# Guanys-dar/GM-Diffusion

Hardware: AMD Instinct MI355X
Metric: HDR images/sec @ 512x512, 50 PNDM steps, dual-UNet (higher is better)
Workload: dtype bf16; 1 GPU; SD-v1-5 dual-UNet (SDR 4ch + GM 8ch) 512x512, 50 PNDM steps (51 iterations), CFG 7.5, batch 4/GPU, 2 VAE decodes + Eq.1 HDR tail; global_batch=4, per_gpu_batch=4, resolution=512, inference_steps=50, parallelism=prompt-batch sharding x1, RCCL broadcast of text hidden states + latents

## Files before the change

gm-diffusion_amd/csrc/gemm.hip:

```cpp
#include "gemm_shared.h"
#include <stdlib.h>
#include <type_traits>

namespace {

template <typename HT>
__device__ __forceinline__ void epilogue_store8(const GemmParams& p, int z, int m, int n, float (&v)[8]) {
    const bool vec_ok = (p.ldc % 8 == 0) && (p.sC % 8 == 0) && (p.residual == nullptr || (p.ldr % 8 == 0 && p.sR % 8 == 0));
    const int nvalid = p.N - n < 8 ? p.N - n : 8;
    const float* rb = p.rowbias ? p.rowbias + (int64_t)(m / p.rows_per_group) * p.ldrb : nullptr;
    const HT* res = p.residual ? (const HT*)p.residual + (int64_t)z * p.sR + (int64_t)m * p.ldr + n : nullptr;
    float rv[8];
    if (res) {
        if (nvalid == 8 && vec_ok) load_vec(res, rv);
        else
            for (int j = 0; j < 8; ++j) rv[j] = j < nvalid ? Elem<HT>::ld(res + j) : 0.f;
    }
#pragma unroll
    for (int j = 0; j < 8; ++j) {
        if (j < nvalid) {
            float x = v[j] * p.alpha;
            if (p.bias) x += p.bias[n + j];
            float add = 0.f;
            if (res) add += rv[j];
            if (rb) add += rb[n + j];
            v[j] = apply_act(x + add, p.act);
        }
    }
    const int64_t coff = (int64_t)z * p.sC + (int64_t)m * p.ldc + n;
    if (p.out_f32) {
        float* o = (float*)p.C + coff;
        if (nvalid == 8 && p.ldc % 4 == 0 && p.sC % 4 == 0) {
            *reinterpret_cast<float4*>(o) = make_float4(v[0], v[1], v[2], v[3]);
            *reinterpret_cast<float4*>(o + 4) = make_float4(v[4], v[5], v[6], v[7]);
        } else {
            for (int j = 0; j < nvalid; ++j) o[j] = v[j];
        }
    } else {
        HT* o = (HT*)p.C + coff;
        if (nvalid == 8 && vec_ok) store_vec(o, v);
        else
            for (int j = 0; j < nvalid; ++j) Elem<HT>::st(o + j, v[j]);
    }
}

template <typename HT>
__global__ __launch_bounds__(256) void splitk_reduce_kernel(const GemmParams p) {
    GMD_WG_TRACE_SCOPE(WGK_SPLITK_REDUCE);
    const int NC = (p.N + 7) / 8;
    const int64_t total = (int64_t)p.M * NC;
    const int64_t slab = (int64_t)p.M * p.N;
    for (int64_t i = (int64_t)blockIdx.x * blockDim.x + threadIdx.x; i < total; i += (int64_t)gridDim.x * blockDim.x) {
        const int m = (int)(i / NC), n = (int)(i - (int64_t)m * NC) * 8;
        const int nvalid = p.N - n < 8 ? p.N - n : 8;
        float v[8];
#pragma unroll
        for (int j = 0; j < 8; ++j) v[j] = 0.f;
        const float* src = p.ws + (int64_t)m * p.N + n;
        for (int s = 0; s < p.ksplit; ++s, src += slab) {
            if (nvalid == 8 && p.N % 4 == 0) {
                const float4 a = *reinterpret_cast<const float4*>(src), b = *reinterpret_cast<const float4*>(src + 4);
                v[0] += a.x; v[1] += a.y; v[2] += a.z; v[3] += a.w; v[4] += b.x; v[5] += b.y; v[6] += b.z; v[7] += b.w;
            } else {
                for (int j = 0; j < nvalid; ++j) v[j] += src[j];
            }
        }
        epilogue_store8<HT>(p, 0, m, n, v);
    }
}

template <typename HT, int TM, int TN>
__device__ __forceinline__ void epilogue_regs(const GemmParams& p, const f32x4 (&acc)[TM][TN], int mw, int nw, int frow, int fq,
                                              int z, int ks) {
    const bool vec_c = (p.ldc % 4 == 0) && (p.sC % 4 == 0);
    const bool vec_r = p.residual != nullptr && (p.ldr % 4 == 0) && (p.sR % 4 == 0);
    const bool vec_n = (p.N % 4 == 0);
    const bool vec_rb = vec_n && (p.ldrb % 4 == 0) && ((reinterpret_cast<uintptr_t>(p.rowbias) & 15) == 0);
    float bz[TN][4];
#pragma unroll
    for (int j = 0; j < TN; ++j) {
        const int n = nw + j * 16 + fq * 4;
        bz[j][0] = bz[j][1] = bz[j][2] = bz[j][3] = 0.f;
        if (p.bias && p.ksplit <= 1 && n < p.N) {
            if (n + 4 <= p.N && vec_n) {
                const float4 t = *reinterpret_cast<const float4*>(p.bias + n);
                bz[j][0] = t.x; bz[j][1] = t.y; bz[j][2] = t.z; bz[j][3] = t.w;
            } else {
                for (int e = 0; e < 4; ++e) if (n + e < p.N) bz[j][e] = p.bias[n + e];
            }
        }
    }
    if constexpr (TN % 2 == 0) {
        if (p.act == GMD_ACT_GEGLU) {
#pragma unroll
            for (int i = 0; i < TM; ++i) {
                const int m = mw + i * 16 + frow;
                if (m >= p.M) continue;
#pragma unroll
                for (int j = 0; j < TN; j += 2) {
                    const int n = nw + j * 16 + fq * 4;
                    if (n >= p.N) continue;
                    float o4[4];
#pragma unroll
                    for (int e = 0; e < 4; ++e) {
                        const float h = acc[i][j][e] * p.alpha + bz[j][e];
                        const float g = acc[i][j + 1][e] * p.alpha + bz[j + 1][e];
                        o4[e] = h * (0.5f * g * (1.0f + fast_erf(g * 0.70710678118654752440f)));
                    }
                    const int no = (nw + j * 16) / 2 + fq * 4;
                    HT* o = (HT*)p.C + (int64_t)z * p.sC + (int64_t)m * p.ldc + no;
                    *reinterpret_cast<uint2*>(o) = make_uint2(Half<HT>::pack2(o4[0], o4[1]), Half<HT>::pack2(o4[2], o4[3]));
                }
            }
            return;
        }
    }
#pragma unroll
    for (int i = 0; i < TM; ++i) {
        const int m = mw + i * 16 + frow;
        if (m >= p.M) continue;
        const float* rb = p.rowbias ? p.rowbias + (int64_t)(m / p.rows_per_group) * p.ldrb : nullptr;
#pragma unroll
        for (int j = 0; j < TN; ++j) {
            const int n = nw + j * 16 + fq * 4;
            if (n >= p.N) continue;
            const int nvalid = p.N - n < 4 ? p.N - n : 4;
            float v[4] = {acc[i][j][0], acc[i][j][1], acc[i][j][2], acc[i][j][3]};
            if (p.ksplit > 1) {
                float* o = p.ws + ((int64_t)ks * p.M + m) * p.N + n;
                if (nvalid == 4 && vec_n) *reinterpret_cast<float4*>(o) = make_float4(v[0], v[1], v[2], v[3]);
                else
                    for (int e = 0; e < nvalid; ++e) o[e] = v[e];
                continue;
            }
            float rv[4] = {0.f, 0.f, 0.f, 0.f};
            if (p.residual) {
                const HT* res = (const HT*)p.residual + (int64_t)z * p.sR + (int64_t)m * p.ldr + n;
                if (nvalid == 4 && vec_r) {
                    const uint2 w = *reinterpret_cast<const uint2*>(res);
                    Half<HT>::unpack2(w.x, rv[0], rv[1]);
                    Half<HT>::unpack2(w.y, rv[2], rv[3]);
                } else {
                    for (int e = 0; e < nvalid; ++e) rv[e] = Elem<HT>::ld(res + e);
                }
            }
            if (rb) {
                if (nvalid == 4 && vec_rb) {
                    const float4 t = *reinterpret_cast<const float4*>(rb + n);
                    rv[0] += t.x; rv[1] += t.y; rv[2] += t.z; rv[3] += t.w;
                } else {
                    for (int e = 0; e < nvalid; ++e) rv[e] += rb[n + e];
                }
            }
#pragma unroll
            for (int e = 0; e < 4; ++e) v[e] = apply_act(v[e] * p.alpha + bz[j][e] + rv[e], p.act);
            const int64_t coff = (int64_t)z * p.sC + (int64_t)m * p.ldc + n;
            if (p.out_f32) {
                float* o = (float*)p.C + coff;
                if (nvalid == 4 && vec_c) *reinterpret_cast<float4*>(o) = make_float4(v[0], v[1], v[2], v[3]);
                else
                    for (int e = 0; e < nvalid; ++e) o[e] = v[e];
            } else {
                HT* o = (HT*)p.C + coff;
                if (nvalid == 4 && vec_c) *reinterpret_cast<uint2*>(o) = make_uint2(Half<HT>::pack2(v[0], v[1]), Half<HT>::pack2(v[2], v[3]));
                else
                    for (int e = 0; e < nvalid; ++e) Elem<HT>::st(o + e, v[e]);
            }
        }
    }
}

template <typename HT, int TM, int TN>
__device__ __forceinline__ void epilogue_cols_vt(const GemmParams& p, const f32x4 (&acc)[TM][TN], float* strip, int mw, int nw, int lane) {
    constexpr int NCOL = TN * 16, ROWF = NCOL + 4;
    const int frow = lane & 15, fq = lane >> 4;
    const int b = mw / p.vt_tokens, tok0 = mw - b * p.vt_tokens;
#pragma unroll
    for (int h = 0; h < TM / 2; ++h) {
#pragma unroll
        for (int i2 = 0; i2 < 2; ++i2)
#pragma unroll
            for (int j = 0; j < TN; ++j)
                *reinterpret_cast<float4*>(strip + (i2 * 16 + frow) * ROWF + j * 16 + fq * 4) =
                    make_float4(acc[2 * h + i2][j][0], acc[2 * h + i2][j][1], acc[2 * h + i2][j][2], acc[2 * h + i2][j][3]);
        __builtin_amdgcn_wave_barrier();
#pragma unroll
        for (int k = 0; k < (NCOL + 63) / 64; ++k) {
            const int cc = lane + 64 * k < NCOL ? lane + 64 * k : NCOL - 1;
            const float bz = p.bias ? p.bias[nw + cc] : 0.f;
            unsigned pk[16];
#pragma unroll
            for (int r = 0; r < 32; r += 2)
                pk[r / 2] = Half<HT>::pack2(strip[r * ROWF + cc] * p.alpha + bz, strip[(r + 1) * ROWF + cc] * p.alpha + bz);
            if (lane + 64 * k < NCOL) {
                HT* o = (HT*)p.vt_out + ((int64_t)b * (p.N - p.vt_col0) + (nw + cc - p.vt_col0)) * p.vt_ld + tok0 + h * 32;
#pragma unroll
                for (int q = 0; q < 4; ++q) *reinterpret_cast<uint4*>(o + 8 * q) = make_uint4(pk[4 * q], pk[4 * q + 1], pk[4 * q + 2], pk[4 * q + 3]);
            }
        }
        __builtin_amdgcn_wave_barrier();
    }
}

template <typename HT, int TM, int TN, bool PLAIN>
__device__ __forceinline__ void epilogue_rows_impl(const GemmParams& p, const f32x4 (&acc)[TM][TN], float* strip, int mw, int nw, int lane,
                                                   int z) {
    static_assert(TM % 2 == 0, "halves of two 16-row tiles");
    if (p.vt_out && nw >= p.vt_col0) {
        epilogue_cols_vt<HT, TM, TN>(p, acc, strip, mw, nw, lane);
        return;
    }
    constexpr int NCOL = TN * 16, ROWF = NCOL + 4, CH = NCOL / 8;
    constexpr int ITER = (32 * CH + 63) / 64;
    const int frow = lane & 15, fq = lane >> 4;
    int g0 = 0, grem = 0;
    if (p.rowbias) {
        g0 = mw / p.rows_per_group;
        grem = mw - g0 * p.rows_per_group;
    }
    float cs[(NCOL + 63) / 64] = {}, cq[(NCOL + 63) / 64] = {};
#if defined(GMD_PP_DIAG) && defined(GMD_WG_TRACE)
    unsigned long long et[6] = {0, 0, 0, 0, 0, 0};
    int eti = 0;
#define EPI_STAMP() { unsigned long long t_; asm volatile("s_memrealtime %0\n\ts_waitcnt lgkmcnt(0)" : "=s"(t_)::"memory"); if (eti < 6) et[eti++] = t_; }
#else
#define EPI_STAMP()
#endif
    EPI_STAMP()
    static_assert(NCOL / 4 <= 32, "one bias float4 per strip row");
    uint4 resv[2][ITER];
    if (lane < NCOL / 4)
        *reinterpret_cast<float4*>(strip + lane * ROWF + NCOL) = p.bias ? *reinterpret_cast<const float4*>(p.bias + nw + lane * 4) : make_float4(0.f, 0.f, 0.f, 0.f);
    const bool rb_pre = PLAIN && p.rowbias != nullptr && p.residual == nullptr;
    auto request_residual = [&](int hh) {
#pragma unroll
        for (int t = 0; t < ITER; ++t) {
            const int idx = lane + 64 * t;
            const int r = idx / CH, c = idx - r * CH;
            if (32 * CH % 64 != 0 && r >= 32) continue;
            resv[hh & 1][t] = *reinterpret_cast<const uint4*>((const HT*)p.residual + (int64_t)z * p.sR + (int64_t)(mw + hh * 32 + r) * p.ldr + nw + c * 8);
        }
    };
    const bool res_pre = PLAIN && p.residual != nullptr;
    if (res_pre) request_residual(0);
#pragma unroll
    for (int h = 0; h < TM / 2; ++h) {
        if (rb_pre) {
#pragma unroll
            for (int t = 0; t < ITER; ++t) {
                const int idx = lane + 64 * t;
                const int r = idx / CH, c = idx - r * CH;
                if (32 * CH % 64 != 0 && r >= 32) continue;
                const int ro = h * 32 + r;
                const int grp = p.rows_per_group >= 64 ? g0 + (grem + ro >= p.rows_per_group ? 1 : 0) : (mw + ro) / p.rows_per_group;
                const float* rb = p.rowbias + (int64_t)grp * p.ldrb + nw + c * 8;
                resv[0][t] = __builtin_bit_cast(uint4, *reinterpret_cast<const float4*>(rb));
                resv[1][t] = __builtin_bit_cast(uint4, *reinterpret_cast<const float4*>(rb + 4));
            }
        }
#pragma unroll
        for (int i2 = 0; i2 < 2; ++i2)
#pragma unroll
            for (int j = 0; j < TN; ++j)
                *reinterpret_cast<float4*>(strip + (i2 * 16 + frow) * ROWF + j * 16 + fq * 4) =
                    make_float4(acc[2 * h + i2][j][0], acc[2 * h + i2][j][1], acc[2 * h + i2][j][2], acc[2 * h + i2][j][3]);
        __builtin_amdgcn_wave_barrier();
        EPI_STAMP()
        if (res_pre && h + 1 < TM / 2) request_residual(h + 1);
#pragma unroll
        for (int t = 0; t < ITER; ++t) {
            const int idx = lane + 64 * t;
            const int r = idx / CH, c = idx - r * CH;
            if (32 * CH % 64 != 0 && r >= 32) continue;
            const int m = mw + h * 32 + r, n = nw + c * 8;
            const float4 a0 = *reinterpret_cast<const float4*>(strip + r * ROWF + c * 8);
            const float4 a1 = *reinterpret_cast<const float4*>(strip + r * ROWF + c * 8 + 4);
            float v[8] = {a0.x, a0.y, a0.z, a0.w, a1.x, a1.y, a1.z, a1.w};
            float add[8] = {0.f, 0.f, 0.f, 0.f, 0.f, 0.f, 0.f, 0.f};
            if (p.residual) {
                const uint4 w = PLAIN ? resv[h & 1][t] : *reinterpret_cast<const uint4*>((const HT*)p.residual + (int64_t)z * p.sR + (int64_t)m * p.ldr + n);
                const unsigned ww[4] = {w.x, w.y, w.z, w.w};
#pragma unroll
                for (int e = 0; e < 4; ++e) Half<HT>::unpack2(ww[e], add[2 * e], add[2 * e + 1]);
            }
            if (rb_pre) {
                const float4 t0 = __builtin_bit_cast(float4, resv[0][t]), t1 = __builtin_bit_cast(float4, resv[1][t]);
                add[0] += t0.x; add[1] += t0.y; add[2] += t0.z; add[3] += t0.w; add[4] += t1.x; add[5] += t1.y; add[6] += t1.z; add[7] += t1.w;
            } else if (p.rowbias) {
                const int ro = h * 32 + r;
                const int grp = p.rows_per_group >= 64 ? g0 + (grem + ro >= p.rows_per_group ? 1 : 0) : m / p.rows_per_group;
                const float* rb = p.rowbias + (int64_t)grp * p.ldrb + n;
                const float4 t0 = *reinterpret_cast<const float4*>(rb), t1 = *reinterpret_cast<const float4*>(rb + 4);
                add[0] += t0.x; add[1] += t0.y; add[2] += t0.z; add[3] += t0.w; add[4] += t1.x; add[5] += t1.y; add[6] += t1.z; add[7] += t1.w;
            }
            const float4 b0 = *reinterpret_cast<const float4*>(strip + (2 * c) * ROWF + NCOL), b1 = *reinterpret_cast<const float4*>(strip + (2 * c + 1) * ROWF + NCOL);
            const float bz[8] = {b0.x, b0.y, b0.z, b0.w, b1.x, b1.y, b1.z, b1.w};
#pragma unroll
            for (int e = 0; e < 8; ++e) v[e] = apply_act(v[e] * p.alpha + bz[e] + add[e], PLAIN ? GMD_ACT_NONE : p.act);
            HT* o = (HT*)p.C + (int64_t)z * p.sC + (int64_t)m * p.ldc + n;
            const uint4 packed = make_uint4(Half<HT>::pack2(v[0], v[1]), Half<HT>::pack2(v[2], v[3]), Half<HT>::pack2(v[4], v[5]), Half<HT>::pack2(v[6], v[7]));
#if defined(GMD_EPI_NOSTORE)
            if (packed.x == 0x12345678u && packed.y == 0x9abcdef0u) *reinterpret_cast<uint4*>(o) = packed;
#elif defined(GMD_EPI_NT)
            __builtin_nontemporal_store(__builtin_bit_cast(u32x4, packed), reinterpret_cast<u32x4*>(o));
#else
            *reinterpret_cast<uint4*>(o) = packed;
#endif
            asm volatile("" ::: "memory");
            __builtin_amdgcn_sched_barrier(0);
            if (p.colstats) {
                const unsigned pw[4] = {packed.x, packed.y, packed.z, packed.w};
                float rv[8];
#pragma unroll
                for (int e = 0; e < 4; ++e) Half<HT>::unpack2(pw[e], rv[2 * e], rv[2 * e + 1]);
                *reinterpret_cast<float4*>(strip + r * ROWF + c * 8) = make_float4(rv[0], rv[1], rv[2], rv[3]);
                *reinterpret_cast<float4*>(strip + r * ROWF + c * 8 + 4) = make_float4(rv[4], rv[5], rv[6], rv[7]);
            }
        }
        __builtin_amdgcn_wave_barrier();
        EPI_STAMP()
        if (p.colstats) {
            colstats_pass<NCOL, ROWF>(strip, lane, cs, cq);
            __builtin_amdgcn_wave_barrier();
        }
    }
#if defined(GMD_PP_DIAG) && defined(GMD_WG_TRACE)
    if (threadIdx.x == 0 && g_wg_trace != nullptr) {
        GmdWgTraceHeader* hh = g_wg_trace;
        const unsigned hw = __builtin_amdgcn_s_getreg((31 << 11) | 4), xcc = __builtin_amdgcn_s_getreg((31 << 11) | 20);
        const unsigned shard = ((((xcc & 7u) * 8u + ((hw >> 13) & 7u)) * 2u + ((hw >> 12) & 1u)) * 16u) + ((hw >> 8) & 15u);
        unsigned long long* counters = reinterpret_cast<unsigned long long*>(hh + 1);
        const unsigned long long i2 = __hip_atomic_fetch_add(counters + 16ull * shard, 1ull, __ATOMIC_RELAXED, __HIP_MEMORY_SCOPE_WORKGROUP);
        if (i2 < hh->capacity) {
            uint4* rec = reinterpret_cast<uint4*>(counters + 16ull * hh->shards) + 2ull * (shard * hh->capacity + i2);
            rec[0] = make_uint4((unsigned)(et[1] - et[0]), (unsigned)(et[2] - et[1]), (unsigned)(et[3] - et[2]), (unsigned)(et[4] - et[3]));
            rec[1] = make_uint4(hw, (xcc & 15u) | ((unsigned)(WGK_PP | 0x80) << 8) | (0xFEu << 16), (unsigned)TN << 16, p.residual ? 1u : 0u);
        }
    }
#endif
#undef EPI_STAMP
    if (p.colstats)
        colstats_store<NCOL, ROWF>(strip, lane, cs, cq, p.cs_bucket,
                                   p.colstats + ((int64_t)(mw / (TM * 16)) * (p.N / p.cs_bucket) + nw / p.cs_bucket) * 2);
}

template <typename HT, int TM, int TN>
__device__ __forceinline__ void epilogue_rows(const GemmParams& p, const f32x4 (&acc)[TM][TN], float* strip, int mw, int nw, int lane, int z) {
    if (__builtin_expect(p.act == GMD_ACT_NONE, 1)) epilogue_rows_impl<HT, TM, TN, true>(p, acc, strip, mw, nw, lane, z);
    else epilogue_rows_impl<HT, TM, TN, false>(p, acc, strip, mw, nw, lane, z);
}

template <int TM, int TN>
__device__ __forceinline__ void epilogue_rows_slab(const GemmParams& p, const f32x4 (&acc)[TM][TN], float* strip, int mw, int nw, int lane,
                                                   int ks) {
    static_assert(TM == 4, "two halves of two 16-row tiles");
    constexpr int NCOL = TN * 16, ROWF = NCOL + 4, CH = NCOL / 4;
    constexpr int ITER = (32 * CH + 63) / 64;
    const int frow = lane & 15, fq = lane >> 4;
    float* slab = p.ws + (int64_t)ks * p.M * p.N;
#pragma unroll
    for (int h = 0; h < 2; ++h) {
#pragma unroll
        for (int i2 = 0; i2 < 2; ++i2)
#pragma unroll
            for (int j = 0; j < TN; ++j)
                *reinterpret_cast<float4*>(strip + (i2 * 16 + frow) * ROWF + j * 16 + fq * 4) =
                    make_float4(acc[2 * h + i2][j][0], acc[2 * h + i2][j][1], acc[2 * h + i2][j][2], acc[2 * h + i2][j][3]);
        __builtin_amdgcn_wave_barrier();
#pragma unroll
        for (int t = 0; t < ITER; ++t) {
            const int idx = lane + 64 * t;
            const int r = idx / CH, c = idx - r * CH;
            if (32 * CH % 64 != 0 && r >= 32) continue;
            *reinterpret_cast<float4*>(slab + (int64_t)(mw + h * 32 + r) * p.N + nw + c * 4) =
                *reinterpret_cast<const float4*>(strip + r * ROWF + c * 4);
        }
        __builtin_amdgcn_wave_barrier();
    }
}

template <int TM, int TN, int NCONS>
__device__ __forceinline__ bool splitk_fixup(const GemmParams& p, f32x4 (&acc)[TM][TN], int ks, int wid, int lane) {
    constexpr unsigned FR = TM * TN;
    const unsigned tile = blockIdx.x, ntiles = gridDim.x;
    const int last = p.ksplit - 1;
    unsigned* cnt = p.fix_cnt + tile;
    const __amdgpu_buffer_rsrc_t rs = __builtin_amdgcn_make_buffer_rsrc(p.ws, 0, (int)p.fix_bytes, 0x00020000);
    const unsigned wave_off = ((tile * NCONS + (unsigned)wid) * FR) * 1024u + (unsigned)lane * 16u;
    const unsigned slice_bytes = ntiles * NCONS * FR * 1024u;
    if (ks != last) {
        const unsigned base = (unsigned)ks * slice_bytes + wave_off;
#pragma unroll
        for (int i = 0; i < TM; ++i)
#pragma unroll
            for (int j = 0; j < TN; ++j)
                __builtin_amdgcn_raw_buffer_store_b128(__builtin_bit_cast(u32x4, acc[i][j]), rs, base + (unsigned)(i * TN + j) * 1024u, 0, 16 );
        asm volatile("s_waitcnt vmcnt(0)" ::: "memory");
        __syncthreads();
        if (threadIdx.x == 0) __hip_atomic_fetch_add(cnt, 1u, __ATOMIC_RELAXED, __HIP_MEMORY_SCOPE_AGENT);
        return false;
    }
    if (threadIdx.x == 0) {
        int spins = 0;
        while (__hip_atomic_load(cnt, __ATOMIC_RELAXED, __HIP_MEMORY_SCOPE_AGENT) != (unsigned)last && ++spins < (1 << 21)) __builtin_amdgcn_s_sleep(8);
    }
    __syncthreads();
    static_assert(TM % 2 == 0, "fragment rows are fetched in pairs");
#pragma unroll
    for (int i = 0; i < TM; i += 2) {
        f32x4 t[2][TN];
#pragma unroll
        for (int ii = 0; ii < 2; ++ii)
#pragma unroll
            for (int j = 0; j < TN; ++j)
                t[ii][j] = __builtin_bit_cast(f32x4, __builtin_amdgcn_raw_buffer_load_b128(rs, wave_off + (unsigned)((i + ii) * TN + j) * 1024u, 0, 16 ));
        for (int s = 1; s < last; ++s) {
#pragma unroll
            for (int ii = 0; ii < 2; ++ii) {
                f32x4 u[TN];
#pragma unroll
                for (int j = 0; j < TN; ++j)
                    u[j] = __builtin_bit_cast(f32x4, __builtin_amdgcn_raw_buffer_load_b128(rs, (unsigned)s * slice_bytes + wave_off + (unsigned)((i + ii) * TN + j) * 1024u, 0, 16));
#pragma unroll
                for (int j = 0; j < TN; ++j) {
                    t[ii][j] += u[j];
                    asm volatile("" : "+v"(t[ii][j])::"memory");
// ... 426 lines not shown
        if (CONV) {
            c0 += BK;
            if (c0 >= cb0 + p.cblk) {
                c0 = cb0;
                ++tap;
                newtap = true;
                if (tap == 9) { tap = 0; cb0 += p.cblk; c0 = cb0; }
            }
        }
    };
    auto wait_tiles = [&](int ahead) {
        if (ahead <= 0) { wait_vmcnt<0>(); return; }
        if (w_last) {
            if (ahead == 1) wait_vmcnt<NA + NW>();
            else wait_vmcnt<2 * (NA + NW)>();
        } else {
            if (ahead == 1) wait_vmcnt<NA + NW - 1>();
            else wait_vmcnt<2 * (NA + NW - 1)>();
        }
    };

    const int frow = lane & 15, fq = lane >> 4;
    auto compute = [&](int stage_idx) {
        const unsigned char* sA = smem + stage_idx * kStage;
        const unsigned char* sW = sA + BM * 128;
#pragma unroll
        for (int s2 = 0; s2 < 2; ++s2) {
            uint4 a[TM], b[TN];
#pragma unroll
            for (int i = 0; i < TM; ++i) a[i] = *reinterpret_cast<const uint4*>(sA + lds_off(wr * 64 + i * 16 + frow, 4 * s2 + fq));
#pragma unroll
            for (int j = 0; j < TN; ++j) b[j] = *reinterpret_cast<const uint4*>(sW + lds_off(wc * (TN * 16) + j * 16 + frow, 4 * s2 + fq));
#pragma unroll
            for (int i = 0; i < TM; ++i)
#pragma unroll
                for (int j = 0; j < TN; ++j) acc[i][j] = Half<HT>::mfma16(b[j], a[i], acc[i][j]);
        }
    };

    if (nk > 0) {
#pragma unroll
        for (int t = 0; t < D; ++t)
            if (t < nk) dma_tile(t, t);
        int st_cur = 0, st_fill = D % NST;
        for (int kt = 0; kt < nk; ++kt) {
            const int rem = nk - 1 - kt;
            wait_tiles(rem < D - 1 ? rem : D - 1);
            __syncthreads();
            if (kt + D < nk) dma_tile(kt + D, st_fill);
            compute(st_cur);
            st_cur = st_cur + 1 == NST ? 0 : st_cur + 1;
            st_fill = st_fill + 1 == NST ? 0 : st_fill + 1;
        }
    }
    const bool rows_ok = !p.out_f32 && p.ksplit <= 1 && p.act != GMD_ACT_GEGLU && m0 + BM <= p.M && n0 + BN <= p.N && (p.ldc & 7) == 0 &&
                         (p.sC & 7) == 0 && (p.residual == nullptr || ((p.ldr & 7) == 0 && (p.sR & 7) == 0)) &&
                         (p.rowbias == nullptr || ((p.ldrb & 3) == 0 && (reinterpret_cast<uintptr_t>(p.rowbias) & 15) == 0)) &&
                         (reinterpret_cast<uintptr_t>(p.bias) & 15) == 0;
    if constexpr (TN % 2 == 0) {
        if (p.act == GMD_ACT_GEGLU && !p.out_f32 && p.ksplit <= 1 && m0 + BM <= p.M && n0 + BN <= p.N && (p.ldc & 7) == 0 && (p.sC & 7) == 0 &&
            (reinterpret_cast<uintptr_t>(p.bias) & 15) == 0) {
            __syncthreads();
            constexpr int kStripG = 32 * (TN * 8 + 4);
            epilogue_rows_geglu<HT, TM, TN>(p, acc, reinterpret_cast<float*>(smem) + wid * kStripG, m0 + wr * 64, n0 + wc * (TN * 16), lane, z);
            return;
        }
    }
    if (p.ksplit > 1 && m0 + BM <= p.M && n0 + BN <= p.N && (p.N & 3) == 0) {
        __syncthreads();
        constexpr int kStripS = 32 * (TN * 16 + 4);
        epilogue_rows_slab<TM, TN>(p, acc, reinterpret_cast<float*>(smem) + wid * kStripS, m0 + wr * 64, n0 + wc * (TN * 16), lane, ks);
        return;
    }
    if (__builtin_expect(rows_ok, 1)) {
        __syncthreads();
        constexpr int kStrip = 32 * (TN * 16 + 4);
        static_assert((size_t)NWAVES * kStrip * 4 <= (size_t)NST * kStage, "epilogue strips must fit in the ring stages");
        epilogue_rows<HT, TM, TN>(p, acc, reinterpret_cast<float*>(smem) + wid * kStrip, m0 + wr * 64, n0 + wc * (TN * 16), lane, z);
    } else {
        epilogue_regs<HT, TM, TN>(p, acc, m0 + wr * 64, n0 + wc * (TN * 16), frow, fq, z, ks);
    }
}

template <typename HT, bool CONV, int TN>
__global__ __launch_bounds__(768, 3) void gemm_pp_kernel(const GemmParams p) {
    GMD_WG_TRACE_SCOPE(WGK_PP | (CONV ? WGK_CONV_BIT : 0));
    constexpr int WN = 2, NCONS = 8, LW = 4, TM = 4, NST = 3;
    constexpr int BM = 256, BN = WN * TN * 16;
    constexpr int RPP = LW * 8;
    constexpr int NA = BM / RPP;
    constexpr int NW = BN / RPP;
    constexpr int NP = NA + NW;
    static_assert(BN % RPP == 0, "W tile rows must be whole staging passes");
    extern __shared__ __attribute__((aligned(16))) unsigned char smem[];
    constexpr int kStage = (BM + BN) * 128;

    const int tid = threadIdx.x, lane = tid & 63, wid = tid >> 6;
    const int wuni = __builtin_amdgcn_readfirstlane(wid);
    const bool loader = wuni >= NCONS;
    const bool late = wuni >= 4 && !loader;
    int m0, n0;
    {
        const int nwg = gridDim.x, id = blockIdx.x;
        const int q = nwg >> 3, r = nwg & 7, xcd = id & 7, j = id >> 3;
        const int L = (xcd < r ? xcd * (q + 1) : r * (q + 1) + (xcd - r) * q) + j;
        const int tiles_n = (p.N + BN - 1) / BN, tiles_m = (p.M + BM - 1) / BM;
        int mt, nt;
        grouped_tile(L, tiles_m, tiles_n, p.tile_group, mt, nt);
        m0 = mt * BM;
        n0 = nt * BN;
    }
    const int z = p.ksplit > 1 ? 0 : blockIdx.z;
    const int ks = p.ksplit > 1 ? blockIdx.z : 0;
    const int nk_total = p.K / BK;
    const int per = (nk_total + p.ksplit - 1) / p.ksplit;
    const int kt_begin = ks * per;
    const int nk = (kt_begin + per <= nk_total ? per : nk_total - kt_begin);

    auto seg_barrier = [&]() {
        __builtin_amdgcn_sched_barrier(0);
        __builtin_amdgcn_s_barrier();
        __builtin_amdgcn_sched_barrier(0);
    };
#ifdef GMD_PP_DIAG
    unsigned long long dg[8] = {0, 0, 0, 0, 0, 0, 0, 0}, dprev = 0, dreal0 = 0, dtime0 = 0;
    auto stamp_now = [&]() {
        unsigned long long t;
        __builtin_amdgcn_sched_barrier(0);
        asm volatile("s_memtime %0\n\ts_waitcnt lgkmcnt(0)" : "=s"(t)::"memory");
        __builtin_amdgcn_sched_barrier(0);
        return t;
    };
    auto diag_begin = [&]() {
        dprev = stamp_now();
        dtime0 = dprev;
        asm volatile("s_memrealtime %0\n\ts_waitcnt lgkmcnt(0)" : "=s"(dreal0)::"memory");
    };
    auto diag_end = [&]() {
        unsigned long long dreal1;
        asm volatile("s_memrealtime %0\n\ts_waitcnt lgkmcnt(0)" : "=s"(dreal1)::"memory");
        dg[7] = dreal1 - dreal0;
#ifdef GMD_WG_TRACE
        if (lane == 0 && g_wg_trace != nullptr) {
            GmdWgTraceHeader* h = g_wg_trace;
            const unsigned hw = __builtin_amdgcn_s_getreg((31 << 11) | 4), xcc = __builtin_amdgcn_s_getreg((31 << 11) | 20);
            const unsigned shard = ((((xcc & 7u) * 8u + ((hw >> 13) & 7u)) * 2u + ((hw >> 12) & 1u)) * 16u) + ((hw >> 8) & 15u);
            unsigned long long* counters = reinterpret_cast<unsigned long long*>(h + 1);
            const unsigned long long i = __hip_atomic_fetch_add(counters + 16ull * shard, 1ull, __ATOMIC_RELAXED, __HIP_MEMORY_SCOPE_WORKGROUP);
            if (i < h->capacity) {
                uint4* rec = reinterpret_cast<uint4*>(counters + 16ull * h->shards) + 2ull * (shard * h->capacity + i);
                const unsigned a0 = (unsigned)(loader ? dg[1] : dg[0]), a1 = (unsigned)dg[3], a2 = (unsigned)(loader ? 0 : dg[4]), a3 = (unsigned)(loader ? dg[6] : dg[5]);
                rec[0] = make_uint4(a0, a1, a2, a3);
                rec[1] = make_uint4(hw, (xcc & 15u) | ((unsigned)((WGK_PP | (CONV ? WGK_CONV_BIT : 0)) | 0x80) << 8) | ((unsigned)wid << 16), (unsigned)nk | ((unsigned)TN << 16),
                                    (unsigned)(dprev - dtime0));
            }
        }
#else
        if (p.ws && lane == 0) {
            unsigned long long* o = reinterpret_cast<unsigned long long*>(p.ws) + ((size_t)blockIdx.x * (NCONS + LW) + wid) * 10;
            for (int k = 0; k < 8; ++k) o[k] = dg[k];
            o[8] = dprev - dtime0;
            o[9] = (unsigned long long)nk;
        }
#endif
    };
#define PP_STAMP(k) { const unsigned long long t_ = stamp_now(); dg[k] += t_ - dprev; dprev = t_; }
#else
#define PP_STAMP(k)
#endif

    if (loader) {
        const int lw = wuni - NCONS;
        const int ltid = tid - NCONS * 64;
        const int srow = ltid >> 3;
        const int chunk = (ltid & 7) ^ ((srow >> 1) & 7);
        unsigned aoff[NA], woff[NW];
        int pb[NA], py[NA], px[NA];
        bool pv[NA];
#pragma unroll
        for (int i = 0; i < NA; ++i) {
            const int m = m0 + srow + RPP * i;
            pv[i] = m < p.M;
            pb[i] = py[i] = px[i] = 0;
            if (CONV) {
                if (pv[i]) {
                    const int hw = p.Hout * p.Wout;
                    if (((hw & (hw - 1)) | (p.Wout & (p.Wout - 1))) == 0) {
                        const int sh = __builtin_ctz(hw), sw = __builtin_ctz(p.Wout);
                        pb[i] = m >> sh;
                        const int rem = m & (hw - 1);
                        py[i] = rem >> sw;
                        px[i] = rem & (p.Wout - 1);
                    } else {
                        pb[i] = m / hw;
                        const int rem = m - pb[i] * hw;
                        py[i] = rem / p.Wout;
                        px[i] = rem - py[i] * p.Wout;
                    }
                }
                aoff[i] = kOOB;
            } else {
                aoff[i] = pv[i] ? (unsigned)m * (unsigned)p.lda * 2u + (unsigned)chunk * 16u : kOOB;
            }
        }
#pragma unroll
        for (int i = 0; i < NW; ++i) {
            const int n = n0 + srow + RPP * i;
            woff[i] = n < p.N ? (unsigned)n * (unsigned)p.ldw * 2u + (unsigned)chunk * 16u : kOOB;
        }
        int tap = 0, c0 = 0, cb0 = 0;
        bool newtap = true;
        if (CONV) {
            const int sb = p.cblk / BK, per_cb = 9 * sb, nconv = 9 * (p.Cin / BK);
            if (kt_begin >= nconv) {
                tap = 9;
                cb0 = p.Cin;
                c0 = (kt_begin - nconv) * BK;
            } else {
                const int cbi = kt_begin / per_cb, rem = kt_begin - cbi * per_cb;
                tap = rem / sb;
                cb0 = cbi * p.cblk;
                c0 = cb0 + (rem - tap * sb) * BK;
            }
        }
        const unsigned lds_base = __builtin_amdgcn_readfirstlane((unsigned)(size_t)(__attribute__((address_space(3))) void*)smem);
        u32x4 dA, dW;
        {
            const uint64_t ba = (uint64_t)((const bf16_t*)p.A + (int64_t)z * p.sA), bw = (uint64_t)((const bf16_t*)p.W + (int64_t)z * p.sW);
            dA = u32x4{(unsigned)__builtin_amdgcn_readfirstlane((unsigned)ba), (unsigned)__builtin_amdgcn_readfirstlane((unsigned)(ba >> 32) & 0xffffu),
                       (unsigned)__builtin_amdgcn_readfirstlane(p.a_bytes), 0x00020000u};
            dW = u32x4{(unsigned)__builtin_amdgcn_readfirstlane((unsigned)bw), (unsigned)__builtin_amdgcn_readfirstlane((unsigned)(bw >> 32) & 0xffffu),
                       (unsigned)__builtin_amdgcn_readfirstlane(p.w_bytes), 0x00020000u};
        }
        u32x4 dA2 = dA;
        if (CONV && p.K2 > 0) {
            const uint64_t b2 = (uint64_t)p.A2;
            dA2 = u32x4{(unsigned)__builtin_amdgcn_readfirstlane((unsigned)b2), (unsigned)__builtin_amdgcn_readfirstlane((unsigned)(b2 >> 32) & 0xffffu),
                        (unsigned)__builtin_amdgcn_readfirstlane(p.a2_bytes), 0x00020000u};
        }
        auto dma16 = [&](const u32x4& desc, unsigned lds_addr, unsigned voff, unsigned soff) {
#pragma clang diagnostic push
#pragma clang diagnostic ignored "-Winline-asm"
            asm volatile("s_mov_b32 m0, %1\n\ts_nop 0\n\tbuffer_load_dwordx4 %0, %2, %3 offen lds"
                         :
                         : "v"(voff), "s"(lds_addr), "s"(desc), "s"(soff)
                         : "memory", "m0");
#pragma clang diagnostic pop
        };
        auto dma_part = [&](auto QC, int kt, int stage_idx) {
            constexpr int Q = decltype(QC)::value;
            constexpr int lo = Q == 4 ? 0 : Q * NP / 4, hi = Q == 4 ? NP : (Q + 1) * NP / 4;
            unsigned kbytes = (unsigned)(kt_begin + kt) * (BK * 2);
            unsigned abytes = kbytes;
            const bool tail = CONV && tap == 9;
            if (CONV) {
                if ((Q == 0 || Q == 4) && newtap) {
                    if (tail) {
#pragma unroll
                        for (int i = 0; i < NA; ++i)
                            aoff[i] = pv[i] ? (unsigned)(m0 + srow + RPP * i) * (unsigned)p.lda2 * 2u + (unsigned)chunk * 16u : kOOB;
                    } else {
                        const int ky = tap / 3, kx = tap - ky * 3;
#pragma unroll
                        for (int i = 0; i < NA; ++i) aoff[i] = conv_tap_offset<CONV>(p, pv[i], pb[i], py[i], px[i], ky, kx, chunk);
                    }
                    newtap = false;
                }
                abytes = (unsigned)c0 * 2u;
                kbytes = (unsigned)((tail ? 9 * p.Cin : tap * p.Cin) + c0) * 2u;
            }
            const u32x4 dAs = tail ? dA2 : dA;
            const unsigned stage = lds_base + (unsigned)stage_idx * kStage + (unsigned)lw * (8 * 128);
#pragma unroll
            for (int i = 0; i < NA; ++i)
                if (i >= lo && i < hi) dma16(dAs, stage + i * (RPP * 128), aoff[i], abytes);
#pragma unroll
            for (int i = 0; i < NW; ++i)
                if (NA + i >= lo && NA + i < hi) dma16(dW, stage + BM * 128 + i * (RPP * 128), woff[i], kbytes);
            if (CONV && (Q == 3 || Q == 4)) {
                c0 += BK;
                if (tap < 9 && c0 >= cb0 + p.cblk) {
                    c0 = cb0;
                    ++tap;
                    newtap = true;
                    if (tap == 9) {
                        cb0 += p.cblk;
                        if (cb0 >= p.Cin) c0 = 0;
                        else { tap = 0; c0 = cb0; }
                    }
                }
            }
        };
        if (nk > 0) {
            dma_part(IntC<4>{}, 0, 0);
            if (nk > 1) {
                dma_part(IntC<4>{}, 1, 1);
                wait_vmcnt<NP>();
            } else {
                wait_vmcnt<0>();
            }
            seg_barrier();
            int st_fill = 2;
#ifdef GMD_PP_DIAG
            diag_begin();
#endif
            for (int kt = 0; kt < nk; ++kt) {
                const bool more = kt + 2 < nk;
                if (more) dma_part(IntC<0>{}, kt + 2, st_fill);
                PP_STAMP(1)
                seg_barrier();
                PP_STAMP(3)
                if (more) dma_part(IntC<1>{}, kt + 2, st_fill);
                PP_STAMP(1)
                seg_barrier();
                PP_STAMP(3)
                if (more) dma_part(IntC<2>{}, kt + 2, st_fill);
                PP_STAMP(1)
                seg_barrier();
                PP_STAMP(3)
                if (more) dma_part(IntC<3>{}, kt + 2, st_fill);
                PP_STAMP(1)
                if (more) wait_vmcnt<NP>();
                else wait_vmcnt<0>();
                PP_STAMP(6)
                seg_barrier();
                PP_STAMP(3)
                st_fill = st_fill == NST - 1 ? 0 : st_fill + 1;
            }
#ifdef GMD_PP_DIAG
            diag_end();
#endif
            seg_barrier();
        }
        __syncthreads();
        return;
    }

    const int wr = wid / WN, wc = wid % WN;
    f32x4 acc[TM][TN];
#pragma unroll
    for (int i = 0; i < TM; ++i)
#pragma unroll
        for (int j = 0; j < TN; ++j) acc[i][j] = f32x4{0.f, 0.f, 0.f, 0.f};
    const int frow = lane & 15, fq = lane >> 4;
    uint4 fa[TM], fb[TN];
    auto frag_reads = [&](int stage_idx, int s2) {
        const unsigned char* sA = smem + stage_idx * kStage;
        const unsigned char* sW = sA + BM * 128;
#pragma unroll
        for (int i = 0; i < TM; ++i) fa[i] = *reinterpret_cast<const uint4*>(sA + lds_off(wr * 64 + i * 16 + frow, 4 * s2 + fq));
#pragma unroll
        for (int j = 0; j < TN; ++j) fb[j] = *reinterpret_cast<const uint4*>(sW + lds_off(wc * (TN * 16) + j * 16 + frow, 4 * s2 + fq));
    };
    auto mfmas = [&]() {
#pragma unroll
        for (int i = 0; i < TM; ++i)
#pragma unroll
            for (int j = 0; j < TN; ++j) acc[i][j] = Half<HT>::mfma16(fb[j], fa[i], acc[i][j]);
    };
    auto lgkm0 = [&]() { asm volatile("s_waitcnt lgkmcnt(0)" ::: "memory"); };

    if (nk > 0) {
        seg_barrier();
        if (late) seg_barrier();
        int st = 0;
#ifdef GMD_PP_DIAG
        diag_begin();
#endif
        for (int kt = 0; kt < nk; ++kt) {
#pragma unroll
            for (int s2 = 0; s2 < 2; ++s2) {
                frag_reads(st, s2);
                lgkm0();
                PP_STAMP(0)
                seg_barrier();
                PP_STAMP(3)
                __builtin_amdgcn_s_setprio(1);
                mfmas();
                __builtin_amdgcn_s_setprio(0);
                PP_STAMP(4)
                seg_barrier();
                PP_STAMP(5)
            }
            st = st == NST - 1 ? 0 : st + 1;
        }
#ifdef GMD_PP_DIAG
        diag_end();
#endif
        if (!late) seg_barrier();
    }
#if defined(GMD_PP_DIAG) && defined(GMD_WG_TRACE)
    unsigned long long ph_sync = 0;
    auto real_now = [&]() { unsigned long long t; asm volatile("s_memrealtime %0\n\ts_waitcnt lgkmcnt(0)" : "=s"(t)::"memory"); return t; };
    auto phase_emit = [&]() {
        if (wid != 0 || lane != 0 || g_wg_trace == nullptr || nk <= 0) return;
        const unsigned long long t_end = real_now();
        GmdWgTraceHeader* h = g_wg_trace;
        const unsigned hw = __builtin_amdgcn_s_getreg((31 << 11) | 4), xcc = __builtin_amdgcn_s_getreg((31 << 11) | 20);
        const unsigned shard = ((((xcc & 7u) * 8u + ((hw >> 13) & 7u)) * 2u + ((hw >> 12) & 1u)) * 16u) + ((hw >> 8) & 15u);
        unsigned long long* counters = reinterpret_cast<unsigned long long*>(h + 1);
        const unsigned long long i2 = __hip_atomic_fetch_add(counters + 16ull * shard, 1ull, __ATOMIC_RELAXED, __HIP_MEMORY_SCOPE_WORKGROUP);
        if (i2 < h->capacity) {
            uint4* rec = reinterpret_cast<uint4*>(counters + 16ull * h->shards) + 2ull * (shard * h->capacity + i2);
            rec[0] = make_uint4((unsigned)(dreal0 - gmd_wg_trace_scope_.t0), (unsigned)dg[7], (unsigned)(ph_sync - (dreal0 + dg[7])), (unsigned)(t_end - ph_sync));
            rec[1] = make_uint4(hw, (xcc & 15u) | ((unsigned)((WGK_PP | (CONV ? WGK_CONV_BIT : 0)) | 0x80) << 8) | (0xFFu << 16), (unsigned)nk | ((unsigned)TN << 16),
                                (gridDim.x * gridDim.z) | ((unsigned)p.ksplit << 20) | (p.residual ? (1u << 28) : 0u) | (p.fixup ? (1u << 29) : 0u));
        }
    };
#define PP_PHASE_SYNC() ph_sync = real_now()
#define PP_PHASE_EMIT() phase_emit()
#else
#define PP_PHASE_SYNC()
#define PP_PHASE_EMIT()
#endif
    __syncthreads();
    GemmParams q = p;
    if (p.fixup) {
        if (!splitk_fixup<TM, TN, NCONS>(p, acc, ks, wid, lane)) return;
        q.ksplit = 1;
    }
    PP_PHASE_SYNC();
    const bool rows_ok = !q.out_f32 && q.ksplit <= 1 && q.act != GMD_ACT_GEGLU && m0 + BM <= q.M && n0 + BN <= q.N && (q.ldc & 7) == 0 &&
                         (q.sC & 7) == 0 && (q.residual == nullptr || ((q.ldr & 7) == 0 && (q.sR & 7) == 0)) &&
                         (q.rowbias == nullptr || ((q.ldrb & 3) == 0 && (reinterpret_cast<uintptr_t>(q.rowbias) & 15) == 0)) &&
                         (reinterpret_cast<uintptr_t>(q.bias) & 15) == 0;
    if constexpr (TN % 2 == 0) {
        if (q.act == GMD_ACT_GEGLU && !q.out_f32 && q.ksplit <= 1 && m0 + BM <= q.M && n0 + BN <= q.N && (q.ldc & 7) == 0 && (q.sC & 7) == 0 &&
            (reinterpret_cast<uintptr_t>(q.bias) & 15) == 0) {
            constexpr int kStripG = 32 * (TN * 8 + 4);
            epilogue_rows_geglu<HT, TM, TN>(q, acc, reinterpret_cast<float*>(smem) + wid * kStripG, m0 + wr * 64, n0 + wc * (TN * 16), lane, z);
            PP_PHASE_EMIT();
            return;
        }
    }
    if (__builtin_expect(q.ksplit > 1 && m0 + BM <= q.M && n0 + BN <= q.N && (q.N & 3) == 0, 0)) {
        constexpr int kStripS = 32 * (TN * 16 + 4);
        epilogue_rows_slab<TM, TN>(q, acc, reinterpret_cast<float*>(smem) + wid * kStripS, m0 + wr * 64, n0 + wc * (TN * 16), lane, ks);
        PP_PHASE_EMIT();
        return;
    }
    if (__builtin_expect(rows_ok, 1)) {
        constexpr int kStrip = 32 * (TN * 16 + 4);
        static_assert((size_t)NCONS * kStrip * 4 <= (size_t)NST * kStage, "epilogue strips must fit in the ring stages");
        epilogue_rows<HT, TM, TN>(q, acc, reinterpret_cast<float*>(smem) + wid * kStrip, m0 + wr * 64, n0 + wc * (TN * 16), lane, z);
    } else {
        epilogue_regs<HT, TM, TN>(q, acc, m0 + wr * 64, n0 + wc * (TN * 16), frow, fq, z, ks);
    }
    PP_PHASE_EMIT();
}
#undef PP_STAMP
#undef PP_PHASE_SYNC
#undef PP_PHASE_EMIT

template <typename HT, bool CONV, int TM, int TN>
__global__ __launch_bounds__(512, 2) void gemm_lc_kernel(const GemmParams p) {
    GMD_WG_TRACE_SCOPE(WGK_LC | (CONV ? WGK_CONV_BIT : 0));
    constexpr int WN = 2, NCONS = 4, LW = 4, NST = 4;
    constexpr int BM = 2 * TM * 16, BN = WN * TN * 16;
    constexpr int RPP = LW * 8;
    constexpr int NA = BM / RPP, NW = BN / RPP, NP = NA + NW;
    static_assert(BM % RPP == 0 && BN % RPP == 0, "tile rows must be whole staging passes");
    extern __shared__ __attribute__((aligned(16))) unsigned char smem[];
    constexpr int kStage = (BM + BN) * 128;

    const int tid = threadIdx.x, lane = tid & 63, wid = tid >> 6;
    const int wuni = __builtin_amdgcn_readfirstlane(wid);
    const bool loader = wuni >= NCONS;
    int m0, n0;
    {
        const int nwg = gridDim.x, id = blockIdx.x;
        const int q = nwg >> 3, r = nwg & 7, xcd = id & 7, j = id >> 3;
        const int L = (xcd < r ? xcd * (q + 1) : r * (q + 1) + (xcd - r) * q) + j;
        const int tiles_n = (p.N + BN - 1) / BN, tiles_m = (p.M + BM - 1) / BM;
        int mt, nt;
        grouped_tile(L, tiles_m, tiles_n, p.tile_group, mt, nt);
        m0 = mt * BM;
        n0 = nt * BN;
    }
    const int z = p.ksplit > 1 ? 0 : blockIdx.z;
    const int ks = p.ksplit > 1 ? blockIdx.z : 0;
    const int nk_total = p.K / BK;
    const int per = (nk_total + p.ksplit - 1) / p.ksplit;
    const int kt_begin = ks * per;
    const int nk = (kt_begin + per <= nk_total ? per : nk_total - kt_begin);
    auto seg_barrier = [&]() {
        __builtin_amdgcn_sched_barrier(0);
        __builtin_amdgcn_s_barrier();
        __builtin_amdgcn_sched_barrier(0);
    };

    if (loader) {
        const int lw = wuni - NCONS;
        const int ltid = tid - NCONS * 64;
        const int srow = ltid >> 3;
        const int chunk = (ltid & 7) ^ ((srow >> 1) & 7);
        unsigned aoff[NA], woff[NW];
        int pb[NA], py[NA], px[NA];
        bool pv[NA];
#pragma unroll
        for (int i = 0; i < NA; ++i) {
            const int m = m0 + srow + RPP * i;
            pv[i] = m < p.M;
            pb[i] = py[i] = px[i] = 0;
            if (CONV) {
// ... 711 lines not shown
        for (int j = 0; j < 4; ++j) {
            const int n = n0 + tx * 4 + j;
            if (n >= p.N) continue;
            float x = acc[i][j] * p.alpha;
            if (p.bias) x += p.bias[n];
            if (rb) x += rb[n];
            if (res) x += res[n];
            o[n] = apply_act(x, p.act);
        }
    }
}

template <typename HT, bool CONV, int BM, int BN, int PF>
hipError_t launch_bf16(const GemmParams& p, int gz, hipStream_t s) {
    constexpr size_t smem = 2 * (BM + BN) * 128;
    if (smem > 64 * 1024) {
        hipError_t e = opt_in_lds(reinterpret_cast<const void*>(&gemm_bf16_kernel<HT, CONV, BM, BN, PF>), (int)smem);
        if (e != hipSuccess) return e;
    }
    dim3 grid(((p.N + BN - 1) / BN) * ((p.M + BM - 1) / BM), 1, gz);
    gemm_bf16_kernel<HT, CONV, BM, BN, PF><<<grid, 256, smem, s>>>(p);
    return hipGetLastError();
}

template <typename HT, bool CONV, int WM, int WN, int TN, int NST>
hipError_t launch_ring(const GemmParams& p, int gz, hipStream_t s) {
    constexpr int BM = WM * 64, BN = WN * TN * 16;
    constexpr size_t smem = (size_t)NST * (BM + BN) * 128;
    if (smem > 64 * 1024) {
        hipError_t e = opt_in_lds(reinterpret_cast<const void*>(&gemm_ring_kernel<HT, CONV, WM, WN, TN, NST>), (int)smem);
        if (e != hipSuccess) return e;
    }
    dim3 grid(((p.N + BN - 1) / BN) * ((p.M + BM - 1) / BM), 1, gz);
    gemm_ring_kernel<HT, CONV, WM, WN, TN, NST><<<grid, WM * WN * 64, smem, s>>>(p);
    return hipGetLastError();
}

template <typename HT, bool CONV, int TM, int TN>
hipError_t launch_lc(const GemmParams& p, int gz, hipStream_t s) {
    constexpr int BM = 2 * TM * 16, BN = 2 * TN * 16;
    constexpr size_t smem = (size_t)4 * (BM + BN) * 128;
    hipError_t e = opt_in_lds(reinterpret_cast<const void*>(&gemm_lc_kernel<HT, CONV, TM, TN>), (int)smem);
    if (e != hipSuccess) return e;
    dim3 grid(((p.N + BN - 1) / BN) * ((p.M + BM - 1) / BM), 1, gz);
    gemm_lc_kernel<HT, CONV, TM, TN><<<grid, 512, smem, s>>>(p);
    return hipGetLastError();
}

template <typename HT, int TN>
hipError_t launch_conv_patch(const GemmParams& p, bool continuous, int gz, hipStream_t s) {
    constexpr int BM = 256, BN = 2 * TN * 16;
    const int H = p.Hin, W = p.Win, HW = H * W;
    const int R = HW >= 256 ? 256 / W : H, nimg = 256 / (R * W);
    const int npieces = (nimg * (R + 2) * (W + 2) + 7) / 8;
    const size_t smem = (size_t)2 * npieces * 1024 + (size_t)3 * BN * 128;
    const size_t strips = (size_t)8 * 32 * (TN * 16 + 4) * 4;
    const size_t need = smem > strips ? smem : strips;
    dim3 grid(((p.N + BN - 1) / BN) * ((p.M + BM - 1) / BM), 1, gz);
    hipError_t e;
    if (continuous) {
        if (npieces > 44) {
            e = opt_in_lds(reinterpret_cast<const void*>(&conv_patch_cont_kernel<HT, TN, 13>), 163840);
            if (e != hipSuccess) return e;
            conv_patch_cont_kernel<HT, TN, 13><<<grid, 768, need, s>>>(p);
        } else {
            e = opt_in_lds(reinterpret_cast<const void*>(&conv_patch_cont_kernel<HT, TN, 11>), 163840);
            if (e != hipSuccess) return e;
            conv_patch_cont_kernel<HT, TN, 11><<<grid, 768, need, s>>>(p);
        }
        return hipGetLastError();
    }
    if (npieces > 44) {
        e = opt_in_lds(reinterpret_cast<const void*>(&conv_patch_kernel<HT, TN, 13>), 163840);
        if (e != hipSuccess) return e;
        conv_patch_kernel<HT, TN, 13><<<grid, 768, need, s>>>(p);
    } else {
        e = opt_in_lds(reinterpret_cast<const void*>(&conv_patch_kernel<HT, TN, 11>), 163840);
        if (e != hipSuccess) return e;
        conv_patch_kernel<HT, TN, 11><<<grid, 768, need, s>>>(p);
    }
    return hipGetLastError();
}

template <typename HT, bool CONV, int TN>
hipError_t launch_pp(const GemmParams& p, int gz, hipStream_t s) {
    constexpr int BM = 256, BN = 2 * TN * 16;
    constexpr size_t smem = (size_t)3 * (BM + BN) * 128;
    hipError_t e = opt_in_lds(reinterpret_cast<const void*>(&gemm_pp_kernel<HT, CONV, TN>), (int)smem);
    if (e != hipSuccess) return e;
    dim3 grid(((p.N + BN - 1) / BN) * ((p.M + BM - 1) / BM), 1, gz);
    gemm_pp_kernel<HT, CONV, TN><<<grid, 768, smem, s>>>(p);
    return hipGetLastError();
}

template <typename HT, bool CONV>
int launch_half(GemmParams p, int batch, void* ws, int64_t ws_bytes, hipStream_t s, const char* name) {
    constexpr bool kTune = std::is_same<HT, bf16_t>::value;
    hipError_t e = hipSuccess;
    const PlanConfig cfg = plan_config();
    const int64_t usable = ws ? ws_bytes : 0;
    const Plan pl = make_plan(cfg, p.M, p.N, p.K, batch, usable, p.act == GMD_ACT_GEGLU, p.colstats != nullptr);
    if (p.vt_out && !qkv_vt_plan_ok(pl, p.M, p.N, batch, p.vt_col0, p.vt_tokens)) {
        gmd_set_error("%s: plan %dx%d ksplit=%d cannot write transposed V tiles (ask gmd_gemm_qkv_vt_ok first)", name, pl.bm, pl.bn, pl.ksplit);
        return GMD_ERR_UNSUPPORTED;
    }
    if (const char* why = plan_unsupported(cfg, pl, p, batch, usable)) {
        gmd_set_error("%s: plan %dx%d pf=%d ksplit=%d (M=%d N=%d bucket=%d) %s", name, pl.bm, pl.bn, pl.pf, pl.ksplit, p.M, p.N, p.cs_bucket, why);
        return GMD_ERR_UNSUPPORTED;
    }
    if (CONV && p.K2 > 0 && !(pl.pf == kPingPong && pl.bm == 256 && (pl.bn == 160 || pl.bn == 128))) {
        gmd_set_error("%s: plan %dx%d pf=%d has no K-tail loader (M=%d N=%d K=%d): only the 256-row ping-pong kernel does", name, pl.bm, pl.bn,
                      pl.pf, p.M, p.N, p.K);
        return GMD_ERR_INVALID;
    }
    p.ksplit = pl.ksplit;
    p.ws = (float*)ws;
    p.tile_group = CONV ? 1 : pick_tile_group(pl, p.M, p.N, p.K);
    const int gz = pl.ksplit > 1 ? pl.ksplit : batch;
    p.fixup = 0;
    if (fixup_plan_ok(cfg, pl, p.M, p.N, usable, p.defer_reduce != 0)) {
        p.fixup = 1;
        p.fix_bytes = (unsigned)fixup_bytes(pl, p.M, p.N);
        p.fix_cnt = reinterpret_cast<unsigned*>(reinterpret_cast<char*>(ws) + ws_bytes);
    }
    bool done = false;
    if (pl.pf == kLoaderConsumer) {
        if (pl.bm == 128 && pl.bn == 160) e = launch_lc<HT, CONV, 4, 5>(p, gz, s);
        else if (pl.bm == 128 && pl.bn == 128) e = launch_lc<HT, CONV, 4, 4>(p, gz, s);
        else if (pl.bm == 64 && pl.bn == 160) e = launch_lc<HT, CONV, 2, 5>(p, gz, s);
        else if (pl.bm == 64 && pl.bn == 128) e = launch_lc<HT, CONV, 2, 4>(p, gz, s);
        else { gmd_set_error("%s: loader/consumer tile %dx%d is not instantiated", name, pl.bm, pl.bn); return GMD_ERR_UNSUPPORTED; }
        done = true;
    } else if (CONV && (p.K2 == 0 || cfg.conv_patch_mode == 2) && use_conv_patch(cfg, pl, p)) {
        if (pl.bn == 160) e = launch_conv_patch<HT, 5>(p, cfg.conv_patch_mode == 2, gz, s);
        else if (pl.bn == 128) e = launch_conv_patch<HT, 4>(p, cfg.conv_patch_mode == 2, gz, s);
        else { gmd_set_error("%s: ping-pong tile %dx%d is not instantiated", name, pl.bm, pl.bn); return GMD_ERR_UNSUPPORTED; }
        done = true;
    } else if (pl.pf == kPingPong) {
        if (pl.bm == 256 && pl.bn == 160) e = launch_pp<HT, CONV, 5>(p, gz, s);
        else if (pl.bm == 256 && pl.bn == 128) e = launch_pp<HT, CONV, 4>(p, gz, s);
        else { gmd_set_error("%s: ping-pong tile %dx%d is not instantiated", name, pl.bm, pl.bn); return GMD_ERR_UNSUPPORTED; }
        done = true;
    } else if constexpr (kTune) {
        done = true;
        if (pl.pf == 143 && pl.bn == 160) e = launch_ring<HT, CONV, 4, 2, 5, 3>(p, gz, s);
        else if (pl.pf == 143 && pl.bn == 128) e = launch_ring<HT, CONV, 4, 2, 4, 3>(p, gz, s);
        else if (pl.pf == 123 && pl.bn == 160) e = launch_ring<HT, CONV, 2, 2, 5, 3>(p, gz, s);
        else if (pl.pf == 124 && pl.bn == 160) e = launch_ring<HT, CONV, 2, 2, 5, 4>(p, gz, s);
        else if (pl.pf == 122 && pl.bn == 160) e = launch_ring<HT, CONV, 2, 2, 5, 2>(p, gz, s);
        else if (pl.pf == 122 && pl.bn == 128) e = launch_ring<HT, CONV, 2, 2, 4, 2>(p, gz, s);
        else if (pl.pf == 123 && pl.bn == 128) e = launch_ring<HT, CONV, 2, 2, 4, 3>(p, gz, s);
        else if (pl.pf == 124 && pl.bn == 128) e = launch_ring<HT, CONV, 2, 2, 4, 4>(p, gz, s);
        else if (pl.pf == 103 && pl.bm == 64 && pl.bn == 64) e = launch_ring<HT, CONV, 1, 4, 1, 3>(p, gz, s);
        else if (pl.pf == 104 && pl.bm == 64 && pl.bn == 64) e = launch_ring<HT, CONV, 1, 4, 1, 4>(p, gz, s);
        else if (pl.pf == 103 && pl.bm == 64 && pl.bn == 128) e = launch_ring<HT, CONV, 1, 4, 2, 3>(p, gz, s);
        else if (pl.pf == 104 && pl.bm == 64 && pl.bn == 128) e = launch_ring<HT, CONV, 1, 4, 2, 4>(p, gz, s);
        else if (is_ring_variant(pl.pf)) { gmd_set_error("%s: ring variant %d not instantiated for BN=%d", name, pl.pf, pl.bn); return GMD_ERR_UNSUPPORTED; }
        else if (pl.pf != kRing && pl.bm == 128 && pl.bn == 160)
            e = pl.pf == kRegStaged1 ? launch_bf16<HT, CONV, 128, 160, 1>(p, gz, s) : launch_bf16<HT, CONV, 128, 160, 2>(p, gz, s);
        else if (pl.pf != kRing && pl.bm == 128 && pl.bn == 128)
            e = pl.pf == kRegStaged1 ? launch_bf16<HT, CONV, 128, 128, 1>(p, gz, s) : launch_bf16<HT, CONV, 128, 128, 2>(p, gz, s);
        else if (pl.pf != kRing && !(pl.bm == 128))
            e = pl.pf == kRegStaged1 ? launch_bf16<HT, CONV, 64, 64, 1>(p, gz, s) : launch_bf16<HT, CONV, 64, 64, 2>(p, gz, s);
        else done = false;
    } else if (pl.pf != kRing) {
        gmd_set_error("%s: plan override pf=%d is instantiated for bfloat16 only", name, pl.pf);
        return GMD_ERR_UNSUPPORTED;
    }
    if (!done) {
        if (pl.bm == 128 && pl.bn == 160) e = launch_ring<HT, CONV, 2, 2, 5, 2>(p, gz, s);
        else if (pl.bm == 128 && pl.bn == 128) e = launch_ring<HT, CONV, 2, 2, 4, 2>(p, gz, s);
        else if (pl.bm == 64 && pl.bn == 64) e = launch_bf16<HT, CONV, 64, 64, 0>(p, gz, s);
        else { gmd_set_error("%s: tile %dx%d is not instantiated", name, pl.bm, pl.bn); return GMD_ERR_UNSUPPORTED; }
    }
    if (e == hipSuccess && pl.ksplit > 1 && !p.defer_reduce && !p.fixup) {
        const int64_t total = (int64_t)p.M * ((p.N + 7) / 8);
        int64_t g = (total + 255) / 256;
        if (g > 4096) g = 4096;
        splitk_reduce_kernel<HT><<<(int)g, 256, 0, s>>>(p);
        e = hipGetLastError();
    }
    if (e != hipSuccess) {
        gmd_set_error("%s: launch failed: %s", name, hipGetErrorString(e));
        return GMD_ERR_LAUNCH;
    }
    return GMD_OK;
}

template <bool CONV>
int launch(GemmParams p, int dtype, int batch, void* ws, int64_t ws_bytes, hipStream_t s, const char* name) {
    if (dtype == GMD_BF16) return launch_half<bf16_t, CONV>(p, batch, ws, ws_bytes, s, name);
    if (dtype == GMD_F16) return launch_half<f16_t, CONV>(p, batch, ws, ws_bytes, s, name);
    if (p.colstats) {
        gmd_set_error("%s: column statistics are implemented for the 16-bit types only", name);
        return GMD_ERR_UNSUPPORTED;
    }
    p.ksplit = 1;
    p.ws = nullptr;
    dim3 grid((p.N + 63) / 64, (p.M + 63) / 64, batch);
    gemm_f32_kernel<CONV><<<grid, 256, 0, s>>>(p);
    const hipError_t e = hipGetLastError();
    if (e != hipSuccess) {
        gmd_set_error("%s: launch failed: %s", name, hipGetErrorString(e));
        return GMD_ERR_LAUNCH;
    }
    return GMD_OK;
}

}

extern "C" {

int gmd_gemm_qkv_vt(const void* A, const void* W, void* C, void* Vt, int dtype, int M, int N, int K, int64_t ldc, int vt_col0, int vt_tokens,
                    int64_t vt_ld, float alpha, void* workspace, int64_t workspace_bytes, gmd_stream_t stream) {
    workspace_bytes = gmd_ws_usable_bytes(workspace_bytes);
    const bool split = dtype == GMD_F32SW || dtype == GMD_F32SA;
    GMD_REQUIRE(gmd_is_half(dtype) || split, "gmd_gemm_qkv_vt: the 16-bit types and GMD_F32SW / GMD_F32SA only (dtype %d)", dtype);
    GMD_REQUIRE(M > 0 && N > 0 && K > 0 && K % (split ? 32 : 64) == 0, "gmd_gemm_qkv_vt: bad shape M=%d N=%d K=%d", M, N, K);
    GMD_REQUIRE(A && W && C && Vt && gmd_aligned16(A) && gmd_aligned16(W) && gmd_aligned16(C) && gmd_aligned16(Vt), "gmd_gemm_qkv_vt: null or unaligned pointer");
    GMD_REQUIRE(vt_col0 > 0 && vt_col0 < N && ldc >= vt_col0 && ldc % 8 == 0 && vt_tokens > 0 && M % vt_tokens == 0 && vt_ld >= vt_tokens && vt_ld % 8 == 0,
                "gmd_gemm_qkv_vt: bad V geometry (vt_col0=%d ldc=%lld tokens=%d vt_ld=%lld)", vt_col0, (long long)ldc, vt_tokens, (long long)vt_ld);
    GMD_REQUIRE(!split || ((reinterpret_cast<uintptr_t>(W) & 127) == 0 && (dtype != GMD_F32SA || (reinterpret_cast<uintptr_t>(A) & 127) == 0)),
                "gmd_gemm_qkv_vt: a pre-split operand must be 128-byte aligned (32-element chunks of [hi | lo])");
    GMD_REQUIRE(qkv_vt_ok(plan_config(), dtype, M, N, K, vt_col0, vt_tokens, workspace ? workspace_bytes : 0), "gmd_gemm_qkv_vt: this launch cannot write transposed V tiles (ask gmd_gemm_qkv_vt_ok)");
    GemmParams p{};
    p.A = A; p.W = W; p.C = C; p.M = M; p.N = N; p.K = K;
    p.lda = K; p.ldw = K; p.ldc = ldc;
    {
        const int es = split ? 4 : 2;
        const int64_t ab = (int64_t)M * K * es, wb = (int64_t)N * K * es;
        GMD_REQUIRE(ab < 0xFFFF0000LL && wb < 0xFFFF0000LL, "gmd_gemm_qkv_vt: operand slab larger than 4 GiB");
        p.a_bytes = (unsigned)ab; p.w_bytes = (unsigned)wb;
    }
    p.rows_per_group = 1; p.ldrb = N; p.alpha = alpha; p.act = GMD_ACT_NONE; p.cblk = K;
    p.vt_out = Vt; p.vt_col0 = vt_col0; p.vt_tokens = vt_tokens; p.vt_ld = vt_ld;
    if (split) {
        p.out_f32 = 1;
        return gmd_launch_split_gemm(p, dtype == GMD_F32SA ? 2 : 1, 1, workspace, workspace_bytes, (hipStream_t)stream, "gmd_gemm_qkv_vt");
    }
    return launch<false>(p, dtype, 1, workspace, workspace_bytes, (hipStream_t)stream, "gmd_gemm_qkv_vt");
}

int gmd_gemm_nt(const void* A, const void* W, void* C, int dtype, int out_dtype, int M, int N, int K, int64_t lda,
                int64_t ldw, int64_t ldc, int batch, int64_t strideA, int64_t strideW, int64_t strideC, const float* bias,
                const float* rowbias, int rows_per_group, int64_t ldrb, const void* residual, int64_t ldr, int64_t strideR, float alpha,
                int act, float* colstats, int colstats_bucket, void* workspace, int64_t workspace_bytes, gmd_stream_t stream) {
    workspace_bytes = gmd_ws_usable_bytes(workspace_bytes);
    const bool split = gmd_is_split(dtype);
    GMD_REQUIRE(dtype == GMD_BF16 || dtype == GMD_F16 || dtype == GMD_F32 || split, "gmd_gemm_nt: bad dtype %d", dtype);
    const bool is16 = gmd_is_half(dtype);
    const bool c_split = split && out_dtype == GMD_F32SA;
    GMD_REQUIRE(out_dtype == GMD_F32 || (!split && out_dtype == dtype) || c_split, "gmd_gemm_nt: out_dtype must be F32 or the input dtype");
    GMD_REQUIRE(M >= 0 && N >= 0 && K > 0 && batch >= 0, "gmd_gemm_nt: bad shape M=%d N=%d K=%d batch=%d", M, N, K, batch);
    if (c_split) {
        const int nout = act == GMD_ACT_GEGLU ? N / 2 : N;
        GMD_REQUIRE(batch == 1 && nout % 32 == 0 && ldc == nout && !colstats && f32_out_ok(M, N, K, act == GMD_ACT_GEGLU, workspace ? workspace_bytes : 0),
                    "gmd_gemm_nt: this launch cannot store its output pre-split (ask gmd_gemm_out_split_ok; ldc must equal the row length)");
    }
    if (M == 0 || N == 0 || batch == 0) return GMD_OK;
    const int kmul = is16 ? 64 : split ? 32 : 4, vec = is16 ? 8 : 4;
    GMD_REQUIRE(K % kmul == 0, "gmd_gemm_nt: K=%d must be a multiple of %d", K, kmul);
    GMD_REQUIRE(lda >= K && ldw >= K && (ldc >= N || act == GMD_ACT_GEGLU), "gmd_gemm_nt: leading dimension too small");
    GMD_REQUIRE(lda % vec == 0 && ldw % vec == 0 && strideA % vec == 0 && strideW % vec == 0,
                "gmd_gemm_nt: lda/ldw/strides must be multiples of %d elements", vec);
    GMD_REQUIRE(A && W && C && gmd_aligned16(A) && gmd_aligned16(W) && gmd_aligned16(C), "gmd_gemm_nt: null or unaligned pointer");
    if (dtype == GMD_F32SW || dtype == GMD_F32SA)
        GMD_REQUIRE(ldw % 32 == 0 && strideW % 32 == 0 && (reinterpret_cast<uintptr_t>(W) & 127) == 0,
                    "gmd_gemm_nt: a pre-split W operand needs ldw and strideW multiples of 32 elements and a 128-byte aligned base");
    if (dtype == GMD_F32SA)
        GMD_REQUIRE(lda % 32 == 0 && strideA % 32 == 0 && (reinterpret_cast<uintptr_t>(A) & 127) == 0,
                    "gmd_gemm_nt: a pre-split A operand (GMD_F32SA) needs lda and strideA multiples of 32 elements and a 128-byte aligned base");
// ... 38 lines not shown
    void* Ynorm;
    int G;
    float eps;
    const float* gamma;
    const float* beta;
    int silu;
};

int conv3x3_impl(const void* X, const void* Wt, void* Y, int dtype, int out_dtype, int B, int Hin, int Win, int Cin, int Cout,
                 int stride, int upsample, int pad_mode, const float* bias, const float* rowbias, int64_t ldrb, const void* residual,
                 float alpha, float* colstats, int colstats_bucket, void* workspace, int64_t workspace_bytes, gmd_stream_t stream,
                 const GnTail* gn, const void* X2 = nullptr, int K2 = 0, int64_t ldx2 = 0) {
    const bool split = gmd_is_split(dtype);
    GMD_REQUIRE(dtype == GMD_BF16 || dtype == GMD_F16 || dtype == GMD_F32 || split, "gmd_conv3x3: bad dtype %d", dtype);
    const bool is16 = gmd_is_half(dtype);
    GMD_REQUIRE(out_dtype == GMD_F32 || (!split && out_dtype == dtype), "gmd_conv3x3: out_dtype must be F32 or the input dtype");
    GMD_REQUIRE(B >= 0 && Hin > 0 && Win > 0 && Cin > 0 && Cout > 0, "gmd_conv3x3: bad shape");
    if (B == 0) return GMD_OK;
    GMD_REQUIRE(stride == 1 || stride == 2, "gmd_conv3x3: stride must be 1 or 2");
    GMD_REQUIRE(!(upsample && stride != 1), "gmd_conv3x3: upsample requires stride 1");
    GMD_REQUIRE(pad_mode == 0 || (pad_mode == 1 && stride == 2 && !upsample), "gmd_conv3x3: pad_mode 1 requires stride 2");
    int Hout, Wout, pad_lo;
    if (!conv_out_shape(Hin, Win, stride, upsample, pad_mode, Hout, Wout, pad_lo)) return GMD_ERR_INVALID;
    const int kmul = is16 ? 64 : split ? 32 : 16;
    GMD_REQUIRE(Cin % kmul == 0, "gmd_conv3x3: Cin=%d must be a multiple of %d (pad the channels)", Cin, kmul);
    GMD_REQUIRE(X && Wt && (Y || gn) && gmd_aligned16(X) && gmd_aligned16(Wt) && gmd_aligned16(Y), "gmd_conv3x3: null or unaligned pointer");
    GMD_REQUIRE(bias == nullptr || gmd_aligned16(bias), "gmd_conv3x3: bias must be 16-byte aligned (it is read with float4 loads)");
    GMD_REQUIRE(residual == nullptr || gmd_aligned16(residual), "gmd_conv3x3: unaligned residual");
    GMD_REQUIRE(residual == nullptr || out_dtype == dtype || !is16, "gmd_conv3x3: residual needs out_dtype == dtype");
    const int64_t M = (int64_t)B * Hout * Wout;
    GMD_REQUIRE(M < (1LL << 31), "gmd_conv3x3: too many output pixels");
    if (X2 || K2) {
        GMD_REQUIRE(is16, "gmd_conv3x3_tail: the 16-bit types only (dtype %d)", dtype);
        GMD_REQUIRE(stride == 1 && !upsample && pad_mode == 0 && !gn, "gmd_conv3x3_tail: stride 1, no upsampling, no fused GroupNorm");
        GMD_REQUIRE(K2 > 0 && K2 % 64 == 0, "gmd_conv3x3_tail: K2=%d must be a positive multiple of 64", K2);
        GMD_REQUIRE(X2 && gmd_aligned16(X2) && ldx2 >= K2 && ldx2 % 8 == 0, "gmd_conv3x3_tail: null or unaligned X2, or bad ldx2=%lld", (long long)ldx2);
    }
    GemmParams p{};
    p.A = X; p.W = Wt; p.C = Y; p.M = (int)M; p.N = Cout; p.K = 9 * Cin + K2;
    p.lda = Cin; p.ldw = 9 * (int64_t)Cin + K2; p.ldc = Cout;
    {
        const int es = is16 ? 2 : 4;
        const int64_t ab = (int64_t)B * Hin * Win * Cin * es, wb = (int64_t)Cout * (9 * (int64_t)Cin + K2) * es;
        const int64_t a2b = K2 ? ((M - 1) * ldx2 + K2) * es : 0;
        GMD_REQUIRE(!(is16 || split) || (ab < 0xFFFF0000LL && wb < 0xFFFF0000LL && a2b < 0xFFFF0000LL), "gmd_conv3x3: tensor larger than 4 GiB");
        p.a_bytes = (unsigned)ab; p.w_bytes = (unsigned)wb; p.a2_bytes = (unsigned)a2b;
    }
    p.A2 = X2; p.K2 = K2; p.lda2 = ldx2;
    p.bias = bias; p.rowbias = rowbias; p.rows_per_group = Hout * Wout; p.ldrb = ldrb > 0 ? ldrb : Cout;
    p.residual = residual; p.ldr = Cout; p.alpha = alpha; p.act = GMD_ACT_NONE;
    p.out_f32 = out_dtype == GMD_F32;
    p.Hin = Hin; p.Win = Win; p.Cin = Cin; p.Hout = Hout; p.Wout = Wout; p.stride = stride; p.upsample = upsample; p.pad_lo = pad_lo;
    const PlanConfig cfg = plan_config();
    p.cblk = conv_channel_block(cfg, B, Hin, Win, Cin, Cout, dtype);
    p.colstats = colstats; p.cs_bucket = colstats_bucket;
    int ks = 1;
    if (gn) {
        const int act_dtype = split ? GMD_F32 : dtype;
        ks = workspace ? conv_plan_ksplit(cfg, dtype, M, Cin, Cout, workspace_bytes) : 1;
        if (ks <= 1 || colstats || out_dtype != act_dtype || !gmd_gn_from_slabs_ok(act_dtype, B, (int64_t)Hout * Wout, Cout, gn->G)) {
            gmd_set_error("gmd_conv3x3_groupnorm: this launch does not fuse (split-K factor %d; ask gmd_conv3x3_gn_fusable first)", ks);
            return GMD_ERR_UNSUPPORTED;
        }
        p.defer_reduce = 1;
    }
    const int rc = split ? gmd_launch_split_conv(p, dtype == GMD_F32SA ? 2 : dtype == GMD_F32SW ? 1 : 0, workspace, workspace_bytes, (hipStream_t)stream, "gmd_conv3x3")
                         : launch<true>(p, dtype, 1, workspace, workspace_bytes, (hipStream_t)stream, "gmd_conv3x3");
    if (rc != GMD_OK || !gn) return rc;
    return gmd_launch_gn_from_slabs((const float*)workspace, ks, alpha, bias, rowbias, p.ldrb, residual, Y, gn->Ynorm, split ? GMD_F32 : dtype, B,
                                    (int64_t)Hout * Wout, Cout, gn->G, gn->eps, gn->gamma, gn->beta, gn->silu, (hipStream_t)stream);
}

}

extern "C" {

int gmd_conv3x3(const void* X, const void* Wt, void* Y, int dtype, int out_dtype, int B, int Hin, int Win, int Cin, int Cout,
                int stride, int upsample, int pad_mode, const float* bias, const float* rowbias, int64_t ldrb, const void* residual,
                float alpha, float* colstats, int colstats_bucket, void* workspace, int64_t workspace_bytes, gmd_stream_t stream) {
    return conv3x3_impl(X, Wt, Y, dtype, out_dtype, B, Hin, Win, Cin, Cout, stride, upsample, pad_mode, bias, rowbias, ldrb, residual, alpha,
                        colstats, colstats_bucket, workspace, gmd_ws_usable_bytes(workspace_bytes), stream, nullptr);
}

int gmd_conv3x3_tail(const void* X, const void* X2, const void* Wt, void* Y, int dtype, int out_dtype, int B, int Hin, int Win, int Cin, int K2,
                     int64_t ldx2, int Cout, int stride, int upsample, int pad_mode, const float* bias, const float* rowbias, int64_t ldrb,
                     const void* residual, float alpha, float* colstats, int colstats_bucket, void* workspace, int64_t workspace_bytes,
                     gmd_stream_t stream) {
    GMD_REQUIRE(X2 && K2 > 0, "gmd_conv3x3_tail: no second operand (X2 NULL or K2=%d)", K2);
    return conv3x3_impl(X, Wt, Y, dtype, out_dtype, B, Hin, Win, Cin, Cout, stride, upsample, pad_mode, bias, rowbias, ldrb, residual, alpha,
                        colstats, colstats_bucket, workspace, gmd_ws_usable_bytes(workspace_bytes), stream, nullptr, X2, K2, ldx2);
}

int gmd_conv3x3_gn_fusable(int dtype, int B, int Hin, int Win, int Cin, int Cout, int stride, int upsample, int pad_mode, int groups,
                           int64_t workspace_bytes) {
    workspace_bytes = gmd_ws_usable_bytes(workspace_bytes);
    const bool split = gmd_is_split(dtype);
    if (!(gmd_is_half(dtype) || split) || B <= 0 || Hin <= 0 || Win <= 0 || Cin <= 0 || Cout <= 0 || groups <= 0) return 0;
    if (!(stride == 1 || stride == 2) || (upsample && stride != 1) || !(pad_mode == 0 || (pad_mode == 1 && stride == 2 && !upsample))) return 0;
    int Hout, Wout, pad_lo;
    if (!conv_out_shape(Hin, Win, stride, upsample, pad_mode, Hout, Wout, pad_lo)) return 0;
    const int64_t M = (int64_t)B * Hout * Wout;
    if (M >= (1LL << 31) || Cin % (split ? 32 : 64)) return 0;
    if ((int64_t)B * groups < 256) return 0;
    return conv_plan_ksplit(plan_config(), dtype, M, Cin, Cout, workspace_bytes) > 1 &&
           gmd_gn_from_slabs_ok(split ? GMD_F32 : dtype, B, (int64_t)Hout * Wout, Cout, groups) ? 1 : 0;
}

int gmd_conv3x3_groupnorm(const void* X, const void* Wt, void* Yraw, void* Ynorm, int dtype, int B, int Hin, int Win, int Cin, int Cout,
                          int stride, int upsample, int pad_mode, const float* bias, const float* rowbias, int64_t ldrb,
                          const void* residual, float alpha, int groups, float eps, const float* gamma, const float* beta, int silu,
                          void* workspace, int64_t workspace_bytes, gmd_stream_t stream) {
    workspace_bytes = gmd_ws_usable_bytes(workspace_bytes);
    GMD_REQUIRE(Ynorm && gamma && beta && groups > 0 && gmd_aligned16(Ynorm), "gmd_conv3x3_groupnorm: null or unaligned GroupNorm argument");
    const bool split = gmd_is_split(dtype);
    const GnTail gn{Ynorm, groups, eps, gamma, beta, silu};
    return conv3x3_impl(X, Wt, Yraw, dtype, split ? GMD_F32 : dtype, B, Hin, Win, Cin, Cout, stride, upsample, pad_mode, bias, rowbias, ldrb,
                        residual, alpha, nullptr, 0, workspace, workspace_bytes, stream, &gn);
}

}

GMD_WG_TRACE_SETTER(gemm)
```

gm-diffusion_amd/csrc/gemm_params.h:

```cpp
#pragma once
#include <stdint.h>

namespace gmd {

constexpr int BK = 64;
constexpr int BKS = 32;

struct GemmParams {
    const void* A;
    const void* W;
    void* C;
    int M, N, K;
    int64_t lda, ldw, ldc, sA, sW, sC;
    const float* bias;
    const float* rowbias;
    int rows_per_group;
    int64_t ldrb;
    const void* residual;
    int64_t ldr, sR;
    float alpha;
    int act;
    int out_f32;
    int c_split;
    unsigned a_bytes, w_bytes;
    int ksplit;
    float* ws;
    int Hin, Win, Cin, Hout, Wout, stride, upsample, pad_lo;
    int cblk;
    float* colstats;
    int cs_bucket;
    int defer_reduce;
    int tile_group;
    void* vt_out;
    int vt_col0, vt_tokens;
    int64_t vt_ld;
    int fixup;
    unsigned fix_bytes;
    unsigned* fix_cnt;
    const void* A2;
    int K2;
    int64_t lda2;
    unsigned a2_bytes;
};

constexpr int kFixupCounters = 16384;
constexpr int64_t kWsTail = (int64_t)kFixupCounters * 4;
static inline int64_t gmd_ws_usable_bytes(int64_t bytes) { return bytes > kWsTail ? bytes - kWsTail : 0; }

}
```

gm-diffusion_amd/csrc/gemm_plan.cpp:

```cpp
#include "gemm_plan.h"
#include <stdio.h>
#include <stdlib.h>

namespace gmd {

namespace {

inline int64_t cdiv(int64_t a, int64_t b) { return (a + b - 1) / b; }
inline int64_t tile_count(const Plan& pl, int M, int N) { return cdiv(M, pl.bm) * cdiv(N, pl.bn); }

bool tuning_enabled() {
    const char* t = getenv("GMD_TUNING");
    return t && t[0] == '1';
}

PlanConfig g_cfg = load_plan_config();
thread_local int t_plan_family = 0;

}

PlanConfig load_plan_config() {
    PlanConfig c{};
    const bool tuning = tuning_enabled();
    const char* e;
// ... 167 lines not shown

bool f32_colstats_ok(int M, int N, int K, int batch, int64_t ws_bytes, int bucket) {
    if (M <= 0 || N <= 0 || K <= 0 || K % BKS || batch != 1 || bucket <= 0) return false;
    const Plan pl = f32_plan(M, N, K, batch, ws_bytes, false);
    return f32_full_rows(pl, M, N, batch) && (pl.bn / 2) % bucket == 0;
}

bool f32_out_ok(int M, int N, int K, bool geglu, int64_t ws_bytes) {
    if (M <= 0 || N <= 0 || K <= 0 || K % BKS) return false;
    return f32_full_rows(f32_plan(M, N, K, 1, ws_bytes, geglu), M, N, 1);
}

bool f32_qkv_vt_ok(int M, int N, int K, int vt_col0, int vt_tokens, int64_t ws_bytes) {
    if (M <= 0 || N <= 0 || K <= 0 || K % BKS || vt_col0 <= 0 || vt_col0 >= N || vt_tokens <= 0 || vt_tokens % 64 || M % vt_tokens) return false;
    const Plan pl = f32_plan(M, N, K, 1, ws_bytes, false);
    return f32_full_rows(pl, M, N, 1) && vt_col0 % pl.bn == 0;
}

bool qkv_vt_ok(const PlanConfig& cfg, int dtype, int M, int N, int K, int vt_col0, int vt_tokens, int64_t ws_bytes) {
    if (dtype == GMD_F32SW || dtype == GMD_F32SA) return f32_qkv_vt_ok(M, N, K, vt_col0, vt_tokens, ws_bytes);
    if (!is_half(dtype) || M <= 0 || N <= 0 || K <= 0 || K % BK) return false;
    return qkv_vt_plan_ok(make_plan(cfg, M, N, K, 1, ws_bytes, false), M, N, 1, vt_col0, vt_tokens);
}

bool split_lc_fits(const PlanConfig& cfg, const Plan& pl, int M, int N, int K, int batch) {
    if (cfg.split_lc_mode == 0 || batch != 1 || pl.bm != 128 || K / BKS < 4) return false;
    if (cfg.split_lc_mode == 1) return true;
    const int64_t tiles = cdiv(M, 128) * cdiv(N, pl.bn) * (pl.ksplit > 1 ? pl.ksplit : 1);
    return tiles >= 200 && tiles <= 256;
}

int conv_channel_block(int B, int Hin, int Win, int Cin, int Cout, int elem_bytes, int step) {
    const int64_t rows_total = (int64_t)B * Hin * Win;
    const int tiles_n = (Cout + 159) / 160;
    const int64_t rows_resident = (int64_t)(64 / tiles_n > 0 ? 64 / tiles_n : 1) * 128;
    const int64_t rows = rows_total / 8 < rows_resident ? (rows_total + 7) / 8 : rows_resident;
    const int64_t budget = 3ll << 20;
    if (rows * Cin * elem_bytes <= budget) return Cin;
    int best = step;
    for (int d = step; d < Cin; d += step)
        if (Cin % d == 0 && rows * d * elem_bytes <= budget) best = d;
    return best;
}
int conv_channel_block(const PlanConfig& cfg, int B, int Hin, int Win, int Cin, int Cout, int dtype) {
    if (dtype == GMD_F32) return Cin;
    if (is_split(dtype)) return conv_channel_block(B, Hin, Win, Cin, Cout, 4, BKS);
    if (cfg.conv_cblk >= BK && cfg.conv_cblk % BK == 0 && Cin % cfg.conv_cblk == 0) return cfg.conv_cblk;
    return conv_channel_block(B, Hin, Win, Cin, Cout, 2, BK);
}

bool conv_patch_ok(const GemmParams& p) {
    const int H = p.Hin, W = p.Win, HW = H * W;
    if (p.stride != 1 || p.upsample || p.pad_lo != 1 || p.Hout != H || p.Wout != W) return false;
    if (W < 8 || W > 64 || (W & (W - 1)) || p.Cin % BK || p.M % HW) return false;
    if (HW >= 256 ? (HW % 256 != 0) : (256 % HW != 0)) return false;
    const int R = HW >= 256 ? 256 / W : H, nimg = 256 / (R * W);
    return nimg * (R + 2) * (W + 2) <= 400;
}
bool use_conv_patch(const PlanConfig& cfg, const Plan& pl, const GemmParams& p) {
    return pl.pf == kPingPong && cfg.conv_patch_mode != 0 && conv_patch_ok(p) && (int64_t)pl.ksplit <= p.Cin / BK;
}

bool conv_out_shape(int Hin, int Win, int stride, int& upsample, int pad_mode, int& Hout, int& Wout, int& pad_lo) {
    if (upsample == 1) { Hout = 2 * Hin; Wout = 2 * Win; pad_lo = 1; }
    else if (upsample) {
        Hout = upsample >> 16; Wout = upsample & 0xFFFF; pad_lo = 1;
        if (upsample < 0 || !(Hout == 2 * (int64_t)Hin - 1 || Hout == 2 * (int64_t)Hin) || !(Wout == 2 * (int64_t)Win - 1 || Wout == 2 * (int64_t)Win)) {
            gmd_set_error("gmd_conv3x3: upsample to %dx%d from %dx%d: each output side must be 2*in - 1 or 2*in", Hout, Wout, Hin, Win);
            return false;
        }
        upsample = 1;
    }
    else if (pad_mode == 1) { Hout = (Hin + 1 - 3) / 2 + 1; Wout = (Win + 1 - 3) / 2 + 1; pad_lo = 0; }
    else { Hout = (Hin + 2 - 3) / stride + 1; Wout = (Win + 2 - 3) / stride + 1; pad_lo = 1; }
    return true;
}

int conv_plan_ksplit(const PlanConfig& cfg, int dtype, int64_t M, int Cin, int Cout, int64_t ws_bytes) {
    if (is_split(dtype)) return f32_plan((int)M, Cout, 9 * Cin, 1, ws_bytes, false).ksplit;
    if (is_half(dtype)) return make_plan(cfg, (int)M, Cout, 9 * Cin, 1, ws_bytes, false).ksplit;
    return 1;
}

}

using namespace gmd;

namespace {
const char kTuningOnly[] = "%s: kernel-tuning overrides are a debug facility; set GMD_TUNING=1 in the environment to use them";
}

extern "C" {

int gmd_gemm_plan_override(int bm, int bn, int pf, int ksplit) {
    if (!(bm >= 0 && bn >= 0 && pf >= 0 && ksplit >= 0)) {
        gmd_set_error("gmd_gemm_plan_override: negative value");
        return GMD_ERR_INVALID;
    }
    if (!tuning_enabled() && (bm | bn | pf | ksplit) != 0) {
        gmd_set_error(kTuningOnly, "gmd_gemm_plan_override");
        return GMD_ERR_UNSUPPORTED;
    }
    g_cfg.force = Force{bm, bn, pf, ksplit};
    g_cfg.split_lc_mode = pf == kLoaderConsumer ? 1 : 0;
    return GMD_OK;
}

int gmd_gemm_plan_family(int family) {
    const int prev = t_plan_family;
    if (family == 0 || family == 1) t_plan_family = family;
    return prev;
}

int gmd_splitk_fixup_max(int max_slices) {
    const int prev = g_cfg.fixup_max;
    if (max_slices >= 0) g_cfg.fixup_max = max_slices > 16 ? 16 : max_slices;
    return prev;
}

int gmd_conv_patch_override(int mode) {
    if (!(mode >= 0 && mode <= 2)) {
        gmd_set_error("gmd_conv_patch_override: mode 0, 1 or 2");
        return GMD_ERR_INVALID;
    }
    if (!tuning_enabled()) {
        gmd_set_error(kTuningOnly, "gmd_conv_patch_override");
        return GMD_ERR_UNSUPPORTED;
    }
    g_cfg.conv_patch_mode = mode;
    return GMD_OK;
}

int gmd_gemm_colstats_plan(int dtype, int M, int N, int K, int batch, int64_t workspace_bytes, int bucket) {
    const int64_t ws = gmd_ws_usable_bytes(workspace_bytes);
    if (is_split(dtype)) return f32_colstats_ok(M, N, K, batch, ws, bucket);
    if (!is_half(dtype) || M <= 0 || N <= 0 || K <= 0 || K % BK != 0) return 0;
    const PlanConfig cfg = plan_config();
    return colstats_plan_ok(cfg, make_plan(cfg, M, N, K, batch, ws, false, true), M, N, batch, bucket, ws) ? 1 : 0;
}

int gmd_gemm_plan_info(int dtype, int M, int N, int K, int batch, int64_t workspace_bytes, int geglu, int* out4) {
    if (!(is_half(dtype) && M > 0 && N > 0 && K > 0 && K % BK == 0 && batch > 0 && out4)) {
        gmd_set_error("gmd_gemm_plan_info: 16-bit launches only");
        return GMD_ERR_INVALID;
    }
    const Plan pl = make_plan(plan_config(), M, N, K, batch, gmd_ws_usable_bytes(workspace_bytes), geglu != 0);
    out4[0] = pl.bm; out4[1] = pl.bn; out4[2] = pl.pf; out4[3] = pl.ksplit;
    return GMD_OK;
}

int gmd_split_plan_ksplit(int M, int N, int K, int64_t workspace_bytes) {
    if (M <= 0 || N <= 0 || K <= 0 || K % BKS) return 0;
    return f32_plan(M, N, K, 1, gmd_ws_usable_bytes(workspace_bytes), false).ksplit;
}

int gmd_gemm_out_split_ok(int M, int N, int K, int geglu, int64_t workspace_bytes) {
    return f32_out_ok(M, N, K, geglu != 0, gmd_ws_usable_bytes(workspace_bytes));
}

int gmd_gemm_qkv_vt_ok(int dtype, int M, int N, int K, int vt_col0, int vt_tokens, int64_t workspace_bytes) {
    return qkv_vt_ok(plan_config(), dtype, M, N, K, vt_col0, vt_tokens, gmd_ws_usable_bytes(workspace_bytes));
}

}
```

gm-diffusion_amd/csrc/gemm_plan.h:

```cpp
#pragma once
#include "../../include/gmd_hip.h"
#include "gemm_params.h"

void gmd_set_error(const char* fmt, ...);

namespace gmd {

enum Family : int {
    kRing = 0,
    kRegStaged1 = 1,
    kRegStaged2 = 2,
    kForceRing = 9,
    kRingVariant = 100,
    kLoaderConsumer = 244,
    kPingPong = 283,
};
inline bool is_loader_wave(int pf) { return pf == kPingPong || pf == kLoaderConsumer; }
inline bool is_ring_variant(int pf) { return pf >= kRingVariant && !is_loader_wave(pf); }
inline bool has_fixup(int pf) { return is_loader_wave(pf); }

struct Plan {
    int bm, bn, pf, ksplit;
};
inline bool wave_owns_64_rows(const Plan& pl) {
    return (pl.pf == kRing && pl.bm == 128) || (pl.pf == kPingPong && pl.bm == 256) || (pl.pf == kLoaderConsumer && pl.bm == 128);
}
inline bool even_tn(const Plan& pl) { return !(pl.bn == 160 || (is_ring_variant(pl.pf) && pl.bm == 64 && pl.bn == 64)); }

struct Force {
    int bm = 0, bn = 0, pf = 0, ks = 0;
};

struct PlanConfig {
    Force force;
    bool pp_enabled;
    int family_pin;
    int family;
    int f1_target;
    int f1_min_steps;
    bool f1_bn128;
    int fixup_max;
    int conv_patch_mode;
    int split_lc_mode;
    int conv_cblk;
};
PlanConfig load_plan_config();
PlanConfig plan_config();

Plan base_plan(int M, int N, int K, int batch, int64_t ws_bytes, bool pair_tiles, const Force& force);
Plan make_plan(const PlanConfig& cfg, int M, int N, int K, int batch, int64_t ws_bytes, bool pair_tiles, bool want_cs = false);
Plan f32_plan(int M, int N, int K, int batch, int64_t ws_bytes, bool geglu);
int64_t fixup_bytes(const Plan& pl, int M, int N);
bool fixup_plan_ok(const PlanConfig& cfg, const Plan& pl, int M, int N, int64_t ws_bytes, bool defer_reduce);
bool colstats_plan_ok(const PlanConfig& cfg, const Plan& pl, int M, int N, int batch, int bucket, int64_t ws_bytes);
bool qkv_vt_plan_ok(const Plan& pl, int M, int N, int batch, int vt_col0, int vt_tokens);
bool qkv_vt_ok(const PlanConfig& cfg, int dtype, int M, int N, int K, int vt_col0, int vt_tokens, int64_t ws_bytes);
const char* plan_unsupported(const PlanConfig& cfg, const Plan& pl, const GemmParams& p, int batch, int64_t ws_bytes);
int pick_tile_group(const Plan& pl, int M, int N, int K);

bool f32_full_rows(const Plan& pl, int M, int N, int batch);
bool f32_colstats_ok(int M, int N, int K, int batch, int64_t ws_bytes, int bucket);
bool f32_out_ok(int M, int N, int K, bool geglu, int64_t ws_bytes);
bool f32_qkv_vt_ok(int M, int N, int K, int vt_col0, int vt_tokens, int64_t ws_bytes);
bool split_lc_fits(const PlanConfig& cfg, const Plan& pl, int M, int N, int K, int batch);

int conv_channel_block(int B, int Hin, int Win, int Cin, int Cout, int elem_bytes, int step);
int conv_channel_block(const PlanConfig& cfg, int B, int Hin, int Win, int Cin, int Cout, int dtype);
bool conv_patch_ok(const GemmParams& p);
bool use_conv_patch(const PlanConfig& cfg, const Plan& pl, const GemmParams& p);
bool conv_out_shape(int Hin, int Win, int stride, int& upsample, int pad_mode, int& Hout, int& Wout, int& pad_lo);
int conv_plan_ksplit(const PlanConfig& cfg, int dtype, int64_t M, int Cin, int Cout, int64_t ws_bytes);

inline bool is_half(int dtype) { return dtype == GMD_BF16 || dtype == GMD_F16; }
inline bool is_split(int dtype) { return dtype == GMD_F32S || dtype == GMD_F32SW || dtype == GMD_F32SA; }

}
```

gm-diffusion_amd/csrc/gemm_shared.h:

```cpp
#pragma once
#include "gmd_common.h"
#include "gemm_params.h"
#include "gemm_plan.h"
#include <mutex>

using namespace gmd;

int gmd_launch_split_gemm(const GemmParams& p, int presplit, int batch, void* ws, int64_t ws_bytes, hipStream_t s, const char* name);
int gmd_launch_split_conv(const GemmParams& p, int presplit, void* ws, int64_t ws_bytes, hipStream_t s, const char* name);

namespace {

__device__ __forceinline__ void grouped_tile(int L, int tiles_m, int tiles_n, int group, int& mt, int& nt) {
    if (group <= 1) {
        mt = L / tiles_n;
        nt = L - mt * tiles_n;
        return;
    }
    const int gsz = group * tiles_n;
    const int pg = L / gsz, r = L - pg * gsz;
    const int left = tiles_m - pg * group;
    const int rows = left < group ? left : group;
    nt = r / rows;
    mt = pg * group + (r - nt * rows);
// ... 48 lines not shown
    float y = fmaf(1.061405429f, t, -1.453152027f);
    y = fmaf(y, t, 1.421413741f);
    y = fmaf(y, t, -0.284496736f);
    y = fmaf(y, t, 0.254829592f);
    y = y * t * __builtin_amdgcn_exp2f(-1.4426950408889634f * ax * ax);
    return copysignf(1.0f - y, x);
}

__device__ __forceinline__ float apply_act(float v, int act) {
    if (act == GMD_ACT_SILU) return silu_f(v);
    if (act == GMD_ACT_QUICK_GELU) return v / (1.0f + __expf(-1.702f * v));
    return v;
}

__device__ __forceinline__ float add_f32_single(float a, float b) {
    float r;
    asm volatile("v_add_f32 %0, %1, %2" : "=v"(r) : "v"(a), "v"(b));
    return r;
}

template <int NCOL, int ROWF>
__device__ __forceinline__ void colstats_pass(const float* strip, int lane, float (&cs)[(NCOL + 63) / 64], float (&cq)[(NCOL + 63) / 64]) {
#pragma unroll
    for (int k = 0; k < (NCOL + 63) / 64; ++k) {
        const int cc = lane + 64 * k < NCOL ? lane + 64 * k : NCOL - 1;
        float s_ = 0.f, q_ = 0.f;
#pragma unroll 8
        for (int r = 0; r < 32; ++r) {
            const float x = strip[r * ROWF + cc];
            s_ += x;
            q_ += x * x;
        }
        cs[k] = add_f32_single(cs[k], s_);
        cq[k] = add_f32_single(cq[k], q_);
    }
}

template <int NCOL, int ROWF>
__device__ __forceinline__ void colstats_store(float* strip, int lane, const float (&cs)[(NCOL + 63) / 64], const float (&cq)[(NCOL + 63) / 64],
                                               int bucket, float* out) {
#pragma unroll
    for (int k = 0; k < (NCOL + 63) / 64; ++k) {
        const int cc = lane + 64 * k;
        if (cc < NCOL) {
            strip[cc] = cs[k];
            strip[ROWF + cc] = cq[k];
        }
    }
    __builtin_amdgcn_wave_barrier();
    const int nb = NCOL / bucket;
    const int b0 = (lane < nb ? lane : nb - 1) * bucket;
    float s_ = 0.f, q_ = 0.f;
    for (int e = 0; e < bucket; ++e) {
        s_ = add_f32_single(s_, strip[b0 + e]);
        q_ = add_f32_single(q_, strip[ROWF + b0 + e]);
    }
    if (lane < nb) *reinterpret_cast<float2*>(out + lane * 2) = make_float2(s_, q_);
}

__device__ __forceinline__ int lds_off(int row, int chunk) { return row * 128 + ((chunk ^ ((row >> 1) & 7)) << 4); }

template <int V> struct IntC { static constexpr int value = V; };

typedef unsigned int u32x4 __attribute__((ext_vector_type(4)));
constexpr unsigned kOOB = 0xFFFF0000u;

template <bool CONV>
__device__ __forceinline__ unsigned conv_tap_offset(const GemmParams& p, bool valid, int b, int oy, int ox, int ky, int kx, int chunk) {
    if (!valid) return kOOB;
    int iy, ix;
    if (p.upsample) {
        const int uy = oy + ky - 1, ux = ox + kx - 1;
        if (uy < 0 || ux < 0 || uy >= p.Hout || ux >= p.Wout) return kOOB;
        iy = uy >> 1;
        ix = ux >> 1;
    } else {
        iy = oy * p.stride + ky - p.pad_lo;
        ix = ox * p.stride + kx - p.pad_lo;
        if (iy < 0 || ix < 0 || iy >= p.Hin || ix >= p.Win) return kOOB;
    }
    return (unsigned)(((b * p.Hin + iy) * p.Win + ix) * p.Cin) * 2u + (unsigned)chunk * 16u;
}

template <int N> __device__ __forceinline__ void wait_vmcnt() { asm volatile("s_waitcnt vmcnt(%0)" ::"n"(N) : "memory"); }

hipError_t opt_in_lds(const void* fn, int bytes) {
    constexpr int kMaxDev = 64, kMaxFn = 64;
    static const void* fns[kMaxFn];
    static unsigned long long done[kMaxFn];
    static std::mutex mu;
    int dev = 0;
    hipError_t e = hipGetDevice(&dev);
    if (e != hipSuccess) return e;
    std::lock_guard<std::mutex> lock(mu);
    int slot = -1;
    for (int i = 0; i < kMaxFn; ++i) {
        if (fns[i] == fn) { slot = i; break; }
        if (fns[i] == nullptr) { fns[i] = fn; slot = i; break; }
    }
    if (slot >= 0 && dev < kMaxDev && (done[slot] >> dev & 1ull)) return hipSuccess;
    e = hipFuncSetAttribute(fn, hipFuncAttributeMaxDynamicSharedMemorySize, bytes);
    if (e == hipSuccess && slot >= 0 && dev < kMaxDev) done[slot] |= 1ull << dev;
    return e;
}

}
```

gm-diffusion_amd/gm_diffusion/_native/__init__.py:

```python
from __future__ import annotations

import ctypes
import os
from ctypes import c_char_p, c_float, c_int, c_int64, c_void_p

_HERE = os.path.dirname(os.path.abspath(__file__))
LIB_PATH = os.environ.get("GMD_LIB_OVERRIDE") or os.path.join(_HERE, "libgmd_hip.so")
ABI_VERSION = 14

GMD_F32, GMD_BF16, GMD_F16, GMD_F32S, GMD_F32SW, GMD_F32SA = 0, 1, 2, 3, 4, 5
ACT_NONE, ACT_SILU, ACT_GEGLU, ACT_QUICK_GELU = 0, 1, 2, 3

P, I, L, F = c_void_p, c_int, c_int64, c_float

SIGNATURES = {
    "gmd_abi_version": [],
    "gmd_last_error": [],
    "gmd_hdr_tail": [P, P, I, I, I, I, I, F, F, I, P, P, P, P, P, P, P, P],
    "gmd_hdr_tail_resized": [P, I, I, P, I, I, I, I, I, I, I, F, F, I, P, P, P, P, P, P, P, P, P],
    "gmd_prepare_sdr": [P, I, I, I, P, I, I, I, I, I, P],
    "gmd_apply_gm_to_sdr": [P, P, P, L, F, F, I, P],
    "gmd_tmo": [P, P, L, I, F, F, P],
    "gmd_gamut_compress": [P, P, I, L, P],
    "gmd_stage1_chain": [P, P, P, I, L, F, P],
    "gmd_discretize_u16": [P, P, P, L, P],
    "gmd_quantize_u8": [P, P, L, P],
    "gmd_rgbe_encode": [P, P, L, P],
    "gmd_rgbe_rle_bound": [I, I],
    "gmd_rgbe_rle_encode": [P, I, I, P, L, P],
    "gmd_latent_step": [P, P, P, P, P, P, I, L, I, F, P, F, I, F, F, F, F, F, P, P, P, P],
    "gmd_dpm_step": [P, P, P, I, L, I, F, P, F, I, F, F, F, F, F, F, F, F, P, P, P, P],
    "gmd_dpm_sde_step": [P, P, P, P, I, L, I, F, P, F, I, F, F, F, F, F, F, F, F, F, P, P, P, P],
    "gmd_ddpm_step": [P, P, P, I, L, I, F, P, F, F, F, I, F, F, F, F, F, F, P, P, P],
    "gmd_ddim_step": [P, P, P, I, L, I, F, P, F, F, F, I, F, I, F, F, F, F, F, P, P, P, P],
    "gmd_lcm_step": [P, P, P, I, L, I, F, P, F, F, F, I, F, F, F, F, F, F, F, P, P, P, P],
    "gmd_euler_step": [P, P, P, I, L, I, F, P, F, F, F, F, P, P, P],
    "gmd_lms_step": [P, P, P, P, P, I, L, I, F, P, F, I, F, F, F, F, F, P, P, P, P],
    "gmd_unipc_step": [P, P, P, P, P, P, I, L, I, F, P, F, I, I] + [F] * 19 + [P, P, P, P, P],
    "gmd_cfg_std_ratio": [P, I, L, F, P, P],
    "gmd_pack_unet_input": [P, I, P, I, I, L, I, P, I, I, P],
    "gmd_pack_unet_input_scaled": [P, I, F, P, I, F, I, L, I, P, I, I, P],
    "gmd_unpack_nchw": [P, I, L, I, I, L, P, P],
    "gmd_gemm_plan_override": [I, I, I, I],
    "gmd_gemm_plan_family": [I],
    "gmd_splitk_fixup_max": [I],
    "gmd_gemm_nt": [P, P, P, I, I, I, I, I, L, L, L, I, L, L, L, P, P, I, L, P, L, L, F, I, P, I, P, L, P],
    "gmd_gemm_colstats_plan": [I, I, I, I, I, L, I],
    "gmd_gemm_plan_info": [I, I, I, I, I, L, I, P],
    "gmd_gemm_out_split_ok": [I, I, I, I, L],
    "gmd_split_plan_ksplit": [I, I, I, L],
    "gmd_gemm_qkv_vt_ok": [I, I, I, I, I, I, L],
    "gmd_gemm_qkv_vt": [P, P, P, P, I, I, I, I, L, I, I, L, F, P, L, P],
    "gmd_conv_patch_override": [I],
    "gmd_stamp": [P, P, I, I, P],
    "gmd_split_weights": [P, P, L, L, L, P],
    "gmd_ff_geglu_fused_supported": [I, L, I],
    "gmd_ff_geglu_fused": [P, P, P, P, P, P, P, I, L, I, P],
    "gmd_conv3x3": [P, P, P, I, I, I, I, I, I, I, I, I, I, P, P, L, P, F, P, I, P, L, P],
    "gmd_conv3x3_tail": [P, P, P, P, I, I, I, I, I, I, I, L, I, I, I, I, P, P, L, P, F, P, I, P, L, P],
    "gmd_conv3x3_gn_fusable": [I, I, I, I, I, I, I, I, I, I, L],
    "gmd_conv3x3_groupnorm": [P, P, P, P, I, I, I, I, I, I, I, I, I, P, P, L, P, F, I, F, P, P, I, P, L, P],
    "gmd_attention": [P, P, P, P, I, I, I, I, I, I, L, L, L, L, L, L, L, L, F, I, P],
    "gmd_softmax_rows": [P, L, P, I, L, L, I, F, I, P],
    "gmd_groupnorm_nsplit": [L],
    "gmd_groupnorm_stats": [P, I, I, L, I, I, F, P, P, P, P, P],
    "gmd_groupnorm_apply": [P, P, I, I, L, I, P, I, P],
    "gmd_groupnorm_colstats": [P, P, I, I, L, I, I, F, P, P, P, I, P, I, I, P],
    "gmd_groupnorm_split": [P, P, I, I, L, I, I, F, P, P, P, I, P],
    "gmd_groupnorm_fused": [P, P, I, I, L, I, I, F, P, P, I, P],
    "gmd_layernorm": [P, P, I, L, I, P, P, F, P],
    "gmd_geglu": [P, P, I, L, I, P],
    "gmd_timestep_embedding": [P, P, I, I, I, I, F, P],
    "gmd_timestep_embedding_add": [P, P, P, I, I, I, I, F, P],
    "gmd_concat_channels": [P, I, P, I, P, I, L, P],
    "gmd_embedding_lookup": [P, P, P, P, I, L, I, I, I, P],
    "gmd_cast": [P, I, P, I, L, P],
    "gmd_dup_batch": [P, P, L, P],
}
_RESTYPES = {"gmd_last_error": c_char_p, "gmd_rgbe_rle_bound": c_int64}


class HipExtensionError(RuntimeError):
    """libgmd_hip.so is missing/unloadable, or a kernel call returned an error."""


_lib = None


def lib():
    global _lib
    if _lib is not None:
        return _lib
    if not os.path.exists(LIB_PATH):
        raise HipExtensionError(
            f"{LIB_PATH} not found: build it with `python -c 'import __graft_entry__ as g; g.build()'` "
            "or `make -C gm-diffusion_amd/csrc`. gm_diffusion (MI355X build) has no CPU/eager fallback."
        )
    try:
        handle = ctypes.CDLL(LIB_PATH)
    except OSError as e:
        raise HipExtensionError(f"cannot load {LIB_PATH}: {e}") from e
    for name, args in SIGNATURES.items():
        fn = getattr(handle, name)
        fn.argtypes = args
        fn.restype = _RESTYPES.get(name, c_int)
    got = handle.gmd_abi_version()
    if got != ABI_VERSION:
        raise HipExtensionError(f"libgmd_hip.so ABI {got} != expected {ABI_VERSION}; rebuild")
    _lib = handle
    return handle


def check(rc, what=""):
    if rc != 0:
        msg = lib().gmd_last_error()
        raise HipExtensionError(f"{what}: gmd error {rc}: {msg.decode() if msg else '?'}")
```

gm-diffusion_amd/gm_diffusion/components/autoencoder_kl.py:

```python
from __future__ import annotations

import os
from types import SimpleNamespace

import torch

from .. import hip_ops as ops
from .._native import HipExtensionError
from .configuration import read_state_dict
from .unet_2d_condition import _HipModule, _in_own_f32_mode, _pad_to, composed_attention

SD15_VAE_DEFAULTS = dict(
    in_channels=3, out_channels=3, latent_channels=4, block_out_channels=(128, 256, 512, 512), layers_per_block=2,
    norm_num_groups=32, scaling_factor=0.18215, sample_size=512, act_fn="silu",
    down_block_types=("DownEncoderBlock2D",) * 4, up_block_types=("UpDecoderBlock2D",) * 4,
)


class DiagonalGaussianDistribution:

    def __init__(self, mean, logvar):
        self.mean = mean
        self.logvar = logvar.clamp(-30.0, 20.0)
        self.std = torch.exp(0.5 * self.logvar)
# ... 58 lines not shown
        if self.with_encoder if encoder is None else encoder:
            conv("quant_conv", 2 * lc, 2 * lc, 1)
            conv("encoder.conv_in", ch[0], c.in_channels, 3)
            cout = ch[0]
            for i in range(len(ch)):
                cin, cout = cout, ch[i]
                for j in range(c.layers_per_block):
                    resnet(f"encoder.down_blocks.{i}.resnets.{j}", cin if j == 0 else cout, cout)
                if i != len(ch) - 1:
                    conv(f"encoder.down_blocks.{i}.downsamplers.0.conv", cout, cout, 3)
            mid("encoder.mid_block", ch[-1])
            norm("encoder.conv_norm_out", ch[-1]); conv("encoder.conv_out", 2 * lc, ch[-1], 3)
        return keys

    def load_state_dict(self, sd, strict=True):
        self.with_encoder = any(k.startswith("encoder.") for k in sd)
        return super().load_state_dict(sd, strict)

    @classmethod
    def from_pretrained(cls, path, subfolder=None, torch_dtype=None, **overrides):
        d = os.path.join(path, subfolder) if subfolder else path
        cfg = cls.load_config(d)
        cfg.update(overrides)
        m = cls(**cfg)
        m.load_state_dict(read_state_dict(d))
        if torch_dtype is not None:
            m.to(torch_dtype)
        return m

    def init_random(self, seed=1334, with_encoder=False, device=None):
        self.with_encoder = with_encoder
        g = torch.Generator(device or "cpu").manual_seed(seed)
        keys = self.expected_keys()
        sd = {}
        for k, shp in keys.items():
            if "norm" in k.rsplit(".", 2)[-2]:
                sd[k] = torch.ones(shp) if k.endswith("weight") else torch.zeros(shp)
                continue
            wshape = keys[k.rsplit(".", 1)[0] + ".weight"]
            fan_in = 1
            for s_ in wshape[1:]:
                fan_in *= s_
            sd[k] = (torch.rand(shp, generator=g, device=g.device) * 2 - 1) * fan_in ** -0.5
        return self.load_state_dict(sd)

    def _prepare(self):
        c = self.config
        kmul = self._kmul()
        w = {}
        self._lc_pad = _pad_to(c.latent_channels, kmul)

        def resnet(k):
            r = dict(n1=self._norm(k + ".norm1"), c1=self._conv3(k + ".conv1"), n2=self._norm(k + ".norm2"), c2=self._conv3(k + ".conv2"))
            if k + ".conv_shortcut.weight" in self._raw:
                r["sc"] = self._lin(k + ".conv_shortcut")
                if ops.USE_SHORTCUT_FOLD and ops.is_half(self._dtype) and r["sc"][0].shape[1] % 64 == 0:
                    r["c2sc"] = ops.pack_shortcut(r["c2"][0], r["c2"][1], r["sc"][0], r["sc"][1])
            return r

        def mid(k):
            a = k + ".attentions.0"
            wq, bq = self._raw[a + ".to_q.weight"], self._raw[a + ".to_q.bias"]
            wk, bk = self._raw[a + ".to_k.weight"], self._raw[a + ".to_k.bias"]
            wv, bv = self._raw[a + ".to_v.weight"], self._raw[a + ".to_v.bias"]
            wo, bo = self._raw[a + ".to_out.0.weight"], self._raw[a + ".to_out.0.bias"]
            bo_f = (wo.double() @ bv.double() + bo.double()).float()
            return dict(r0=resnet(k + ".resnets.0"), r1=resnet(k + ".resnets.1"), gn=self._norm(a + ".group_norm"),
                        qk=self._wt(torch.cat([wq, wk], 0)), qkb=self._f32(torch.cat([bq, bk], 0)),
                        v=self._wa(wv), o=self._wt(wo), ob=self._f32(bo_f))

        rev = list(reversed(list(c.block_out_channels)))
        pq_w = torch.zeros(self._lc_pad, self._lc_pad)
        pq_w[: c.latent_channels, : c.latent_channels] = self._raw["post_quant_conv.weight"].reshape(c.latent_channels, -1)
        pq_b = torch.zeros(self._lc_pad)
        pq_b[: c.latent_channels] = self._raw["post_quant_conv.bias"]
        w["pq"] = (self._wt(pq_w), self._f32(pq_b))
        w["d_in"] = self._conv3("decoder.conv_in", self._lc_pad)
        w["d_mid"] = mid("decoder.mid_block")
        w["d_up"] = []
        for i in range(len(rev)):
            e = dict(res=[resnet(f"decoder.up_blocks.{i}.resnets.{j}") for j in range(c.layers_per_block + 1)])
            if i != len(rev) - 1:
                e["us"] = self._conv3(f"decoder.up_blocks.{i}.upsamplers.0.conv")
            w["d_up"].append(e)
        w["d_norm"] = self._norm("decoder.conv_norm_out")
        wo = self._raw["decoder.conv_out.weight"]
        t = torch.zeros(4, 3, 3, wo.shape[1])
        t[: wo.shape[0]] = wo.permute(0, 2, 3, 1)
        bo = torch.zeros(4)
        bo[: wo.shape[0]] = self._raw["decoder.conv_out.bias"]
        w["d_out"] = (self._wt(t.reshape(4, -1)), self._f32(bo))
        if self.with_encoder:
            ch = list(c.block_out_channels)
            self._img_pad = _pad_to(c.in_channels, kmul)
            w["e_in"] = self._conv3("encoder.conv_in", self._img_pad)
            w["e_down"] = []
            for i in range(len(ch)):
                e = dict(res=[resnet(f"encoder.down_blocks.{i}.resnets.{j}") for j in range(c.layers_per_block)])
                if i != len(ch) - 1:
                    e["ds"] = self._conv3(f"encoder.down_blocks.{i}.downsamplers.0.conv")
                w["e_down"].append(e)
            w["e_mid"] = mid("encoder.mid_block")
            w["e_norm"] = self._norm("encoder.conv_norm_out")
            w["e_out"] = self._conv3("encoder.conv_out")
            w["q"] = self._lin("quant_conv")
        return w

    def _resnet(self, r, x, B, H, W):
        G = self.config.norm_num_groups
        h = ops.groupnorm(x, B, G, r["n1"][0], r["n1"][1], 1e-6, silu=True)
        h, _, _ = ops.conv3x3(h, r["c1"][0], B, H, W, bias=r["c1"][1])
        h = ops.groupnorm(h, B, G, r["n2"][0], r["n2"][1], 1e-6, silu=True)
        if "sc" in r:
            if "c2sc" in r and ops.shortcut_fold_ok(self._dtype, B, H, W, h.shape[-1], x.shape[-1], r["c2sc"][0].shape[0]):
                y, _, _ = ops.conv3x3_tail(h, x, r["c2sc"][0], B, H, W, bias=r["c2sc"][1])
                return y
            ops.shortcut_launches += 1
            x = ops.gemm_nt(x.view(-1, x.shape[-1]), r["sc"][0], bias=r["sc"][1]).view(B, H * W, -1)
        y, _, _ = ops.conv3x3(h, r["c2"][0], B, H, W, bias=r["c2"][1], residual=x)
        return y

    def _mid(self, m, x, B, H, W):
        x = self._resnet(m["r0"], x, B, H, W)
        C, N = x.shape[-1], H * W
        h = ops.groupnorm(x, B, self.config.norm_num_groups, m["gn"][0], m["gn"][1], 1e-6, silu=False)
        qk = ops.gemm_nt(h.view(B * N, C), m["qk"], bias=m["qkb"])
        npad = _pad_to(N, 64 if ops.is_half(self._dtype) else 4)
        vt = torch.zeros((B, C, npad), dtype=self._dtype, device=x.device) if npad != N else None
        vt = ops.gemm_nt(m["v"], h.view(B, N, C), out=vt, ldc=npad)
        o = composed_attention(qk, 0, 2 * C, qk, C, 2 * C, vt, B, 1, C, N, N, C ** -0.5, self._dtype)
        x = ops.gemm_nt(o.view(B * N, C), m["o"], bias=m["ob"], residual=x.view(B * N, C)).view(B, N, C)
        return self._resnet(m["r1"], x, B, H, W)

    max_tensor_bytes = (1 << 32) - 1

    @_in_own_f32_mode
    def decode_nhwc(self, z):
        self._ensure()
        w = self._w
        c = self.config
        if z.dtype != torch.float32:
            z = ops.cast(z.contiguous(), torch.float32)
        B, _, H, W = z.shape
        up = 2 ** (len(c.block_out_channels) - 1)
        widest = max(c.block_out_channels[0], c.block_out_channels[min(1, len(c.block_out_channels) - 1)])
        per_image = H * up * W * up * widest * (2 if ops.is_half(self._dtype) else 4)
        max_b = max(1, self.max_tensor_bytes // per_image)
        if B > max_b:
            parts = [self.decode_nhwc(z[i:i + max_b]) for i in range(0, B, max_b)]
            return torch.cat([p[0] for p in parts]), parts[0][1], parts[0][2]
        x = ops.pack_unet_input(z.contiguous(), None, 1, self._lc_pad, self._dtype)
        x = ops.gemm_nt(x.view(B * H * W, self._lc_pad), w["pq"][0], bias=w["pq"][1]).view(B, H * W, self._lc_pad)
        x, _, _ = ops.conv3x3(x, w["d_in"][0], B, H, W, bias=w["d_in"][1])
        x = self._mid(w["d_mid"], x, B, H, W)
        for blk in w["d_up"]:
            for r in blk["res"]:
                x = self._resnet(r, x, B, H, W)
            if "us" in blk:
                x, H, W = ops.conv3x3(x, blk["us"][0], B, H, W, bias=blk["us"][1], upsample=True)
        x = ops.groupnorm(x, B, c.norm_num_groups, w["d_norm"][0], w["d_norm"][1], 1e-6, silu=True)
        y, _, _ = ops.conv3x3(x, w["d_out"][0], B, H, W, bias=w["d_out"][1], out_dtype=torch.float32)
        return y, H, W

    def decode(self, z, return_dict=True, generator=None):
        y, H, W = self.decode_nhwc(z)
        img = ops.unpack_nchw(y, z.shape[0], self.config.out_channels, H, W)
        return (img,) if not return_dict else SimpleNamespace(sample=img)

    @_in_own_f32_mode
    def encode(self, x, return_dict=True):
        self._ensure()
        if not self.with_encoder:
            raise RuntimeError("this AutoencoderKL was loaded without encoder weights")
        w = self._w
        c = self.config
        if x.dtype != torch.float32:
            x = ops.cast(x.contiguous(), torch.float32)
        B, _, H, W = x.shape
        return self.encode_nhwc(ops.pack_unet_input(x.contiguous(), None, 1, self._img_pad, self._dtype), H, W, return_dict)

    def encoder_input_spec(self):
        self._ensure()
        if not self.with_encoder:
            raise RuntimeError("this AutoencoderKL was loaded without encoder weights")
        return self._img_pad, self._dtype

    @_in_own_f32_mode
    def encode_nhwc(self, h, H, W, return_dict=True):
        self._ensure()
        if not self.with_encoder:
            raise RuntimeError("this AutoencoderKL was loaded without encoder weights")
        w = self._w
        c = self.config
        B = h.shape[0]
        if h.dim() != 3 or h.shape[1] != H * W or h.shape[2] != self._img_pad or h.dtype != self._dtype:
            raise ValueError(f"encode_nhwc expects [{B}, {H * W}, {self._img_pad}] {self._dtype}, got {tuple(h.shape)} {h.dtype}")
        h, _, _ = ops.conv3x3(h, w["e_in"][0], B, H, W, bias=w["e_in"][1])
        for blk in w["e_down"]:
            for r in blk["res"]:
                h = self._resnet(r, h, B, H, W)
            if "ds" in blk:
                h, H, W = ops.conv3x3(h, blk["ds"][0], B, H, W, bias=blk["ds"][1], stride=2, pad_mode=1)
        h = self._mid(w["e_mid"], h, B, H, W)
        h = ops.groupnorm(h, B, c.norm_num_groups, w["e_norm"][0], w["e_norm"][1], 1e-6, silu=True)
        h, _, _ = ops.conv3x3(h, w["e_out"][0], B, H, W, bias=w["e_out"][1])
        m = ops.gemm_nt(h.view(B * H * W, -1), w["q"][0], bias=w["q"][1], out_dtype=torch.float32)
        moments = ops.unpack_nchw(m.view(B, H * W, -1), B, 2 * c.latent_channels, H, W)
        dist = DiagonalGaussianDistribution(moments[:, : c.latent_channels].contiguous(), moments[:, c.latent_channels:].contiguous())
        return SimpleNamespace(latent_dist=dist) if return_dict else (dist,)
```

gm-diffusion_amd/gm_diffusion/components/unet_2d_condition.py:

```python
from __future__ import annotations

import os

import torch

from .. import hip_ops as ops
from .._native import HipExtensionError
from .configuration import ConfigMixin, read_state_dict

SD15_UNET_DEFAULTS = dict(
    sample_size=64, in_channels=4, out_channels=4, center_input_sample=False, flip_sin_to_cos=True, freq_shift=0,
    down_block_types=("CrossAttnDownBlock2D", "CrossAttnDownBlock2D", "CrossAttnDownBlock2D", "DownBlock2D"),
    up_block_types=("UpBlock2D", "CrossAttnUpBlock2D", "CrossAttnUpBlock2D", "CrossAttnUpBlock2D"),
    block_out_channels=(320, 640, 1280, 1280), layers_per_block=2, downsample_padding=1, mid_block_scale_factor=1,
    act_fn="silu", norm_num_groups=32, norm_eps=1e-5, cross_attention_dim=768, attention_head_dim=8,
    time_cond_proj_dim=None,
    transformer_layers_per_block=1, use_linear_projection=False, addition_embed_type=None, addition_time_embed_dim=None,
    projection_class_embeddings_input_dim=None,
)

SDXL_UNET_CONFIG = dict(
    block_out_channels=(320, 640, 1280), down_block_types=("DownBlock2D", "CrossAttnDownBlock2D", "CrossAttnDownBlock2D"),
    up_block_types=("CrossAttnUpBlock2D", "CrossAttnUpBlock2D", "UpBlock2D"), transformer_layers_per_block=(1, 2, 10),
    attention_head_dim=(5, 10, 20), cross_attention_dim=2048, use_linear_projection=True, addition_embed_type="text_time",
# ... 347 lines not shown
        w = {}
        self._cin_pad = _pad_to(c.in_channels, self._kmul())
        w["conv_in"] = self._conv3("conv_in", self._cin_pad)
        w["te1"] = self._lin("time_embedding.linear_1")
        w["te2"] = self._lin("time_embedding.linear_2")
        if c.time_cond_proj_dim is not None:
            wc = self._raw["time_embedding.cond_proj.weight"]
            self._tcond_k = _pad_to(wc.shape[1], self._kmul())
            wp = torch.zeros(wc.shape[0], self._tcond_k)
            wp[:, : wc.shape[1]] = wc
            w["cond_proj"] = self._wt(wp)

        te_w, te_b = [], []
        self._transformers = []

        def resnet(k):
            r = dict(n1=self._norm(k + ".norm1"), c1=self._conv3(k + ".conv1"), n2=self._norm(k + ".norm2"), c2=self._conv3(k + ".conv2"))
            r["te_off"] = sum(t.shape[0] for t in te_w)
            te_w.append(self._raw[k + ".time_emb_proj.weight"])
            te_b.append(self._raw[k + ".time_emb_proj.bias"])
            if k + ".conv_shortcut.weight" in self._raw:
                r["sc"] = self._lin(k + ".conv_shortcut")
                if ops.USE_SHORTCUT_FOLD and ops.is_half(self._dtype) and r["sc"][0].shape[1] % 64 == 0:
                    r["c2sc"] = ops.pack_shortcut(r["c2"][0], r["c2"][1], r["sc"][0], r["sc"][1])
            return r

        def transformer(k, heads, depth):
            t = dict(norm=self._norm(k + ".norm"), pin=self._lin(k + ".proj_in"), pout=self._lin(k + ".proj_out"), heads=heads, blocks=[])
            for n_ in range(depth):
                b = f"{k}.transformer_blocks.{n_}"
                blk = dict(heads=heads)
                for nm in ("norm1", "norm2", "norm3"):
                    blk[nm] = self._norm(f"{b}.{nm}")
                q1, k1 = self._raw[f"{b}.attn1.to_q.weight"], self._raw[f"{b}.attn1.to_k.weight"]
                blk["v1"] = self._wa(self._raw[f"{b}.attn1.to_v.weight"])
                blk["qkv1"] = self._wt(torch.cat([q1, k1, self._raw[f"{b}.attn1.to_v.weight"]], 0))
                blk["qk1"] = blk["qkv1"][: q1.shape[0] + k1.shape[0]] if ops.is_half(self._dtype) else self._wt(torch.cat([q1, k1], 0))
                blk["o1"] = self._lin(f"{b}.attn1.to_out.0")
                blk["q2"] = self._lin(f"{b}.attn2.to_q", False)[0]
                blk["k2"] = self._lin(f"{b}.attn2.to_k", False)[0]
                blk["v2"] = self._wa(self._raw[f"{b}.attn2.to_v.weight"])
                blk["o2"] = self._lin(f"{b}.attn2.to_out.0")
                if ops.is_half(self._dtype) or self._split_mode():
                    wf, bf = self._raw[f"{b}.ff.net.0.proj.weight"], self._raw[f"{b}.ff.net.0.proj.bias"]
                    half = wf.shape[0] // 2
                    wi = torch.stack([wf[:half].reshape(half // 16, 16, -1), wf[half:].reshape(half // 16, 16, -1)], 1).reshape(2 * half, -1)
                    bi = torch.stack([bf[:half].reshape(half // 16, 16), bf[half:].reshape(half // 16, 16)], 1).reshape(2 * half)
                    blk["ff1"] = (self._wt(wi), self._f32(bi))
                    blk["ff1_fused"] = True
                else:
                    blk["ff1"] = self._lin(f"{b}.ff.net.0.proj")
                    blk["ff1_fused"] = False
                blk["ff2"] = self._lin(f"{b}.ff.net.2")
                blk["key"] = b
                self._transformers.append(blk)
                t["blocks"].append(blk)
            return t

        downs, ups = self._layout()
        if c.addition_embed_type == "text_time":
            wa = self._raw["add_embedding.linear_1.weight"]
            self._add_k = _pad_to(wa.shape[1], self._kmul())
            wp = torch.zeros(wa.shape[0], self._add_k)
            wp[:, : wa.shape[1]] = wa
            w["add1"] = (self._wt(wp), self._f32(self._raw["add_embedding.linear_1.bias"]))
            w["add2"] = self._lin("add_embedding.linear_2")
        w["down"] = []
        for i, blk in enumerate(downs):
            e = dict(res=[resnet(f"down_blocks.{i}.resnets.{j}") for j in range(len(blk["res"]))])
            if blk["attn"]:
                e["attn"] = [transformer(f"down_blocks.{i}.attentions.{j}", blk["heads"], blk["depth"]) for j in range(len(blk["res"]))]
            if blk["down"]:
                e["ds"] = self._conv3(f"down_blocks.{i}.downsamplers.0.conv")
            w["down"].append(e)
        w["mid"] = dict(r0=resnet("mid_block.resnets.0"), a=transformer("mid_block.attentions.0", downs[-1]["heads"], downs[-1]["depth"]),
                        r1=resnet("mid_block.resnets.1"))
        w["up"] = []
        for i, blk in enumerate(ups):
            e = dict(res=[resnet(f"up_blocks.{i}.resnets.{j}") for j in range(len(blk["res"]))])
            if blk["attn"]:
                e["attn"] = [transformer(f"up_blocks.{i}.attentions.{j}", blk["heads"], blk["depth"]) for j in range(len(blk["res"]))]
            if blk["up"]:
                e["us"] = self._conv3(f"up_blocks.{i}.upsamplers.0.conv")
            w["up"].append(e)
        w["norm_out"] = self._norm("conv_norm_out")
        w["conv_out"] = self._conv3("conv_out")
        w["te_all"] = (self._wt(torch.cat(te_w, 0)), self._f32(torch.cat(te_b, 0)))
        self._kv_cache = {}
        self._graphs = {}
        self._aug = {}
        self._tcond = {}
        self._t_dev = torch.zeros(1, dtype=torch.float32, device=self._device)
        return w

    @staticmethod
    def _sa(*ws):
        return ops.USE_F32SA and all(getattr(w, "_split", False) for w in ws)

    def _resnet(self, r, x, B, H, W, temb, eps):
        G = self.config.norm_num_groups
        cs = self._wants_colstats(H, W)
        h = ops.groupnorm(x, B, G, r["n1"][0], r["n1"][1], eps, silu=True, split_out=self._sa(r["c1"][0]))
        _, h = ops.conv3x3_groupnorm(h, r["c1"][0], B, H, W, G, r["n2"][0], r["n2"][1], eps, silu=True, bias=r["c1"][1],
                                     rowbias=(temb, r["te_off"]), colstats=cs, split_out=self._sa(r["c2"][0]))
        if "sc" in r:
            cin = x.shape[-1]
            if "c2sc" in r and ops.shortcut_fold_ok(self._dtype, B, H, W, h.shape[-1], cin, r["c2sc"][0].shape[0]):
                y, _, _ = ops.conv3x3_tail(h, x, r["c2sc"][0], B, H, W, bias=r["c2sc"][1], colstats=cs)
                return y
            ops.shortcut_launches += 1
            x = ops.gemm_nt(x.view(-1, cin), r["sc"][0], bias=r["sc"][1]).view(B, H * W, -1)
        y, _, _ = ops.conv3x3(h, r["c2"][0], B, H, W, bias=r["c2"][1], residual=x, colstats=cs)
        return y

    @staticmethod
    def _wants_colstats(H, W):
        return H * W >= 1024 and (H * W) % 64 == 0

    def _self_attention(self, t, n1, B, N, C):
        heads = t["heads"]
        d = C // heads
        scale = d ** -0.5
        if "qkv1" in t and (ops.is_half(self._dtype) or ops.split_attention_ok(self._dtype, d)):
            r = ops.gemm_qkv_vt(n1, t["qkv1"], 2 * C, N)
            if r is not None:
                qk = r[0].view(B, N, 2 * C)
                return ops.attention(qk, qk, r[1], heads, N, scale, k_col=C, split_out=self._sa(t["o1"][0]))
        qk = ops.gemm_nt(n1, t["qk1"]).view(B, N, 2 * C)
        if ops.is_half(self._dtype) or ops.split_attention_ok(self._dtype, d):
            nv = n1.view(B, N, C)
            if ops.is_asplit(n1):
                nv._split, nv._alpha = True, 1.0
            vt = ops.gemm_nt(t["v1"], nv, ldc=_pad_to(N, 8 if ops.is_half(self._dtype) else 4))
            return ops.attention(qk, qk, vt, heads, N, scale, k_col=C, split_out=self._sa(t["o1"][0]))
        npad = _pad_to(N, 4)
        if npad != N:
            vt = torch.zeros((B, C, npad), dtype=self._dtype, device=n1.device)
            ops.gemm_nt(t["v1"], n1.view(B, N, C), out=vt, ldc=npad)
        else:
            vt = ops.gemm_nt(t["v1"], n1.view(B, N, C), ldc=npad)
        return composed_attention(qk, 0, 2 * C, qk, C, 2 * C, vt, B, heads, d, N, N, scale, self._dtype)

    def _cross_kv(self, t, ehs):
        key = (ehs.data_ptr(), ehs._version, tuple(ehs.shape))
        B, L, E = ehs.shape
        slot = (t["key"], B, L, self._dtype)
        ent = self._kv_cache.get(slot)
        if ent is not None and ent["key"] == key:
            return ent["kc"], ent["vt"]
        if self._capturing:
            raise HipExtensionError("cross-attention K/V must be prepared (update_context) before graph capture")
        C = t["k2"].shape[0]
        lpad = _pad_to(L, 8 if ops.is_half(self._dtype) else 4)
        if ent is None:
            ent = dict(kc=torch.empty((B, L, C), dtype=self._dtype, device=ehs.device),
                       vt=torch.zeros((B, C, lpad), dtype=self._dtype, device=ehs.device))
            self._kv_cache[slot] = ent
        ops.gemm_nt(ehs.view(B * L, E), t["k2"], out=ent["kc"].view(B * L, C))
        ops.gemm_nt(t["v2"], ehs, out=ent["vt"], ldc=lpad)
        ent["key"] = key
        ent["ehs"] = ehs
        return ent["kc"], ent["vt"]

    @_in_own_f32_mode
    def update_context(self, ehs):
        self._ensure()
# ... 136 lines not shown
                             f" on {cond.device}")
        key = (cond.data_ptr(), cond._version, B)
        ent = self._tcond.get(B)
        if ent is not None and ent["key"] == key:
            return ent["buf"]
        if self._capturing:
            raise HipExtensionError("the timestep conditioning must be prepared (set_timestep_cond) before graph capture")
        ent = self._tcond_entry(B)
        src = cond.contiguous()
        if src.dtype != self._dtype:
            src = ops.cast(src if src.dtype in (torch.float32, torch.bfloat16, torch.float16) else src.float(), self._dtype)
        if self._tcond_k != d:
            pad = torch.zeros((B, self._tcond_k), dtype=self._dtype, device=self._device)
            pad[:, :d].copy_(src)
            src = pad
        ent["buf"].copy_(ops.gemm_nt(src, self._w["cond_proj"]))
        ent["key"] = key
        ent["src"] = cond
        return ent["buf"]

    @_in_own_f32_mode
    def forward_packed(self, x, B, H, W, encoder_hidden_states, cfg_shared=False):
        w = self._w
        c = self.config
        eps = c.norm_eps
        ehs = encoder_hidden_states
        sb = getattr(self, "_stamp_buf", None)
        sk = [0]

        def mark():
            if sb is not None:
                ops.stamp(sb, sk[0], self._stamp_row)
                sk[0] += 1

        mark()
        if ehs.dtype != self._dtype:
            raise HipExtensionError("encoder_hidden_states must already be in the UNet dtype (use prepare_context)")
        if cfg_shared and (B % 2 or not self.supports_cfg_shared()):
            raise HipExtensionError("cfg_shared needs an even batch and a transformer in the first down block")
        if c.time_cond_proj_dim is None:
            te = ops.timestep_embedding(self._t_dev, B, c.block_out_channels[0], self._dtype, c.flip_sin_to_cos, c.freq_shift)
        else:
            te = ops.timestep_embedding_add(self._t_dev, self._tcond_entry(B)["buf"], B, c.block_out_channels[0], self._dtype,
                                            c.flip_sin_to_cos, c.freq_shift)
        te = ops.gemm_nt(te, w["te1"][0], bias=w["te1"][1], act=ops.ACT_SILU)
        aug = None
        if c.addition_embed_type == "text_time":
            ent = self._aug.get(B)
            if ent is None:
                raise HipExtensionError("this UNet needs its added conditioning first: set_added_cond(added_cond_kwargs, batch)")
            aug = ent["aug"]
        temb = ops.gemm_nt(te, w["te2"][0], bias=w["te2"][1], residual=aug, act=ops.ACT_SILU)
        temb = ops.gemm_nt(temb, w["te_all"][0], bias=w["te_all"][1], out_dtype=torch.float32)
        Bc = B // 2 if cfg_shared else B
        x, _, _ = ops.conv3x3(x, w["conv_in"][0], Bc, H, W, bias=w["conv_in"][1], colstats=self._wants_colstats(H, W))
        skips = [(x, H, W)]
        for blk in w["down"]:
            for j, r in enumerate(blk["res"]):
                x = self._resnet(r, x, Bc, H, W, temb[:Bc], eps)
                if "attn" in blk:
                    dup = Bc != B
                    x = self._transformer(blk["attn"][j], x, Bc, H, W, ehs, cfg_dup=dup)
                    if dup:
                        skips = [(self._dup_batch(s_), h_, w_) for s_, h_, w_ in skips]
                        Bc = B
                skips.append((x, H, W))
            if "ds" in blk:
                x, H, W = ops.conv3x3(x, blk["ds"][0], B, H, W, bias=blk["ds"][1], stride=2,
                                      colstats=self._wants_colstats((H + 1) // 2, (W + 1) // 2))
                skips.append((x, H, W))
            mark()
        x = self._resnet(w["mid"]["r0"], x, B, H, W, temb, eps)
        x = self._transformer(w["mid"]["a"], x, B, H, W, ehs)
        x = self._resnet(w["mid"]["r1"], x, B, H, W, temb, eps)
        mark()
        for blk in w["up"]:
            for j, r in enumerate(blk["res"]):
                s, _, _ = skips.pop()
                x = self._resnet(r, ops.concat_channels(x, s), B, H, W, temb, eps)
                if "attn" in blk:
                    x = self._transformer(blk["attn"][j], x, B, H, W, ehs)
            if "us" in blk:
                ho, wo = skips[-1][1:]
                x, H, W = ops.conv3x3(x, blk["us"][0], B, H, W, bias=blk["us"][1], out_size=(ho, wo), colstats=self._wants_colstats(ho, wo))
            mark()
        x = ops.groupnorm(x, B, c.norm_num_groups, w["norm_out"][0], w["norm_out"][1], eps, silu=True, split_out=self._sa(w["conv_out"][0]))
        y, _, _ = ops.conv3x3(x, w["conv_out"][0], B, H, W, bias=w["conv_out"][1], out_dtype=torch.float32)
        out = ops.unpack_nchw(y, B, c.out_channels, H, W)
        mark()
        return out

    @_in_own_f32_mode
    def graphed_forward(self, B, H, W, ehs, cfg_shared=False, co_run=False):
        self._ensure()
        self.update_context(ehs)
        if self.config.addition_embed_type is not None and B not in self._aug:
            raise HipExtensionError("set_added_cond(added_cond_kwargs, batch) must precede graphed_forward for this UNet")
        if self.config.time_cond_proj_dim is not None:
            self._tcond_entry(B)
        key = (B, H, W, tuple(ehs.shape), bool(cfg_shared), bool(co_run))
        g = self._graphs.get(key)
        if g is not None:
            return g
        from .. import profiling

        if profiling.active() is not None:
            raise HipExtensionError("graph capture with an active KernelTimer is not supported")
        g = _GraphedForward()
        g.x = torch.empty((B // 2 if cfg_shared else B, H * W, self._cin_pad), dtype=self._dtype, device=self._device)
        g.x.zero_()
        cur = torch.cuda.current_stream(self._device)
        side = torch.cuda.Stream(device=self._device)
        side.wait_stream(cur)
        with torch.cuda.stream(side), ops.plan_family(co_run):
            for _ in range(2):
                self.forward_packed(g.x, B, H, W, ehs, cfg_shared=cfg_shared)
        cur.wait_stream(side)
        torch.cuda.synchronize(self._device)
        g.graph = torch.cuda.CUDAGraph()
        g.ws = ops.new_workspace(self._device)
        self._capturing = True
        try:
            with ops.capture_in_flight(), ops.workspace_scope(g.ws), ops.plan_family(co_run), torch.cuda.graph(g.graph):
                g.out = self.forward_packed(g.x, B, H, W, ehs, cfg_shared=cfg_shared)
        finally:
            self._capturing = False
        while len(self._graphs) >= self.max_cached_graphs:
            self._graphs.pop(next(iter(self._graphs)))
        self._graphs[key] = g
        return g

    @_in_own_f32_mode
    def prepare_context(self, encoder_hidden_states):
        self._ensure()
        ehs = encoder_hidden_states
        if not ehs.is_cuda:
            raise HipExtensionError("encoder_hidden_states must be on the HIP device")
        ehs = ehs.contiguous()
        if ehs.dtype == self._dtype:
            return ehs
        if ehs.dtype not in (torch.float32, torch.bfloat16, torch.float16):
            ehs = ehs.float()
        return ops.cast(ehs, self._dtype)

    def pack_input(self, sample, dup=1, out=None, div=None):
        self._ensure()
        a, b = (sample if isinstance(sample, (tuple, list)) else (sample, None))
        if a.dtype != torch.float32:
            a = ops.cast(a.contiguous(), torch.float32)
        if b is not None and b.dtype != torch.float32:
            b = ops.cast(b.contiguous(), torch.float32)
        nch = a.shape[1] + (0 if b is None else b.shape[1])
        if nch != self.config.in_channels:
            raise ValueError(f"UNet expects {self.config.in_channels} input channels, got {nch}")
        if div is None:
            return ops.pack_unet_input(a.contiguous(), None if b is None else b.contiguous(), dup, self._cin_pad, self._dtype, out=out)
        div = tuple(div) if isinstance(div, (tuple, list)) else (div, 1.0)
        return ops.pack_unet_input(a.contiguous(), None if b is None else b.contiguous(), dup, self._cin_pad, self._dtype, out=out, div=div)

    @_in_own_f32_mode
    def __call__(self, sample, timestep, encoder_hidden_states=None, timestep_cond=None, cross_attention_kwargs=None,
                 added_cond_kwargs=None, return_dict=True, **kwargs):
        if timestep_cond is not None and self.config.time_cond_proj_dim is None:
            raise ValueError("timestep_cond was given, but this UNet has no time_embedding.cond_proj: its config key "
                             "time_cond_proj_dim is None")
        self._ensure()
        first = sample[0] if isinstance(sample, (tuple, list)) else sample
# ... 18 lines not shown
```

gm-diffusion_amd/gm_diffusion/hip_ops.py:

```python
from __future__ import annotations

import math
import os
import threading
import time

import torch

from . import profiling
from ._native import ACT_GEGLU, ACT_NONE, ACT_QUICK_GELU, ACT_SILU, GMD_BF16, GMD_F16, GMD_F32, GMD_F32S, GMD_F32SA, GMD_F32SW, HipExtensionError, check, lib

__all__ = [
    "ACT_NONE", "ACT_SILU", "ACT_GEGLU", "ACT_QUICK_GELU", "embedding_lookup", "dpm_step", "dpm_sde_step", "ddpm_step", "ddim_step", "lcm_step", "euler_step", "lms_step", "unipc_step", "HipExtensionError", "dtype_code", "gemm_nt", "conv3x3", "conv3x3_tail", "pack_shortcut", "shortcut_fold_ok", "attention", "softmax_rows", "set_f32_mode", "f32_split", "split_weights", "scale_weight", "split_attention_ok", "ff_fused_ok", "ff_geglu_fused", "gemm_qkv_vt", "dup_batch",
    "groupnorm_scale_shift", "groupnorm_apply", "groupnorm", "groupnorm_split", "layernorm", "geglu", "timestep_embedding", "timestep_embedding_add",
    "concat_channels", "cast", "pack_unet_input", "unpack_nchw", "latent_step", "cfg_std_ratio", "hdr_tail", "hdr_tail_resized", "prepare_sdr",
    "apply_gm_to_sdr", "tmo", "gamut_compress", "stage1_chain", "discretize_u16", "quantize_u8",
]


def dtype_code(dt):
    if dt == torch.float32:
        return GMD_F32
    if dt == torch.bfloat16:
        return GMD_BF16
    if dt == torch.float16:
        return GMD_F16
    raise HipExtensionError(f"unsupported dtype {dt}: the HIP kernels take float32, bfloat16 or float16")


HALF_DTYPES = (torch.bfloat16, torch.float16)

_F32_DEFAULT = os.environ.get("GMD_F32_MODE", "split")
if _F32_DEFAULT not in ("split", "exact"):
    raise HipExtensionError(f"GMD_F32_MODE={_F32_DEFAULT!r}: expected 'split' or 'exact'")
_tls = threading.local()


def f32_mode():
    return getattr(_tls, "f32_mode", None) or _F32_DEFAULT


def __getattr__(name):
    if name == "F32_MODE":
        return f32_mode()
    raise AttributeError(f"module {__name__!r} has no attribute {name!r}")


def set_f32_mode(mode):
    global _F32_DEFAULT
    if mode not in ("split", "exact"):
        raise HipExtensionError("f32 mode must be 'split' or 'exact'")
    prev, _F32_DEFAULT = _F32_DEFAULT, mode
    return prev


class f32_mode_scope:

    def __init__(self, mode):
        if mode not in ("split", "exact"):
            raise HipExtensionError("f32 mode must be 'split' or 'exact'")
        self.mode = mode

    def __enter__(self):
        self.prev = getattr(_tls, "f32_mode", None)
        _tls.f32_mode = self.mode
        return self

    def __exit__(self, *exc):
        _tls.f32_mode = self.prev
        return False


def f32_split():
    return f32_mode() == "split"


class plan_family:

    def __init__(self, family):
        self.family = 1 if family else 0

    def __enter__(self):
        self.prev = lib().gmd_gemm_plan_family(self.family)
        return self

    def __exit__(self, *exc):
        lib().gmd_gemm_plan_family(self.prev)
        return False


def check_split_range(what, *tensors, module=None):
    mode = getattr(module, "_f32_mode", None) or f32_mode()
    if mode != "split":
        return
    for t in tensors:
        if t is None or not torch.is_tensor(t) or t.dtype != torch.float32 or not t.is_cuda:
# ... 353 lines not shown
    if rowbias is not None and (rowbias[0] if isinstance(rowbias, tuple) else rowbias).shape[0] != B:
        raise HipExtensionError("conv3x3: rowbias must have one row per sample")
    ws = _workspace(x.device)
    x_split = bool(x_split) or is_asplit(x)
    code = _contract_code(x, w, cin, x_split)
    st = _colstats_buffer(colstats, x.dtype, B * ho * wo, cout, 9 * cin, 1, out_dtype, x.device, code=code)
    tm = profiling.active()
    tm = tm if tm is not None and tm.wants("conv3x3") else None
    t0 = tm.begin() if tm else None
    check(lib().gmd_conv3x3(_ptr(x), _ptr(w), _ptr(y), code, dtype_code(out_dtype), B, H, W, cin, cout,
                            stride, up, pad_mode, _ptr(_f32(bias, "bias")), rb_ptr, rb_ld,
                            _ptr(residual), float(getattr(w, "_alpha", 1.0)), _ptr(st), COLSTATS_BUCKET if st is not None else 0,
                            _ptr(ws), WORKSPACE_BYTES, _stream()), "gmd_conv3x3")
    if tm:
        tm.end("conv3x3", 2.0 * B * ho * wo * cout * 9 * cin, x.numel() * x.element_size() + w.numel() * w.element_size()
               + y.numel() * y.element_size(), t0)
    if st is not None:
        y._colstats = (st, cout)
    return y, ho, wo


USE_SHORTCUT_FOLD = os.environ.get("GMD_FUSE_SHORTCUT", "1") != "0"
shortcut_fold_uses = 0
shortcut_launches = 0


def pack_shortcut(w2, b2, wsc, bsc):
    if w2.dim() != 2 or wsc.dim() != 2 or w2.shape[0] != wsc.shape[0] or w2.dtype != wsc.dtype or w2.device != wsc.device:
        raise HipExtensionError(f"pack_shortcut: W2 {tuple(w2.shape)} {w2.dtype} and Wsc {tuple(wsc.shape)} {wsc.dtype} do not stack")
    if getattr(w2, "_split", False) or getattr(wsc, "_split", False) or getattr(w2, "_alpha", 1.0) != 1.0 or getattr(wsc, "_alpha", 1.0) != 1.0:
        raise HipExtensionError("pack_shortcut: plain (unscaled, unsplit) weights only")
    w = torch.cat([w2, wsc], 1).contiguous()
    b = None
    if b2 is not None or bsc is not None:
        zero = torch.zeros(w.shape[0], dtype=torch.float32, device=w.device)
        b = ((zero if b2 is None else _f32(b2, "bias")) + (zero if bsc is None else _f32(bsc, "bias"))).contiguous()
    return w, b


def shortcut_fold_ok(dtype, B, H, W, cin, k2, cout):
    if not USE_SHORTCUT_FOLD or not is_half(dtype) or k2 <= 0 or k2 % 64 or cin % 64:
        return False
    bm, bn, pf, _ = gemm_plan_info(dtype, B * H * W, cout, 9 * cin + k2)
    return pf == 283 and bm == 256 and bn in (128, 160)


def conv3x3_tail(x, x2, w, B, H, W, bias=None, rowbias=None, residual=None, out_dtype=None, colstats=False, ldx2=None, k2=None,
                 stride=1, upsample=False):
    global shortcut_fold_uses
    _dev(x, x2, w, bias, residual)
    rb_ptr, rb_ld = _rowbias(rowbias)
    cin, cout = x.shape[-1], w.shape[0]
    ldx2 = int(ldx2 or x2.shape[-1])
    k2 = int(k2 if k2 is not None else x2.shape[-1])
    if (x.numel() != B * H * W * cin or x2.numel() != B * H * W * ldx2 or w.shape[1] != 9 * cin + k2 or x.dtype != w.dtype
            or x2.dtype != w.dtype or k2 > ldx2):
        raise HipExtensionError(f"conv3x3_tail: shape/dtype mismatch x={tuple(x.shape)} x2={tuple(x2.shape)} w={tuple(w.shape)} B,H,W={B},{H},{W}")
    if getattr(w, "_split", False) or is_asplit(x) or is_asplit(x2):
        raise HipExtensionError("conv3x3_tail: plain operands only")
    out_dtype = out_dtype or x.dtype
    y = torch.empty((B, H * W, cout), dtype=out_dtype, device=x.device)
    if residual is not None and (residual.numel() != y.numel() or residual.dtype != x.dtype):
        raise HipExtensionError("conv3x3_tail: residual shape/dtype mismatch")
    if rowbias is not None and (rowbias[0] if isinstance(rowbias, tuple) else rowbias).shape[0] != B:
        raise HipExtensionError("conv3x3_tail: rowbias must have one row per sample")
    ws = _workspace(x.device)
    code = dtype_code(x.dtype)
    st = _colstats_buffer(colstats, x.dtype, B * H * W, cout, 9 * cin + k2, 1, out_dtype, x.device) if is_half(x.dtype) else None
    tm = profiling.active()
    tm = tm if tm is not None and tm.wants("conv3x3") else None
    t0 = tm.begin() if tm else None
    check(lib().gmd_conv3x3_tail(_ptr(x), _ptr(x2), _ptr(w), _ptr(y), code, dtype_code(out_dtype), B, H, W, cin, k2, ldx2, cout,
                                 int(stride), int(bool(upsample)), 0, _ptr(_f32(bias, "bias")), rb_ptr, rb_ld, _ptr(residual), 1.0,
                                 _ptr(st), COLSTATS_BUCKET if st is not None else 0, _ptr(ws), WORKSPACE_BYTES, _stream()), "gmd_conv3x3_tail")
    if tm:
        tm.end("conv3x3", 2.0 * B * H * W * cout * (9 * cin + k2), (x.numel() + x2.numel() + w.numel()) * x.element_size()
               + y.numel() * y.element_size(), t0)
    shortcut_fold_uses += 1
    if st is not None:
        y._colstats = (st, cout)
    return y, H, W


USE_CONV_GN_FUSION = os.environ.get("GMD_CONV_GN", "1") != "0"


def conv3x3_groupnorm(x, w, B, H, W, groups, gamma, beta, eps, silu=True, bias=None, rowbias=None, residual=None, want_raw=False,
                      colstats=False, split_out=False):
    _dev(x, w, bias, residual, gamma, beta)
    cin, cout = x.shape[-1], w.shape[0]
    code = _contract_code(x, w, cin, is_asplit(x)) if x.dtype == w.dtype and w.shape[1] == 9 * cin else -1
    if not (USE_CONV_GN_FUSION and code >= 0 and
            lib().gmd_conv3x3_gn_fusable(code, B, H, W, cin, cout, 1, 0, 0, groups, WORKSPACE_BYTES)):
        y, _, _ = conv3x3(x, w, B, H, W, bias=bias, rowbias=rowbias, residual=residual, colstats=colstats)
        return (y if want_raw else None), groupnorm(y, B, groups, gamma, beta, eps, silu=silu, split_out=split_out)
    if x.numel() != B * H * W * cin:
        raise HipExtensionError(f"conv3x3_groupnorm: shape mismatch x={tuple(x.shape)} B,H,W={B},{H},{W}")
    if residual is not None and (residual.numel() != B * H * W * cout or residual.dtype != x.dtype):
        raise HipExtensionError("conv3x3_groupnorm: residual shape/dtype mismatch")
    if rowbias is not None and (rowbias[0] if isinstance(rowbias, tuple) else rowbias).shape[0] != B:
        raise HipExtensionError("conv3x3_groupnorm: rowbias must have one row per sample")
    rb_ptr, rb_ld = _rowbias(rowbias)
    yn = torch.empty((B, H * W, cout), dtype=x.dtype, device=x.device)
    yr = torch.empty_like(yn) if want_raw else None
    ws = _workspace(x.device)
    tm = profiling.active()
    tm = tm if tm is not None and tm.wants("conv3x3") else None
    t0 = tm.begin() if tm else None
    check(lib().gmd_conv3x3_groupnorm(_ptr(x), _ptr(w), _ptr(yr), _ptr(yn), code, B, H, W, cin, cout, 1, 0, 0, _ptr(_f32(bias, "bias")),
                                      rb_ptr, rb_ld, _ptr(residual), float(getattr(w, "_alpha", 1.0)), groups, float(eps),
                                      _ptr(_f32(gamma, "gamma")), _ptr(_f32(beta, "beta")), int(silu), _ptr(ws), WORKSPACE_BYTES, _stream()),
          "gmd_conv3x3_groupnorm")
    if tm:
        tm.end("conv3x3", 2.0 * B * H * W * cout * 9 * cin, x.numel() * x.element_size() + w.numel() * w.element_size()
               + yn.numel() * yn.element_size(), t0)
    return yr, yn


SPLIT_ATTENTION_HEAD_DIMS = (40, 64, 80, 160)


def split_attention_ok(dtype, d):
    return dtype == torch.float32 and f32_split() and d in SPLIT_ATTENTION_HEAD_DIMS


def attention(q, k, vt, heads, nk, scale, k_col=0, causal=False, split_out=False):
    _dev(q, k, vt)
    B, nq = q.shape[0], q.shape[1]
    hd = vt.shape[1]
    d = hd // heads
    ldq, ldk = q.shape[2], k.shape[2]
    if k.shape[1] < nk or vt.shape[2] < nk or k_col + hd > ldk or hd > ldq:
        raise HipExtensionError("attention: operand shapes inconsistent")
    o = torch.empty((B, nq, hd), dtype=q.dtype, device=q.device)
    if q.dtype == torch.float32:
        if not (f32_split() and d in SPLIT_ATTENTION_HEAD_DIMS):
            raise HipExtensionError("attention: float32 runs on the split (three float16 products) kernel, head dims 40/64/80/160, "
                                    "in F32_MODE 'split' only; the exact float32 path composes gemm_nt + softmax_rows")
        so = bool(split_out) and want_split_out(q.dtype, hd)
        code = GMD_F32SA if so else GMD_F32S
    else:
        so = False
        code = dtype_code(q.dtype)
    tm = profiling.active()
    tm = tm if tm is not None and tm.wants("attention") else None
    t0 = tm.begin() if tm else None
    check(lib().gmd_attention(_ptr(q), _ptr(k) + k_col * k.element_size(), _ptr(vt), _ptr(o), code, B, heads, d,
                              nq, nk, ldq, ldk, vt.shape[2], hd, nq * ldq, k.shape[1] * ldk, hd * vt.shape[2], nq * hd,
                              float(scale), int(bool(causal)), _stream()), "gmd_attention")
    if tm:
        tm.end("attention", 4.0 * B * nq * nk * hd, (2 * B * nq * hd + 2 * B * nk * hd) * q.element_size(), t0)
    return _mark_asplit(o) if so else o


def softmax_rows(s, cols, scale, out_dtype, ldp=None, causal_nq=0):
    _dev(s)
    _f32(s, "softmax_rows input")
    lds_ = s.shape[-1]
    rows = s.numel() // lds_
    ldp = ldp or lds_
    p = torch.empty(s.shape[:-1] + (ldp,), dtype=out_dtype, device=s.device)
    check(lib().gmd_softmax_rows(_ptr(s), lds_, _ptr(p), dtype_code(out_dtype), ldp, rows, cols, float(scale), int(causal_nq), _stream()),
          "gmd_softmax_rows")
    return p


# ... 638 lines not shown
```

include/gmd_hip.h:

```cpp
#ifndef GMD_HIP_H
#define GMD_HIP_H

#include <stdint.h>

#ifdef __cplusplus
extern "C" {
#endif

#define GMD_ABI_VERSION 14
#define GMD_WS_TAIL_BYTES 65536

#define GMD_OK 0
#define GMD_ERR_INVALID 1
#define GMD_ERR_LAUNCH 2
#define GMD_ERR_UNSUPPORTED 3

#define GMD_F32 0
#define GMD_BF16 1
#define GMD_F16 2
#define GMD_F32S 3
#define GMD_F32SW 4
#define GMD_F32SA 5

#define GMD_ACT_NONE 0
// ... 68 lines not shown
int gmd_lcm_step(const float* eps_in, const float* x, const float* noise, int B, int64_t chw,
                 int do_cfg, float guidance_scale, const float* rescale_ratio, float guidance_rescale,
                 float sched_sqrt_alpha, float sched_sqrt_one_minus_alpha, int clip_sample, float clip_range,
                 float c_skip, float c_out, float sqrt_alpha_prev, float sqrt_beta_prev,
                 float sqrt_alpha, float sqrt_one_minus_alpha,
                 float* x_prev, float* x0, float* denoised, gmd_stream_t stream);

int gmd_euler_step(const float* eps_in, const float* x, const float* noise, int B, int64_t chw,
                   int do_cfg, float guidance_scale, const float* rescale_ratio, float guidance_rescale,
                   float sigma_hat, float dt, float sigma_up, float* x_prev, float* pred_x0, gmd_stream_t stream);

int gmd_lms_step(const float* eps_in, const float* x, const float* d1, const float* d2, const float* d3, int B, int64_t chw,
                 int do_cfg, float guidance_scale, const float* rescale_ratio, float guidance_rescale,
                 int order, float sigma, float c0, float c1, float c2, float c3,
                 float* d_out, float* x_prev, float* pred_x0, gmd_stream_t stream);

int gmd_unipc_step(const float* eps_in, const float* x, const float* last_sample, const float* h1, const float* h2, const float* h3,
                   int B, int64_t chw, int do_cfg, float guidance_scale, const float* rescale_ratio, float guidance_rescale,
                   int corr_order, int pred_order, float sigma_s, float alpha_s,
                   float c_x, float c_m, float c_b, float c_rho1, float c_rho2, float c_rho3, float c_r1, float c_r2,
                   float p_x, float p_m, float p_b, float p_rho1, float p_rho2, float p_r1, float p_r2,
                   float sqrt_alpha, float sqrt_one_minus_alpha,
                   float* m0_out, float* x_corr, float* x_prev, float* x0, gmd_stream_t stream);

int gmd_cfg_std_ratio(const float* eps_in, int B, int64_t chw, float guidance_scale,
                      float* ratio, gmd_stream_t stream);

int gmd_pack_unet_input(const float* src0, int C0, const float* src1, int C1, int B, int64_t HW,
                        int dup, void* out, int CP, int out_dtype, gmd_stream_t stream);
int gmd_pack_unet_input_scaled(const float* src0, int C0, float div0, const float* src1, int C1, float div1,
                               int B, int64_t HW, int dup, void* out, int CP, int out_dtype, gmd_stream_t stream);
int gmd_unpack_nchw(const void* in, int in_dtype, int64_t ld, int B, int C, int64_t HW,
                    float* out, gmd_stream_t stream);


int gmd_gemm_plan_override(int bm, int bn, int pf, int ksplit);

int gmd_gemm_plan_family(int family);

int gmd_splitk_fixup_max(int max_slices);

int gmd_gemm_nt(const void* A, const void* W, void* C, int dtype, int out_dtype,
                int M, int N, int K, int64_t lda, int64_t ldw, int64_t ldc,
                int batch, int64_t strideA, int64_t strideW, int64_t strideC,
                const float* bias, const float* rowbias, int rows_per_group, int64_t ldrb,
                const void* residual, int64_t ldr, int64_t strideR,
                float alpha, int act, float* colstats, int colstats_bucket,
                void* workspace, int64_t workspace_bytes, gmd_stream_t stream);

int gmd_split_weights(const float* W, void* out, int64_t N, int64_t K, int64_t ldw, gmd_stream_t stream);

int gmd_gemm_colstats_plan(int dtype, int M, int N, int K, int batch, int64_t workspace_bytes, int bucket);

int gmd_gemm_plan_info(int dtype, int M, int N, int K, int batch, int64_t workspace_bytes, int geglu, int* out4);

int gmd_gemm_qkv_vt_ok(int dtype, int M, int N, int K, int vt_col0, int vt_tokens, int64_t workspace_bytes);
int gmd_gemm_qkv_vt(const void* A, const void* W, void* C, void* Vt, int dtype, int M, int N, int K, int64_t ldc, int vt_col0, int vt_tokens,
                    int64_t vt_ld, float alpha, void* workspace, int64_t workspace_bytes, gmd_stream_t stream);

int gmd_gemm_out_split_ok(int M, int N, int K, int geglu, int64_t workspace_bytes);

int gmd_split_plan_ksplit(int M, int N, int K, int64_t workspace_bytes);

int gmd_conv_patch_override(int mode);

int gmd_stamp(uint64_t* base, const int* row, int stride, int k, gmd_stream_t stream);

int gmd_ff_geglu_fused_supported(int dtype, int64_t M, int C);
int gmd_ff_geglu_fused(const void* X, const void* W1i, const float* b1i, const void* W2, const float* b2, const void* residual,
                       void* Y, int dtype, int64_t M, int C, gmd_stream_t stream);

#define GMD_UPSAMPLE_TO(Hout, Wout) (((int)(Hout) << 16) | (int)(Wout))
int gmd_conv3x3(const void* X, const void* Wt, void* Y, int dtype, int out_dtype,
                int B, int Hin, int Win, int Cin, int Cout, int stride, int upsample, int pad_mode,
                const float* bias, const float* rowbias, int64_t ldrb, const void* residual, float alpha,
                float* colstats, int colstats_bucket,
                void* workspace, int64_t workspace_bytes, gmd_stream_t stream);

int gmd_conv3x3_tail(const void* X, const void* X2, const void* Wt, void* Y, int dtype, int out_dtype,
                     int B, int Hin, int Win, int Cin, int K2, int64_t ldx2, int Cout, int stride, int upsample, int pad_mode,
                     const float* bias, const float* rowbias, int64_t ldrb, const void* residual, float alpha,
                     float* colstats, int colstats_bucket,
                     void* workspace, int64_t workspace_bytes, gmd_stream_t stream);

int gmd_conv3x3_gn_fusable(int dtype, int B, int Hin, int Win, int Cin, int Cout, int stride, int upsample, int pad_mode,
                           int groups, int64_t workspace_bytes);
int gmd_conv3x3_groupnorm(const void* X, const void* Wt, void* Yraw, void* Ynorm, int dtype,
                          int B, int Hin, int Win, int Cin, int Cout, int stride, int upsample, int pad_mode,
                          const float* bias, const float* rowbias, int64_t ldrb, const void* residual, float alpha,
                          int groups, float eps, const float* gamma, const float* beta, int silu,
                          void* workspace, int64_t workspace_bytes, gmd_stream_t stream);

int gmd_attention(const void* Q, const void* K, const void* Vt, void* O, int dtype,
                  int B, int H, int D, int Nq, int Nk,
                  int64_t ldq, int64_t ldk, int64_t ldvt, int64_t ldo,
                  int64_t strideQ, int64_t strideK, int64_t strideVt, int64_t strideO,
                  float scale, int causal, gmd_stream_t stream);

int gmd_softmax_rows(const float* S, int64_t lds, void* P, int out_dtype, int64_t ldp,
                     int64_t rows, int cols, float scale, int causal_nq, gmd_stream_t stream);

int gmd_groupnorm_nsplit(int64_t HW);
int gmd_groupnorm_stats(const void* X, int dtype, int B, int64_t HW, int C, int G, float eps,
                        const float* gamma, const float* beta, float* workspace,
                        float* scale_shift, gmd_stream_t stream);
int gmd_groupnorm_split(const void* X, void* Y, int dtype, int B, int64_t HW, int C, int G, float eps,
                        const float* gamma, const float* beta, float* workspace, int silu, gmd_stream_t stream);
int gmd_groupnorm_apply(const void* X, void* Y, int dtype, int B, int64_t HW, int C,
                        const float* scale_shift, int silu, gmd_stream_t stream);
int gmd_groupnorm_colstats(const void* X, void* Y, int dtype, int B, int64_t HW, int C, int G, float eps,
                           const float* gamma, const float* beta, const float* stats_a, int Ca,
                           const float* stats_b, int bucket, int silu, gmd_stream_t stream);
int gmd_groupnorm_fused(const void* X, void* Y, int dtype, int B, int64_t HW, int C, int G, float eps,
                        const float* gamma, const float* beta, int silu, gmd_stream_t stream);
int gmd_layernorm(const void* X, void* Y, int dtype, int64_t rows, int C,
                  const float* gamma, const float* beta, float eps, gmd_stream_t stream);
int gmd_geglu(const void* X, void* Y, int dtype, int64_t rows, int F, gmd_stream_t stream);
int gmd_timestep_embedding(const float* t_dev, void* out, int dtype, int B, int dim,
                           int flip_sin_to_cos, float freq_shift, gmd_stream_t stream);
int gmd_timestep_embedding_add(const float* t_dev, const void* addend, void* out, int dtype, int B, int dim,
                               int flip_sin_to_cos, float freq_shift, gmd_stream_t stream);
int gmd_concat_channels(const void* A, int Ca, const void* Bm, int Cb, void* out, int dtype,
                        int64_t rows, gmd_stream_t stream);
int gmd_embedding_lookup(const int32_t* ids, const void* table, const void* pos, void* out, int dtype,
                         int64_t rows, int T, int C, int vocab, gmd_stream_t stream);
int gmd_dup_batch(const void* in, void* out, int64_t bytes, gmd_stream_t stream);
int gmd_cast(const void* in, int in_dtype, void* out, int out_dtype, int64_t n, gmd_stream_t stream);

#ifdef __cplusplus
}
#endif
#endif
```

Baseline: 5.593 HDR images/s.

## Fold nearest-2x upsample into four 2x2 phase convolutions for upsampler conv

Replaces the 3x3 convolution applied after nearest-neighbor 2x upsampling with four sub-pixel phase convolutions. Each phase uses 2x2 taps whose weights are pre-summed from the original 3x3 kernel, so K shrinks from 9*Cin to 4*Cin per output and the input is read at its original resolution. The GEMM kernel gains an UP2 mode that remaps output rows per phase, covering the residual, rowbias and colstats paths. This adds a new kernel instantiation and extra index arithmetic in the epilogue, and summing the taps in float before casting back changes rounding slightly.

```diff
diff --git a/gm-diffusion_amd/csrc/gemm.hip b/gm-diffusion_amd/csrc/gemm.hip
--- a/gm-diffusion_amd/csrc/gemm.hip
+++ b/gm-diffusion_amd/csrc/gemm.hip
@@ -69,9 +69,9 @@
     }
 }
 
-template <typename HT, int TM, int TN>
+template <typename HT, int TM, int TN, bool UP2 = false>
 __device__ __forceinline__ void epilogue_regs(const GemmParams& p, const f32x4 (&acc)[TM][TN], int mw, int nw, int frow, int fq,
-                                              int z, int ks) {
+                                              int z, int ks, int ph = 0) {
     const bool vec_c = (p.ldc % 4 == 0) && (p.sC % 4 == 0);
     const bool vec_r = p.residual != nullptr && (p.ldr % 4 == 0) && (p.sR % 4 == 0);
     const bool vec_n = (p.N % 4 == 0);
@@ -117,16 +117,23 @@
     }
 #pragma unroll
     for (int i = 0; i < TM; ++i) {
-        const int m = mw + i * 16 + frow;
-        if (m >= p.M) continue;
-        const float* rb = p.rowbias ? p.rowbias + (int64_t)(m / p.rows_per_group) * p.ldrb : nullptr;
+        int64_t m = mw + i * 16 + frow;
+        int grp;
+        if constexpr (UP2) {
+            if (m >= p.up2_rows) continue;
+            m = up2_out_row(p, (int)m, ph, grp);
+        } else {
+            if (m >= p.M) continue;
+            grp = (int)m / p.rows_per_group;
+        }
+        const float* rb = p.rowbias ? p.rowbias + (int64_t)grp * p.ldrb : nullptr;
 #pragma unroll
         for (int j = 0; j < TN; ++j) {
             const int n = nw + j * 16 + fq * 4;
             if (n >= p.N) continue;
             const int nvalid = p.N - n < 4 ? p.N - n : 4;
             float v[4] = {acc[i][j][0], acc[i][j][1], acc[i][j][2], acc[i][j][3]};
-            if (p.ksplit > 1) {
+            if (!UP2 && p.ksplit > 1) {
                 float* o = p.ws + ((int64_t)ks * p.M + m) * p.N + n;
                 if (nvalid == 4 && vec_n) *reinterpret_cast<float4*>(o) = make_float4(v[0], v[1], v[2], v[3]);
                 else
@@ -202,19 +209,21 @@
     }
 }
 
-template <typename HT, int TM, int TN, bool PLAIN>
+template <typename HT, int TM, int TN, bool PLAIN, bool UP2 = false>
 __device__ __forceinline__ void epilogue_rows_impl(const GemmParams& p, const f32x4 (&acc)[TM][TN], float* strip, int mw, int nw, int lane,
-                                                   int z) {
+                                                   int z, int ph = 0) {
     static_assert(TM % 2 == 0, "halves of two 16-row tiles");
-    if (p.vt_out && nw >= p.vt_col0) {
+    if (!UP2 && p.vt_out && nw >= p.vt_col0) {
         epilogue_cols_vt<HT, TM, TN>(p, acc, strip, mw, nw, lane);
         return;
     }
     constexpr int NCOL = TN * 16, ROWF = NCOL + 4, CH = NCOL / 8;
     constexpr int ITER = (32 * CH + 63) / 64;
     const int frow = lane & 15, fq = lane >> 4;
+    Up2Tile ut{};
+    if constexpr (UP2) ut = up2_tile(p, __builtin_amdgcn_readfirstlane(mw));
     int g0 = 0, grem = 0;
-    if (p.rowbias) {
+    if (!UP2 && p.rowbias) {
         g0 = mw / p.rows_per_group;
         grem = mw - g0 * p.rows_per_group;
     }
@@ -238,7 +247,12 @@
             const int idx = lane + 64 * t;
             const int r = idx / CH, c = idx - r * CH;
             if (32 * CH % 64 != 0 && r >= 32) continue;
-            resv[hh & 1][t] = *reinterpret_cast<const uint4*>((const HT*)p.residual + (int64_t)z * p.sR + (int64_t)(mw + hh * 32 + r) * p.ldr + nw + c * 8);
+            int64_t mo = mw + hh * 32 + r;
+            if constexpr (UP2) {
+                int smp;
+                mo = up2_tile_row(p, ut, hh * 32 + r, ph, smp);
+            }
+            resv[hh & 1][t] = *reinterpret_cast<const uint4*>((const HT*)p.residual + (int64_t)z * p.sR + mo * p.ldr + nw + c * 8);
         }
     };
     const bool res_pre = PLAIN && p.residual != nullptr;
@@ -252,7 +266,9 @@
                 const int r = idx / CH, c = idx - r * CH;
                 if (32 * CH % 64 != 0 && r >= 32) continue;
                 const int ro = h * 32 + r;
-                const int grp = p.rows_per_group >= 64 ? g0 + (grem + ro >= p.rows_per_group ? 1 : 0) : (mw + ro) / p.rows_per_group;
+                int grp;
+                if constexpr (UP2) up2_tile_row(p, ut, ro, ph, grp);
+                else grp = p.rows_per_group >= 64 ? g0 + (grem + ro >= p.rows_per_group ? 1 : 0) : (mw + ro) / p.rows_per_group;
                 const float* rb = p.rowbias + (int64_t)grp * p.ldrb + nw + c * 8;
                 resv[0][t] = __builtin_bit_cast(uint4, *reinterpret_cast<const float4*>(rb));
                 resv[1][t] = __builtin_bit_cast(uint4, *reinterpret_cast<const float4*>(rb + 4));
@@ -272,7 +288,10 @@
             const int idx = lane + 64 * t;
             const int r = idx / CH, c = idx - r * CH;
             if (32 * CH % 64 != 0 && r >= 32) continue;
-            const int m = mw + h * 32 + r, n = nw + c * 8;
+            const int n = nw + c * 8;
+            int64_t m = mw + h * 32 + r;
+            int smp = 0;
+            if constexpr (UP2) m = up2_tile_row(p, ut, h * 32 + r, ph, smp);
             const float4 a0 = *reinterpret_cast<const float4*>(strip + r * ROWF + c * 8);
             const float4 a1 = *reinterpret_cast<const float4*>(strip + r * ROWF + c * 8 + 4);
             float v[8] = {a0.x, a0.y, a0.z, a0.w, a1.x, a1.y, a1.z, a1.w};
@@ -288,7 +307,7 @@
                 add[0] += t0.x; add[1] += t0.y; add[2] += t0.z; add[3] += t0.w; add[4] += t1.x; add[5] += t1.y; add[6] += t1.z; add[7] += t1.w;
             } else if (p.rowbias) {
                 const int ro = h * 32 + r;
-                const int grp = p.rows_per_group >= 64 ? g0 + (grem + ro >= p.rows_per_group ? 1 : 0) : m / p.rows_per_group;
+                const int grp = UP2 ? smp : p.rows_per_group >= 64 ? g0 + (grem + ro >= p.rows_per_group ? 1 : 0) : (int)m / p.rows_per_group;
                 const float* rb = p.rowbias + (int64_t)grp * p.ldrb + n;
                 const float4 t0 = *reinterpret_cast<const float4*>(rb), t1 = *reinterpret_cast<const float4*>(rb + 4);
                 add[0] += t0.x; add[1] += t0.y; add[2] += t0.z; add[3] += t0.w; add[4] += t1.x; add[5] += t1.y; add[6] += t1.z; add[7] += t1.w;
@@ -339,9 +358,14 @@
     }
 #endif
 #undef EPI_STAMP
-    if (p.colstats)
-        colstats_store<NCOL, ROWF>(strip, lane, cs, cq, p.cs_bucket,
-                                   p.colstats + ((int64_t)(mw / (TM * 16)) * (p.N / p.cs_bucket) + nw / p.cs_bucket) * 2);
+    if (p.colstats) {
+        int64_t blk = mw / (TM * 16);
+        if constexpr (UP2) {
+            const int bps = p.Hin * p.Win / (TM * 16), smp = (int)blk / bps;
+            blk = ((int64_t)smp * 4 + ph) * bps + ((int)blk - smp * bps);
+        }
+        colstats_store<NCOL, ROWF>(strip, lane, cs, cq, p.cs_bucket, p.colstats + (blk * (p.N / p.cs_bucket) + nw / p.cs_bucket) * 2);
+    }
 }
 
 template <typename HT, int TM, int TN>
@@ -934,10 +958,12 @@
     }
 }
 
-template <typename HT, bool CONV, int TN>
+template <typename HT, bool CONV, int TN, bool UP2 = false>
 __global__ __launch_bounds__(768, 3) void gemm_pp_kernel(const GemmParams p) {
+    static_assert(CONV || !UP2, "the phase mode is a convolution");
     GMD_WG_TRACE_SCOPE(WGK_PP | (CONV ? WGK_CONV_BIT : 0));
     constexpr int WN = 2, NCONS = 8, LW = 4, TM = 4, NST = 3;
+    constexpr int NT = UP2 ? 4 : 9;
     constexpr int BM = 256, BN = WN * TN * 16;
     constexpr int RPP = LW * 8;
     constexpr int NA = BM / RPP;
@@ -962,6 +988,8 @@
         m0 = mt * BM;
         n0 = nt * BN;
     }
+    const int ph = UP2 ? (m0 / BM) & 3 : 0;
+    const int r0 = UP2 ? ((m0 / BM) >> 2) * BM : m0;
     const int z = p.ksplit > 1 ? 0 : blockIdx.z;
     const int ks = p.ksplit > 1 ? blockIdx.z : 0;
     const int nk_total = p.K / BK;
@@ -1031,23 +1059,24 @@
         bool pv[NA];
 #pragma unroll
         for (int i = 0; i < NA; ++i) {
-            const int m = m0 + srow + RPP * i;
-            pv[i] = m < p.M;
+            const int m = r0 + srow + RPP * i;
+            pv[i] = m < (UP2 ? p.up2_rows : p.M);
             pb[i] = py[i] = px[i] = 0;
             if (CONV) {
                 if (pv[i]) {
-                    const int hw = p.Hout * p.Wout;
-                    if (((hw & (hw - 1)) | (p.Wout & (p.Wout - 1))) == 0) {
-                        const int sh = __builtin_ctz(hw), sw = __builtin_ctz(p.Wout);
+                    const int iw = UP2 ? p.Win : p.Wout;
+                    const int hw = (UP2 ? p.Hin : p.Hout) * iw;
+                    if (((hw & (hw - 1)) | (iw & (iw - 1))) == 0) {
+                        const int sh = __builtin_ctz(hw), sw = __builtin_ctz(iw);
                         pb[i] = m >> sh;
                         const int rem = m & (hw - 1);
                         py[i] = rem >> sw;
-                        px[i] = rem & (p.Wout - 1);
+                        px[i] = rem & (iw - 1);
                     } else {
                         pb[i] = m / hw;
                         const int rem = m - pb[i] * hw;
-                        py[i] = rem / p.Wout;
-                        px[i] = rem - py[i] * p.Wout;
+                        py[i] = rem / iw;
+                        px[i] = rem - py[i] * iw;
                     }
                 }
                 aoff[i] = kOOB;
@@ -1058,14 +1087,14 @@
 #pragma unroll
         for (int i = 0; i < NW; ++i) {
             const int n = n0 + srow + RPP * i;
-            woff[i] = n < p.N ? (unsigned)n * (unsigned)p.ldw * 2u + (unsigned)chunk * 16u : kOOB;
+            woff[i] = n < p.N ? (unsigned)(UP2 ? ph * p.N + n : n) * (unsigned)p.ldw * 2u + (unsigned)chunk * 16u : kOOB;
         }
         int tap = 0, c0 = 0, cb0 = 0;
         bool newtap = true;
         if (CONV) {
-            const int sb = p.cblk / BK, per_cb = 9 * sb, nconv = 9 * (p.Cin / BK);
+            const int sb = p.cblk / BK, per_cb = NT * sb, nconv = NT * (p.Cin / BK);
             if (kt_begin >= nconv) {
-                tap = 9;
+                tap = NT;
                 cb0 = p.Cin;
                 c0 = (kt_begin - nconv) * BK;
             } else {
@@ -1085,7 +1114,7 @@
                        (unsigned)__builtin_amdgcn_readfirstlane(p.w_bytes), 0x00020000u};
         }
         u32x4 dA2 = dA;
-        if (CONV && p.K2 > 0) {
+        if (CONV && !UP2 && p.K2 > 0) {
             const uint64_t b2 = (uint64_t)p.A2;
             dA2 = u32x4{(unsigned)__builtin_amdgcn_readfirstlane((unsigned)b2), (unsigned)__builtin_amdgcn_readfirstlane((unsigned)(b2 >> 32) & 0xffffu),
                         (unsigned)__builtin_amdgcn_readfirstlane(p.a2_bytes), 0x00020000u};
@@ -1104,13 +1133,16 @@
             constexpr int lo = Q == 4 ? 0 : Q * NP / 4, hi = Q == 4 ? NP : (Q + 1) * NP / 4;
             unsigned kbytes = (unsigned)(kt_begin + kt) * (BK * 2);
             unsigned abytes = kbytes;
-            const bool tail = CONV && tap == 9;
+            const bool tail = CONV && !UP2 && tap == 9;
             if (CONV) {
                 if ((Q == 0 || Q == 4) && newtap) {
                     if (tail) {
 #pragma unroll
                         for (int i = 0; i < NA; ++i)
                             aoff[i] = pv[i] ? (unsigned)(m0 + srow + RPP * i) * (unsigned)p.lda2 * 2u + (unsigned)chunk * 16u : kOOB;
+                    } else if constexpr (UP2) {
+#pragma unroll
+                        for (int i = 0; i < NA; ++i) aoff[i] = up2_tap_offset(p, pv[i], pb[i], py[i], px[i], ph, tap, chunk);
                     } else {
                         const int ky = tap / 3, kx = tap - ky * 3;
 #pragma unroll
@@ -1131,11 +1163,11 @@
                 if (NA + i >= lo && NA + i < hi) dma16(dW, stage + BM * 128 + i * (RPP * 128), woff[i], kbytes);
             if (CONV && (Q == 3 || Q == 4)) {
                 c0 += BK;
-                if (tap < 9 && c0 >= cb0 + p.cblk) {
+                if (tap < NT && c0 >= cb0 + p.cblk) {
                     c0 = cb0;
                     ++tap;
                     newtap = true;
-                    if (tap == 9) {
+                    if (tap == NT) {
                         cb0 += p.cblk;
                         if (cb0 >= p.Cin) c0 = 0;
                         else { tap = 0; c0 = cb0; }
@@ -1272,6 +1304,22 @@
         q.ksplit = 1;
     }
     PP_PHASE_SYNC();
+    if constexpr (UP2) {
+        const int rw = r0 + wr * 64, nw = n0 + wc * (TN * 16);
+        if (rw >= q.up2_rows) return;
+        const bool rows_up = !q.out_f32 && q.ksplit <= 1 && q.act == GMD_ACT_NONE && rw + 64 <= q.up2_rows && n0 + BN <= q.N && (q.ldc & 7) == 0 &&
+                             (q.residual == nullptr || (q.ldr & 7) == 0) &&
+                             (q.rowbias == nullptr || ((q.ldrb & 3) == 0 && (reinterpret_cast<uintptr_t>(q.rowbias) & 15) == 0)) &&
+                             (reinterpret_cast<uintptr_t>(q.bias) & 15) == 0;
+        if (__builtin_expect(rows_up, 1)) {
+            constexpr int kStrip = 32 * (TN * 16 + 4);
+            epilogue_rows_impl<HT, TM, TN, true, true>(q, acc, reinterpret_cast<float*>(smem) + wid * kStrip, rw, nw, lane, z, ph);
+        } else {
+            epilogue_regs<HT, TM, TN, true>(q, acc, rw, nw, frow, fq, z, ks, ph);
+        }
+        PP_PHASE_EMIT();
+        return;
+    }
     const bool rows_ok = !q.out_f32 && q.ksplit <= 1 && q.act != GMD_ACT_GEGLU && m0 + BM <= q.M && n0 + BN <= q.N && (q.ldc & 7) == 0 &&
                          (q.sC & 7) == 0 && (q.residual == nullptr || ((q.ldr & 7) == 0 && (q.sR & 7) == 0)) &&
                          (q.rowbias == nullptr || ((q.ldrb & 3) == 0 && (reinterpret_cast<uintptr_t>(q.rowbias) & 15) == 0)) &&
@@ -2149,14 +2197,14 @@
     return hipGetLastError();
 }
 
-template <typename HT, bool CONV, int TN>
+template <typename HT, bool CONV, int TN, bool UP2 = false>
 hipError_t launch_pp(const GemmParams& p, int gz, hipStream_t s) {
     constexpr int BM = 256, BN = 2 * TN * 16;
     constexpr size_t smem = (size_t)3 * (BM + BN) * 128;
-    hipError_t e = opt_in_lds(reinterpret_cast<const void*>(&gemm_pp_kernel<HT, CONV, TN>), (int)smem);
+    hipError_t e = opt_in_lds(reinterpret_cast<const void*>(&gemm_pp_kernel<HT, CONV, TN, UP2>), (int)smem);
     if (e != hipSuccess) return e;
     dim3 grid(((p.N + BN - 1) / BN) * ((p.M + BM - 1) / BM), 1, gz);
-    gemm_pp_kernel<HT, CONV, TN><<<grid, 768, smem, s>>>(p);
+    gemm_pp_kernel<HT, CONV, TN, UP2><<<grid, 768, smem, s>>>(p);
     return hipGetLastError();
 }
 
@@ -2254,6 +2302,31 @@
     return GMD_OK;
 }
 
+template <typename HT>
+int launch_up2(GemmParams p, const Plan& pl, void* ws, int64_t ws_bytes, hipStream_t s) {
+    const PlanConfig cfg = plan_config();
+    p.ksplit = pl.ksplit;
+    p.ws = (float*)ws;
+    p.tile_group = 1;
+    p.fixup = 0;
+    if (pl.ksplit > 1) {
+        if (!fixup_plan_ok(cfg, pl, p.M, p.N, ws ? ws_bytes : 0, false)) {
+            gmd_set_error("gmd_conv3x3_up2: plan %dx%d ksplit=%d has no in-kernel reduction", pl.bm, pl.bn, pl.ksplit);
+            return GMD_ERR_UNSUPPORTED;
+        }
+        p.fixup = 1;
+        p.fix_bytes = (unsigned)fixup_bytes(pl, p.M, p.N);
+        p.fix_cnt = reinterpret_cast<unsigned*>(reinterpret_cast<char*>(ws) + ws_bytes);
+    }
+    const int gz = pl.ksplit > 1 ? pl.ksplit : 1;
+    const hipError_t e = pl.bn == 160 ? launch_pp<HT, true, 5, true>(p, gz, s) : launch_pp<HT, true, 4, true>(p, gz, s);
+    if (e != hipSuccess) {
+        gmd_set_error("gmd_conv3x3_up2: launch failed: %s", hipGetErrorString(e));
+        return GMD_ERR_LAUNCH;
+    }
+    return GMD_OK;
+}
+
 template <bool CONV>
 int launch(GemmParams p, int dtype, int batch, void* ws, int64_t ws_bytes, hipStream_t s, const char* name) {
     if (dtype == GMD_BF16) return launch_half<bf16_t, CONV>(p, batch, ws, ws_bytes, s, name);
@@ -2458,6 +2531,42 @@
                         colstats, colstats_bucket, workspace, gmd_ws_usable_bytes(workspace_bytes), stream, nullptr);
 }
 
+int gmd_conv3x3_up2(const void* X, const void* Wp, void* Y, int dtype, int out_dtype, int B, int Hin, int Win, int Cin, int Cout,
+                    const float* bias, const float* rowbias, int64_t ldrb, const void* residual, float* colstats, int colstats_bucket,
+                    void* workspace, int64_t workspace_bytes, gmd_stream_t stream) {
+    workspace_bytes = gmd_ws_usable_bytes(workspace_bytes);
+    GMD_REQUIRE(gmd_is_half(dtype), "gmd_conv3x3_up2: the 16-bit types only (dtype %d)", dtype);
+    GMD_REQUIRE(out_dtype == GMD_F32 || out_dtype == dtype, "gmd_conv3x3_up2: out_dtype must be F32 or the input dtype");
+    GMD_REQUIRE(B >= 0 && Hin > 0 && Win > 0 && Cin > 0 && Cout > 0, "gmd_conv3x3_up2: bad shape");
+    if (B == 0) return GMD_OK;
+    GMD_REQUIRE(Cin % 64 == 0, "gmd_conv3x3_up2: Cin=%d must be a multiple of 64", Cin);
+    GMD_REQUIRE(X && Wp && Y && gmd_aligned16(X) && gmd_aligned16(Wp) && gmd_aligned16(Y), "gmd_conv3x3_up2: null or unaligned pointer");
+    GMD_REQUIRE(bias == nullptr || gmd_aligned16(bias), "gmd_conv3x3_up2: bias must be 16-byte aligned (it is read with float4 loads)");
+    GMD_REQUIRE(residual == nullptr || (gmd_aligned16(residual) && out_dtype == dtype), "gmd_conv3x3_up2: unaligned residual, or out_dtype != dtype with one");
+    GMD_REQUIRE(colstats == nullptr || (colstats_bucket > 0 && out_dtype == dtype && Cout % colstats_bucket == 0),
+                "gmd_conv3x3_up2: column statistics need a bucket dividing Cout and out_dtype == dtype");
+    Plan pl{};
+    int M = 0;
+    if (!up2_plan(plan_config(), dtype, B, Hin, Win, Cin, Cout, colstats ? colstats_bucket : 0, workspace ? workspace_bytes : 0, pl, M)) {
+        gmd_set_error("gmd_conv3x3_up2: B=%d %dx%d %d->%d%s has no phase launch under this plan family (ask gmd_conv3x3_up2_plan first)", B, Hin, Win,
+                      Cin, Cout, colstats ? " with column statistics" : "");
+        return GMD_ERR_UNSUPPORTED;
+    }
+    GemmParams p{};
+    p.A = X; p.W = Wp; p.C = Y; p.M = M; p.N = Cout; p.K = 4 * Cin;
+    p.lda = Cin; p.ldw = 4 * (int64_t)Cin; p.ldc = Cout;
+    p.a_bytes = (unsigned)((int64_t)B * Hin * Win * Cin * 2); p.w_bytes = (unsigned)(16LL * Cout * Cin * 2);
+    p.bias = bias; p.rowbias = rowbias; p.rows_per_group = 4 * Hin * Win; p.ldrb = ldrb > 0 ? ldrb : Cout;
+    p.residual = residual; p.ldr = Cout; p.alpha = 1.0f; p.act = GMD_ACT_NONE;
+    p.out_f32 = out_dtype == GMD_F32;
+    p.Hin = Hin; p.Win = Win; p.Cin = Cin; p.Hout = 2 * Hin; p.Wout = 2 * Win; p.stride = 1; p.upsample = 1; p.pad_lo = 1;
+    p.cblk = conv_channel_block(plan_config(), B, Hin, Win, Cin, Cout, dtype);
+    p.colstats = colstats; p.cs_bucket = colstats_bucket;
+    p.up2 = 1; p.up2_rows = B * Hin * Win;
+    return dtype == GMD_BF16 ? launch_up2<bf16_t>(p, pl, workspace, workspace_bytes, (hipStream_t)stream)
+                             : launch_up2<f16_t>(p, pl, workspace, workspace_bytes, (hipStream_t)stream);
+}
+
 int gmd_conv3x3_tail(const void* X, const void* X2, const void* Wt, void* Y, int dtype, int out_dtype, int B, int Hin, int Win, int Cin, int K2,
                      int64_t ldx2, int Cout, int stride, int upsample, int pad_mode, const float* bias, const float* rowbias, int64_t ldrb,
                      const void* residual, float alpha, float* colstats, int colstats_bucket, void* workspace, int64_t workspace_bytes,
diff --git a/gm-diffusion_amd/csrc/gemm_params.h b/gm-diffusion_amd/csrc/gemm_params.h
--- a/gm-diffusion_amd/csrc/gemm_params.h
+++ b/gm-diffusion_amd/csrc/gemm_params.h
@@ -41,6 +41,8 @@
     int K2;
     int64_t lda2;
     unsigned a2_bytes;
+    int up2;
+    int up2_rows;
 };
 
 constexpr int kFixupCounters = 16384;
diff --git a/gm-diffusion_amd/csrc/gemm_plan.cpp b/gm-diffusion_amd/csrc/gemm_plan.cpp
--- a/gm-diffusion_amd/csrc/gemm_plan.cpp
+++ b/gm-diffusion_amd/csrc/gemm_plan.cpp
@@ -273,6 +273,21 @@
     return 1;
 }
 
+bool up2_plan(const PlanConfig& cfg, int dtype, int B, int Hin, int Win, int Cin, int Cout, int bucket, int64_t ws_bytes, Plan& pl, int& M) {
+    if (!is_half(dtype) || B <= 0 || Hin <= 0 || Win <= 0 || Cin <= 0 || Cout <= 0 || Cin % BK || bucket < 0) return false;
+    const int64_t rows = (int64_t)B * Hin * Win, mv = 4 * cdiv(rows, 256) * 256;
+    if (mv >= (1LL << 31) || rows * Cin * 2 >= 0xFFFF0000LL || 16LL * Cout * Cin * 2 >= 0xFFFF0000LL) return false;
+    M = (int)mv;
+    pl = make_plan(cfg, M, Cout, 4 * Cin, 1, ws_bytes, false, bucket > 0);
+    if (!(pl.pf == kPingPong && pl.bm == 256 && (pl.bn == 160 || pl.bn == 128)) || Cout % pl.bn) return false;
+    if (pl.ksplit > 1 && !fixup_plan_ok(cfg, pl, M, Cout, ws_bytes, false)) {
+        pl.ksplit = cfg.fixup_max >= 2 && pl.ksplit > cfg.fixup_max ? cfg.fixup_max : 1;
+        if (pl.ksplit > 1 && !fixup_plan_ok(cfg, pl, M, Cout, ws_bytes, false)) pl.ksplit = 1;
+    }
+    if (bucket > 0 && (((int64_t)Hin * Win) % 64 || (pl.bn / 2) % bucket)) return false;
+    return true;
+}
+
 }
 
 using namespace gmd;
@@ -340,6 +355,14 @@
     return GMD_OK;
 }
 
+int gmd_conv3x3_up2_plan(int dtype, int B, int Hin, int Win, int Cin, int Cout, int colstats_bucket, int64_t workspace_bytes, int* out4) {
+    Plan pl{};
+    int M = 0;
+    if (!up2_plan(plan_config(), dtype, B, Hin, Win, Cin, Cout, colstats_bucket, gmd_ws_usable_bytes(workspace_bytes), pl, M)) return 0;
+    if (out4) { out4[0] = pl.bm; out4[1] = pl.bn; out4[2] = pl.pf; out4[3] = pl.ksplit; }
+    return 1;
+}
+
 int gmd_split_plan_ksplit(int M, int N, int K, int64_t workspace_bytes) {
     if (M <= 0 || N <= 0 || K <= 0 || K % BKS) return 0;
     return f32_plan(M, N, K, 1, gmd_ws_usable_bytes(workspace_bytes), false).ksplit;
diff --git a/gm-diffusion_amd/csrc/gemm_plan.h b/gm-diffusion_amd/csrc/gemm_plan.h
--- a/gm-diffusion_amd/csrc/gemm_plan.h
+++ b/gm-diffusion_amd/csrc/gemm_plan.h
@@ -71,6 +71,8 @@
 bool conv_out_shape(int Hin, int Win, int stride, int& upsample, int pad_mode, int& Hout, int& Wout, int& pad_lo);
 int conv_plan_ksplit(const PlanConfig& cfg, int dtype, int64_t M, int Cin, int Cout, int64_t ws_bytes);
 
+bool up2_plan(const PlanConfig& cfg, int dtype, int B, int Hin, int Win, int Cin, int Cout, int bucket, int64_t ws_bytes, Plan& pl, int& M);
+
 inline bool is_half(int dtype) { return dtype == GMD_BF16 || dtype == GMD_F16; }
 inline bool is_split(int dtype) { return dtype == GMD_F32S || dtype == GMD_F32SW || dtype == GMD_F32SA; }
 
diff --git a/gm-diffusion_amd/csrc/gemm_shared.h b/gm-diffusion_amd/csrc/gemm_shared.h
--- a/gm-diffusion_amd/csrc/gemm_shared.h
+++ b/gm-diffusion_amd/csrc/gemm_shared.h
@@ -154,6 +154,51 @@
     return (unsigned)(((b * p.Hin + iy) * p.Win + ix) * p.Cin) * 2u + (unsigned)chunk * 16u;
 }
 
+__device__ __forceinline__ unsigned up2_tap_offset(const GemmParams& p, bool valid, int b, int i, int j, int ph, int tap, int chunk) {
+    if (!valid) return kOOB;
+    const int iy = i + (tap >> 1) + (ph >> 1) - 1, ix = j + (tap & 1) + (ph & 1) - 1;
+    if (iy < 0 || ix < 0 || iy >= p.Hin || ix >= p.Win) return kOOB;
+    return (unsigned)(((b * p.Hin + iy) * p.Win + ix) * p.Cin) * 2u + (unsigned)chunk * 16u;
+}
+
+__device__ __forceinline__ int64_t up2_out_row(const GemmParams& p, int r, int ph, int& b) {
+    const int hw = p.Hin * p.Win;
+    b = r / hw;
+    const int rem = r - b * hw;
+    const int i = rem / p.Win, j = rem - i * p.Win;
+    return ((int64_t)b * p.Hout + 2 * i + (ph >> 1)) * p.Wout + 2 * j + (ph & 1);
+}
+
+struct Up2Tile {
+    int b0, i0, j0;
+    float inv_w, inv_h;
+};
+__device__ __forceinline__ Up2Tile up2_tile(const GemmParams& p, int mw) {
+    Up2Tile t;
+    const int hw = p.Hin * p.Win;
+    t.b0 = mw / hw;
+    const int rem = mw - t.b0 * hw;
+    t.i0 = rem / p.Win;
+    t.j0 = rem - t.i0 * p.Win;
+    t.inv_w = 1.0f / (float)p.Win;
+    t.inv_h = 1.0f / (float)p.Hin;
+    return t;
+}
+__device__ __forceinline__ int up2_small_div(int n, int d, float inv) {
+    int q = (int)((float)n * inv);
+    if (q * d > n) --q;
+    if ((q + 1) * d <= n) ++q;
+    return q;
+}
+__device__ __forceinline__ int64_t up2_tile_row(const GemmParams& p, const Up2Tile& t, int ro, int ph, int& b) {
+    const int n = t.j0 + ro, cj = up2_small_div(n, p.Win, t.inv_w);
+    const int j = n - cj * p.Win;
+    const int n2 = t.i0 + cj, ci = up2_small_div(n2, p.Hin, t.inv_h);
+    const int i = n2 - ci * p.Hin;
+    b = t.b0 + ci;
+    return ((int64_t)b * p.Hout + 2 * i + (ph >> 1)) * p.Wout + 2 * j + (ph & 1);
+}
+
 template <int N> __device__ __forceinline__ void wait_vmcnt() { asm volatile("s_waitcnt vmcnt(%0)" ::"n"(N) : "memory"); }
 
 hipError_t opt_in_lds(const void* fn, int bytes) {
diff --git a/gm-diffusion_amd/gm_diffusion/_native/__init__.py b/gm-diffusion_amd/gm_diffusion/_native/__init__.py
--- a/gm-diffusion_amd/gm_diffusion/_native/__init__.py
+++ b/gm-diffusion_amd/gm_diffusion/_native/__init__.py
@@ -58,6 +58,8 @@
     "gmd_ff_geglu_fused": [P, P, P, P, P, P, P, I, L, I, P],
     "gmd_conv3x3": [P, P, P, I, I, I, I, I, I, I, I, I, I, P, P, L, P, F, P, I, P, L, P],
     "gmd_conv3x3_tail": [P, P, P, P, I, I, I, I, I, I, I, L, I, I, I, I, P, P, L, P, F, P, I, P, L, P],
+    "gmd_conv3x3_up2_plan": [I, I, I, I, I, I, I, L, P],
+    "gmd_conv3x3_up2": [P, P, P, I, I, I, I, I, I, I, P, P, L, P, P, I, P, L, P],
     "gmd_conv3x3_gn_fusable": [I, I, I, I, I, I, I, I, I, I, L],
     "gmd_conv3x3_groupnorm": [P, P, P, P, I, I, I, I, I, I, I, I, I, P, P, L, P, F, I, F, P, P, I, P, L, P],
     "gmd_attention": [P, P, P, P, I, I, I, I, I, I, L, L, L, L, L, L, L, L, F, I, P],
diff --git a/gm-diffusion_amd/gm_diffusion/components/autoencoder_kl.py b/gm-diffusion_amd/gm_diffusion/components/autoencoder_kl.py
--- a/gm-diffusion_amd/gm_diffusion/components/autoencoder_kl.py
+++ b/gm-diffusion_amd/gm_diffusion/components/autoencoder_kl.py
@@ -164,6 +164,8 @@
             e = dict(res=[resnet(f"decoder.up_blocks.{i}.resnets.{j}") for j in range(c.layers_per_block + 1)])
             if i != len(rev) - 1:
                 e["us"] = self._conv3(f"decoder.up_blocks.{i}.upsamplers.0.conv")
+                if ops.USE_UPSAMPLE_PHASES and ops.is_half(self._dtype) and e["us"][0].shape[1] % (9 * 64) == 0:
+                    e["us4"] = ops.pack_upsample_phases(e["us"][0])[0]
             w["d_up"].append(e)
         w["d_norm"] = self._norm("decoder.conv_norm_out")
         wo = self._raw["decoder.conv_out.weight"]
@@ -239,7 +241,10 @@
             for r in blk["res"]:
                 x = self._resnet(r, x, B, H, W)
             if "us" in blk:
-                x, H, W = ops.conv3x3(x, blk["us"][0], B, H, W, bias=blk["us"][1], upsample=True)
+                if "us4" in blk and ops.upsample_phases_ok(self._dtype, B, H, W, x.shape[-1], blk["us4"].shape[1]):
+                    x, H, W = ops.conv3x3_up2(x, blk["us4"], B, H, W, bias=blk["us"][1])
+                else:
+                    x, H, W = ops.conv3x3(x, blk["us"][0], B, H, W, bias=blk["us"][1], upsample=True)
         x = ops.groupnorm(x, B, c.norm_num_groups, w["d_norm"][0], w["d_norm"][1], 1e-6, silu=True)
         y, _, _ = ops.conv3x3(x, w["d_out"][0], B, H, W, bias=w["d_out"][1], out_dtype=torch.float32)
         return y, H, W
diff --git a/gm-diffusion_amd/gm_diffusion/components/unet_2d_condition.py b/gm-diffusion_amd/gm_diffusion/components/unet_2d_condition.py
--- a/gm-diffusion_amd/gm_diffusion/components/unet_2d_condition.py
+++ b/gm-diffusion_amd/gm_diffusion/components/unet_2d_condition.py
@@ -453,6 +453,8 @@
                 e["attn"] = [transformer(f"up_blocks.{i}.attentions.{j}", blk["heads"], blk["depth"]) for j in range(len(blk["res"]))]
             if blk["up"]:
                 e["us"] = self._conv3(f"up_blocks.{i}.upsamplers.0.conv")
+                if ops.USE_UPSAMPLE_PHASES and ops.is_half(self._dtype) and e["us"][0].shape[1] % (9 * 64) == 0:
+                    e["us4"] = ops.pack_upsample_phases(e["us"][0])[0]
             w["up"].append(e)
         w["norm_out"] = self._norm("conv_norm_out")
         w["conv_out"] = self._conv3("conv_out")
@@ -755,7 +757,11 @@
                     x = self._transformer(blk["attn"][j], x, B, H, W, ehs)
             if "us" in blk:
                 ho, wo = skips[-1][1:]
-                x, H, W = ops.conv3x3(x, blk["us"][0], B, H, W, bias=blk["us"][1], out_size=(ho, wo), colstats=self._wants_colstats(ho, wo))
+                cs = self._wants_colstats(ho, wo)
+                if "us4" in blk and ops.upsample_phases_ok(self._dtype, B, H, W, x.shape[-1], blk["us4"].shape[1], (ho, wo), colstats=cs):
+                    x, H, W = ops.conv3x3_up2(x, blk["us4"], B, H, W, bias=blk["us"][1], colstats=cs)
+                else:
+                    x, H, W = ops.conv3x3(x, blk["us"][0], B, H, W, bias=blk["us"][1], out_size=(ho, wo), colstats=cs)
             mark()
         x = ops.groupnorm(x, B, c.norm_num_groups, w["norm_out"][0], w["norm_out"][1], eps, silu=True, split_out=self._sa(w["conv_out"][0]))
         y, _, _ = ops.conv3x3(x, w["conv_out"][0], B, H, W, bias=w["conv_out"][1], out_dtype=torch.float32)
diff --git a/gm-diffusion_amd/gm_diffusion/hip_ops.py b/gm-diffusion_amd/gm_diffusion/hip_ops.py
--- a/gm-diffusion_amd/gm_diffusion/hip_ops.py
+++ b/gm-diffusion_amd/gm_diffusion/hip_ops.py
@@ -11,7 +11,7 @@
 from ._native import ACT_GEGLU, ACT_NONE, ACT_QUICK_GELU, ACT_SILU, GMD_BF16, GMD_F16, GMD_F32, GMD_F32S, GMD_F32SA, GMD_F32SW, HipExtensionError, check, lib
 
 __all__ = [
-    "ACT_NONE", "ACT_SILU", "ACT_GEGLU", "ACT_QUICK_GELU", "embedding_lookup", "dpm_step", "dpm_sde_step", "ddpm_step", "ddim_step", "lcm_step", "euler_step", "lms_step", "unipc_step", "HipExtensionError", "dtype_code", "gemm_nt", "conv3x3", "conv3x3_tail", "pack_shortcut", "shortcut_fold_ok", "attention", "softmax_rows", "set_f32_mode", "f32_split", "split_weights", "scale_weight", "split_attention_ok", "ff_fused_ok", "ff_geglu_fused", "gemm_qkv_vt", "dup_batch",
+    "ACT_NONE", "ACT_SILU", "ACT_GEGLU", "ACT_QUICK_GELU", "embedding_lookup", "dpm_step", "dpm_sde_step", "ddpm_step", "ddim_step", "lcm_step", "euler_step", "lms_step", "unipc_step", "HipExtensionError", "dtype_code", "gemm_nt", "conv3x3", "conv3x3_tail", "pack_shortcut", "shortcut_fold_ok", "conv3x3_up2", "pack_upsample_phases", "upsample_phases_ok", "attention", "softmax_rows", "set_f32_mode", "f32_split", "split_weights", "scale_weight", "split_attention_ok", "ff_fused_ok", "ff_geglu_fused", "gemm_qkv_vt", "dup_batch",
     "groupnorm_scale_shift", "groupnorm_apply", "groupnorm", "groupnorm_split", "layernorm", "geglu", "timestep_embedding", "timestep_embedding_add",
     "concat_channels", "cast", "pack_unet_input", "unpack_nchw", "latent_step", "cfg_std_ratio", "hdr_tail", "hdr_tail_resized", "prepare_sdr",
     "apply_gm_to_sdr", "tmo", "gamut_compress", "stage1_chain", "discretize_u16", "quantize_u8",
@@ -531,6 +531,98 @@
     return y, H, W
 
 
+USE_UPSAMPLE_PHASES = os.environ.get("GMD_UPSAMPLE_PHASES", "1") != "0"
+upsample_phase_uses = 0
+_PHASE_TAPS = (((0,), (1, 2)), ((0, 1), (2,)))
+
+
+def pack_upsample_phases(w, bias=None):
+    if w.dim() != 2 or w.shape[1] % 9:
+        raise HipExtensionError(f"pack_upsample_phases: w {tuple(w.shape)} is not [Cout, 9*Cin]")
+    if getattr(w, "_split", False) or getattr(w, "_alpha", 1.0) != 1.0:
+        raise HipExtensionError("pack_upsample_phases: plain (unscaled, unsplit) weights only")
+    co, ci = w.shape[0], w.shape[1] // 9
+    w9 = w.to(torch.float32 if is_half(w.dtype) else w.dtype).view(co, 3, 3, ci)
+    out = torch.empty((4, co, 4, ci), dtype=w9.dtype, device=w.device)
+    for py in range(2):
+        for px in range(2):
+            for a in range(2):
+                for b in range(2):
+                    out[2 * py + px, :, 2 * a + b] = sum(w9[:, ky, kx] for ky in _PHASE_TAPS[py][a] for kx in _PHASE_TAPS[px][b])
+    return out.view(4, co, 4 * ci).to(w.dtype).contiguous(), (None if bias is None else _f32(bias, "bias"))
+
+
+def _up2_plan(dtype, B, H, W, cin, cout, bucket):
+    import ctypes
+
+    out = (ctypes.c_int * 4)()
+    ok = lib().gmd_conv3x3_up2_plan(dtype_code(dtype), B, H, W, cin, cout, bucket, WORKSPACE_BYTES, ctypes.addressof(out))
+    return tuple(out) if ok else None
+
+
+def upsample_phases_plan(dtype, B, H, W, cin, cout, colstats=False):
+    return _up2_plan(dtype, B, H, W, cin, cout, COLSTATS_BUCKET if colstats else 0) if is_half(dtype) else None
+
+
+def _up2_statistics(dtype, B, H, W, cin, cout, colstats):
+    if not is_half(dtype) or cin % 64:
+        return None
+    if colstats and USE_COLSTATS and cout % COLSTATS_BUCKET == 0 and (4 * B * H * W) % 64 == 0:
+        if _up2_plan(dtype, B, H, W, cin, cout, COLSTATS_BUCKET) is not None:
+            return True
+        if lib().gmd_gemm_colstats_plan(dtype_code(dtype), 4 * B * H * W, cout, 9 * cin, 1, WORKSPACE_BYTES, COLSTATS_BUCKET):
+            return None
+    return False if _up2_plan(dtype, B, H, W, cin, cout, 0) is not None else None
+
+
+def upsample_phases_ok(dtype, B, H, W, cin, cout, out_size=None, colstats=False):
+    if not USE_UPSAMPLE_PHASES or (out_size is not None and (int(out_size[0]), int(out_size[1])) != (2 * H, 2 * W)):
+        return False
+    return _up2_statistics(dtype, B, H, W, cin, cout, colstats) is not None
+
+
+def conv3x3_up2(x, wp, B, H, W, bias=None, rowbias=None, residual=None, out_dtype=None, colstats=False, out=None):
+    global upsample_phase_uses
+    _dev(x, wp, bias, residual)
+    rb_ptr, rb_ld = _rowbias(rowbias)
+    cin = x.shape[-1]
+    if wp.dim() != 3 or wp.shape[0] != 4 or wp.shape[2] != 4 * cin or x.numel() != B * H * W * cin or x.dtype != wp.dtype or not wp.is_contiguous():
+        raise HipExtensionError(f"conv3x3_up2: shape/dtype mismatch x={tuple(x.shape)} wp={tuple(wp.shape)} B,H,W={B},{H},{W}")
+    if getattr(wp, "_split", False) or is_asplit(x):
+        raise HipExtensionError("conv3x3_up2: plain operands only")
+    cout = wp.shape[1]
+    out_dtype = out_dtype or x.dtype
+    ho, wo = 2 * H, 2 * W
+    if out is None:
+        y = torch.empty((B, ho * wo, cout), dtype=out_dtype, device=x.device)
+    else:
+        _dev(out)
+        if out.shape != (B, ho * wo, cout) or out.dtype != out_dtype or not out.is_contiguous():
+            raise HipExtensionError(f"conv3x3_up2: out {tuple(out.shape)} {out.dtype} is not a contiguous [{B}, {ho * wo}, {cout}] {out_dtype}")
+        y = out
+    if residual is not None and (residual.numel() != y.numel() or residual.dtype != x.dtype):
+        raise HipExtensionError("conv3x3_up2: residual shape/dtype mismatch")
+    if rowbias is not None and (rowbias[0] if isinstance(rowbias, tuple) else rowbias).shape[0] != B:
+        raise HipExtensionError("conv3x3_up2: rowbias must have one row per sample")
+    ws = _workspace(x.device)
+    st = None
+    if out_dtype == x.dtype and _up2_statistics(x.dtype, B, H, W, cin, cout, colstats):
+        st = torch.empty((B * ho * wo // 64, cout // COLSTATS_BUCKET, 2), dtype=torch.float32, device=x.device)
+    tm = profiling.active()
+    tm = tm if tm is not None and tm.wants("conv3x3") else None
+    t0 = tm.begin() if tm else None
+    check(lib().gmd_conv3x3_up2(_ptr(x), _ptr(wp), _ptr(y), dtype_code(x.dtype), dtype_code(out_dtype), B, H, W, cin, cout,
+                                _ptr(_f32(bias, "bias")), rb_ptr, rb_ld, _ptr(residual), _ptr(st), COLSTATS_BUCKET if st is not None else 0,
+                                _ptr(ws), WORKSPACE_BYTES, _stream()), "gmd_conv3x3_up2")
+    if tm:
+        tm.end("conv3x3", 2.0 * B * ho * wo * cout * 4 * cin, x.numel() * x.element_size() + wp.numel() * wp.element_size()
+               + y.numel() * y.element_size(), t0)
+    upsample_phase_uses += 1
+    if st is not None:
+        y._colstats = (st, cout)
+    return y, ho, wo
+
+
 USE_CONV_GN_FUSION = os.environ.get("GMD_CONV_GN", "1") != "0"
 
 
diff --git a/include/gmd_hip.h b/include/gmd_hip.h
--- a/include/gmd_hip.h
+++ b/include/gmd_hip.h
@@ -174,6 +174,13 @@
                      const float* bias, const float* rowbias, int64_t ldrb, const void* residual, float alpha,
                      float* colstats, int colstats_bucket,
                      void* workspace, int64_t workspace_bytes, gmd_stream_t stream);
+
+int gmd_conv3x3_up2_plan(int dtype, int B, int Hin, int Win, int Cin, int Cout, int colstats_bucket, int64_t workspace_bytes, int* out4);
+int gmd_conv3x3_up2(const void* X, const void* Wp, void* Y, int dtype, int out_dtype,
+                    int B, int Hin, int Win, int Cin, int Cout,
+                    const float* bias, const float* rowbias, int64_t ldrb, const void* residual,
+                    float* colstats, int colstats_bucket,
+                    void* workspace, int64_t workspace_bytes, gmd_stream_t stream);
 
 int gmd_conv3x3_gn_fusable(int dtype, int B, int Hin, int Win, int Cin, int Cout, int stride, int upsample, int pad_mode,
                            int groups, int64_t workspace_bytes);
```

Result: faster. 5.717 HDR images/s (median of 6 runs) (+2.2%).
